# shenyunhang/APE

Hardware: NVIDIA H100
Metric: images_per_sec (higher is better)
Workload: dtype f16

## Files before the change

ape_b200/_lib.py:

```python
import ctypes
import os

import torch

_HERE = os.path.dirname(os.path.abspath(__file__))
LIB_PATH = os.path.join(_HERE, "libape_b200.so")

APE_DTYPE_F32, APE_DTYPE_F16, APE_DTYPE_BF16, APE_DTYPE_E4M3 = 0, 1, 2, 3
_DTYPE_CODE = {torch.float32: APE_DTYPE_F32, torch.float16: APE_DTYPE_F16, torch.bfloat16: APE_DTYPE_BF16,
               torch.float8_e4m3fn: APE_DTYPE_E4M3}

CONTAINER_ONLY = os.environ.get("APE_B200_CONTAINER_ONLY") == "1"


class _NotLoaded:
    def __getattr__(self, name):
        raise RuntimeError(f"libape_b200.so is not loaded (APE_B200_CONTAINER_ONLY=1): `{name}` is unavailable; "
                           "ape_b200 has no CPU / PyTorch fallback")


if CONTAINER_ONLY:
    lib = _NotLoaded()
elif not os.path.exists(LIB_PATH):
    raise ImportError(
        f"{LIB_PATH} not found: build it with `make` (or `python -c 'import __graft_entry__ as g; g.build()'`). "
        "ape_b200 has no CPU / PyTorch fallback."
    )
else:
    lib = ctypes.CDLL(LIB_PATH)

_vp, _i, _i64 = ctypes.c_void_p, ctypes.c_int, ctypes.c_int64


def _declare(lib):

    lib.ape_abi_version.restype = _i
    lib.ape_abi_version.argtypes = []
    lib.ape_last_error.restype = ctypes.c_char_p
    lib.ape_last_error.argtypes = []
    lib.ape_launch_count.restype = ctypes.c_uint64
    lib.ape_launch_count.argtypes = []
    lib.ape_msda_fwd.restype = _i
    lib.ape_msda_fwd.argtypes = [_vp] * 6 + [_i] * 8 + [_vp]
    lib.ape_msda_fwd_variant.restype = _i
    lib.ape_msda_fwd_variant.argtypes = [_vp] * 6 + [_i] * 9 + [_vp]
    lib.ape_msda_fused_fwd.restype = _i
    lib.ape_msda_fused_fwd.argtypes = [_vp, _vp, _vp, _vp, _i64, _vp, _i64, _vp, _i, _vp] + [_i] * 9 + [_vp]

    lib.ape_msda_bwd.restype = _i
    lib.ape_msda_bwd.argtypes = [_vp] * 9 + [_i] * 8 + [_vp]
    lib.ape_msda_pair_values.restype = _i
    lib.ape_msda_pair_values.argtypes = [_vp, _i64, _vp, _vp, _i, _i, _i, _i, _i, _vp]
    lib.ape_msda_pair_supported.restype = _i
    lib.ape_msda_pair_supported.argtypes = [_vp, _i, _i, _i, _i, _i]
    lib.ape_msda_pair_fused_fwd.restype = _i
    lib.ape_msda_pair_fused_fwd.argtypes = [_vp, _vp, _vp, _vp, _vp, _i64, _vp, _i64, _vp, _i, _vp] + [_i] * 12 + [_vp]
    lib.ape_gemm_tn.restype = _i
    lib.ape_gemm_tn.argtypes = [_vp, _i64, _vp, _i64, _vp, _i64, _vp, _vp, _i64] + [_i] * 7 + [_vp]

    lib.ape_gemm_tn_ex.restype = _i
    lib.ape_gemm_tn_ex.argtypes = [_vp, _i64, _vp, _i64, _vp, _i64, _vp, _vp, _i64] + [_i] * 8 + [_vp]
    lib.ape_gemm_tn_fused.restype = _i
    lib.ape_gemm_tn_fused.argtypes = [_vp, _i64, _vp, _i64, _vp, _i64, _vp, _vp, _i64] + [_i] * 8 + [_vp, _i, _vp, ctypes.c_float, ctypes.c_float, _vp, _i, _vp]
    lib.ape_gemm_tn_e4m3.restype = _i
    lib.ape_gemm_tn_e4m3.argtypes = [_vp, _i64, _vp, _i64, _vp, _vp, _vp, _i64, _vp, _i, _i, _i, _i, _i, _vp, _i, _vp]
    lib.ape_conv3x3_nhwc.restype = _i
    lib.ape_conv3x3_nhwc.argtypes = [_vp, _vp, _vp, _vp] + [_i] * 7 + [_vp]
    lib.ape_gemm_set_trace.restype = None
    lib.ape_gemm_set_trace.argtypes = [_vp]
    lib.ape_ffn_fused.restype = _i
    lib.ape_ffn_fused.argtypes = [_vp, _i64, _vp, _i64, _vp, _vp, _i64, _vp, _vp, _i64] + [_i] * 5 + [_vp]
    lib.ape_gemm_tn_rope.restype = _i
    lib.ape_gemm_tn_rope.argtypes = [_vp, _i64, _vp, _i64, _vp, _i64, _vp, _i, _i, _i, _i, _i, _vp, _vp, _vp, _i, _i, _i, _i, _vp]

    lib.ape_layernorm.restype = _i
    lib.ape_layernorm.argtypes = [_vp, _i64, _vp, _i64, _vp, _vp, _vp, _i, _i, ctypes.c_float, _i, _i, _vp]
    lib.ape_layernorm_e4m3.restype = _i
    lib.ape_layernorm_e4m3.argtypes = [_vp, _i64, _vp, _i64, _vp, _vp, _vp, _vp, _i, _i, ctypes.c_float, _i, _vp]
    lib.ape_layernorm_ex.restype = _i
    lib.ape_layernorm_ex.argtypes = [_vp, _i64, _vp, _i64, _vp, _vp, ctypes.c_float, _vp, _vp, ctypes.c_float, _vp, _i64, _i,
                                     _vp, _i64, _vp, _i64, _i, _i, _i, _i, _vp]
    lib.ape_groupnorm_workspace_bytes.restype = _i64
    lib.ape_groupnorm_workspace_bytes.argtypes = [_i, _i, _i]
    lib.ape_groupnorm_nhwc.restype = _i
    lib.ape_groupnorm_nhwc.argtypes = [_vp, _i64, _vp, _i64, _i64, _vp, _vp, _vp, _i, _i, _i, _i, ctypes.c_float, _i, _i, _vp]
    lib.ape_rope_qk.restype = _i
    lib.ape_rope_qk.argtypes = [_vp, _i64, _vp, _vp, _vp, _i, _i, _i, _i, _i, _vp]

    lib.ape_text_embed_packed.restype = _i
    lib.ape_text_embed_packed.argtypes = [_vp] * 5 + [_i] * 4 + [_vp]
    lib.ape_rows_gather.restype = _i
    lib.ape_rows_gather.argtypes = [_vp, _i64, _vp, _vp, _i64, _i, _i, _vp]

    lib.ape_attn_fwd.restype = _i
    lib.ape_attn_fwd.argtypes = [_vp, _i64, _vp, _i64, _i, _i, _i, _i, ctypes.c_float, _i, _vp]
    lib.ape_attn_fwd_ex.restype = _i
    lib.ape_attn_fwd_ex.argtypes = [_vp, _i64, _vp, _i64, _i, _i, _i, _i, _i, ctypes.c_float, _i, _vp, _i, _i, _i64, _vp]
    lib.ape_attn_fwd_mapped.restype = _i
    lib.ape_attn_fwd_mapped.argtypes = [_vp, _i64, _vp, _i64, _i, _i, _i, _i, _i, ctypes.c_float, _i, _vp, _i, _i, _i64, _vp, _vp]
    lib.ape_attn_fwd_seg.restype = _i
    lib.ape_attn_fwd_seg.argtypes = [_vp, _i64, _vp, _i64, _i, _i, _i, _i, _i, ctypes.c_float, _i, _vp, _i, _i, _i64, _vp, _vp]
    lib.ape_attn_variant.restype = _i
    lib.ape_attn_variant.argtypes = [_i]
    lib.ape_attn_cross_fwd.restype = _i
    lib.ape_attn_cross_fwd.argtypes = [_vp, _i64, _vp, _i64, _vp, _i64, _vp, _i64, _i, _i, _i, _i, _i, _i, ctypes.c_float, _i, _vp]
    lib.ape_vlf_pool_workspace_bytes.restype = _i64
    lib.ape_vlf_pool_workspace_bytes.argtypes = [_i, _i, _i, _i]
    lib.ape_vlf_pool.restype = _i
    lib.ape_vlf_pool.argtypes = [_vp, _vp, _vp, _vp, ctypes.POINTER(ctypes.c_void_p), ctypes.POINTER(_i)] + [_i] * 6 + [_vp]
    lib.ape_nms_workspace_bytes.restype = _i64
    lib.ape_nms_workspace_bytes.argtypes = [_i]
    lib.ape_nms_sorted.restype = _i
    lib.ape_nms_sorted.argtypes = [_vp, _i, ctypes.c_float, _vp, _vp, _vp, _vp]
    lib.ape_nms_sorted_dev.restype = _i
    lib.ape_nms_sorted_dev.argtypes = [_vp, _i, _vp, ctypes.c_float, _vp, _vp, _vp, _vp]
    lib.ape_nms_classwise_workspace_bytes.restype = _i64
    lib.ape_nms_classwise_workspace_bytes.argtypes = [_i]
    lib.ape_nms_classwise.restype = _i
    lib.ape_nms_classwise.argtypes = [_vp, _vp, _i64, _vp, _i, _i, ctypes.c_float, ctypes.c_float, _vp, _vp, _vp]
    lib.ape_ref_update.restype = _i
    lib.ape_ref_update.argtypes = [_vp, _vp, _vp, _vp, _vp, _i, _i, _i, ctypes.c_float, _vp]
    lib.ape_gemv_f32.restype = _i
    lib.ape_gemv_f32.argtypes = [_vp, _vp, _vp, _vp, _i, _i, _i, _vp]
    lib.ape_mask_crop_workspace_bytes.restype = _i64
    lib.ape_mask_crop_workspace_bytes.argtypes = [_i, _i, _i]
    lib.ape_mask_crop.restype = _i
    lib.ape_mask_crop.argtypes = [_vp] * 5 + [_i] * 7 + [_vp]
    lib.ape_mask_paste.restype = _i
    lib.ape_mask_paste.argtypes = [_vp, _vp, _vp, _i, _i, _i, _i, ctypes.c_float, _vp]
    lib.ape_mask_paste_rle.restype = _i
    lib.ape_mask_paste_rle.argtypes = [_vp, _vp, _i, _i, _i, _i, ctypes.c_float, _vp, _vp, _vp, _vp]
    lib.ape_rle_to_string.restype = _i
    lib.ape_rle_to_string.argtypes = [_vp, _i, _vp]
    lib.ape_resample_ksize.restype = _i
    lib.ape_resample_ksize.argtypes = [_i, _i]
    lib.ape_resample_coeffs_u8.restype = _i
    lib.ape_resample_coeffs_u8.argtypes = [_i, _i, _vp, _vp]
    lib.ape_resample_u8.restype = _i
    lib.ape_resample_u8.argtypes = [_vp, _i64, _vp, _vp, _i64, _i64, _vp, _vp, _i, _vp, _vp, _i] + [_i] * 6 + [_vp]
    lib.ape_semseg_resample.restype = _i
    lib.ape_semseg_resample.argtypes = [_vp, _vp, _vp, _i64] + [_i] * 13 + [_vp]
    lib.ape_semseg_keys_init.restype = _i
    lib.ape_semseg_keys_init.argtypes = [_vp, _i64, ctypes.c_float, _i, _vp]
    lib.ape_gemm_tn_argmax.restype = _i
    lib.ape_gemm_tn_argmax.argtypes = [_vp, _i64, _vp, _i64, _vp, _i, _i, _i, _i, _i, _vp]
    lib.ape_semseg_keys_decode.restype = _i
    lib.ape_semseg_keys_decode.argtypes = [_vp, _i64, _vp, _vp, _vp]
    lib.ape_panoptic_winners.restype = _i
    lib.ape_panoptic_winners.argtypes = [_vp] * 5 + [_i] * 9 + [ctypes.c_float, _i, _vp]



if not CONTAINER_ONLY:
    _declare(lib)

EXPORTS = (
    "ape_abi_version",
    "ape_last_error",
    "ape_launch_count",
    "ape_msda_fwd",
    "ape_msda_fwd_variant",
    "ape_msda_fused_fwd",
    "ape_msda_bwd",
    "ape_msda_pair_values",
    "ape_msda_pair_supported",
    "ape_msda_pair_fused_fwd",
    "ape_gemm_tn",
    "ape_gemm_tn_ex",
    "ape_gemm_tn_fused",
    "ape_gemm_tn_e4m3",
    "ape_conv3x3_nhwc",
    "ape_gemm_tn_rope",
    "ape_ffn_fused",
    "ape_gemm_set_trace",
    "ape_layernorm",
    "ape_layernorm_e4m3",
    "ape_layernorm_ex",
    "ape_rope_qk",
    "ape_text_embed_packed",
    "ape_rows_gather",
    "ape_attn_fwd",
    "ape_attn_fwd_ex",
    "ape_attn_fwd_mapped",
    "ape_attn_fwd_seg",
    "ape_attn_variant",
    "ape_attn_cross_fwd",
    "ape_groupnorm_workspace_bytes",
    "ape_groupnorm_nhwc",
    "ape_vlf_pool_workspace_bytes",
    "ape_vlf_pool",
    "ape_nms_workspace_bytes",
    "ape_nms_sorted",
    "ape_nms_sorted_dev",
    "ape_nms_classwise_workspace_bytes",
    "ape_nms_classwise",
    "ape_ref_update",
    "ape_gemv_f32",
    "ape_mask_crop_workspace_bytes",
    "ape_mask_crop",
    "ape_mask_paste",
    "ape_mask_paste_rle",
    "ape_rle_to_string",
    "ape_resample_ksize",
    "ape_resample_coeffs_u8",
    "ape_resample_u8",
    "ape_semseg_resample",
    "ape_semseg_keys_init",
    "ape_gemm_tn_argmax",
    "ape_semseg_keys_decode",
    "ape_panoptic_winners",
)


def dtype_code(dt: torch.dtype) -> int:
    try:
        return _DTYPE_CODE[dt]
    except KeyError:
        raise RuntimeError(f"ape_b200: unsupported dtype {dt} (float32 / float16 / bfloat16 / float8_e4m3fn only)") from None


def check(status: int, what: str) -> None:
    if status != 0:
        msg = lib.ape_last_error().decode("utf-8", "replace")
        raise RuntimeError(f"{what} failed (status {status}): {msg}")


def current_stream_ptr() -> int:
    return torch.cuda.current_stream().cuda_stream


def launch_count() -> int:
    return int(lib.ape_launch_count())
```

ape_b200/csrc/ffn_fused.cu:

```cuda
#include "attn.cuh"
#include "common.cuh"
#include "tc.cuh"

namespace ape {
namespace {

constexpr int E = 256, BM = 128, HC = 64;
constexpr int kThreads = 384;

struct alignas(1024) FfnSmem {
  uint8_t x[E / 64][BM * 128];
  uint8_t w1[2][E / 64][HC * 128];
  uint8_t w2[2][E * 128];
  uint64_t x_full, w1_full[2], w1_empty[2], w2_full[2], w2_empty[2];
};

struct FfnParams {
  const float *b1, *b2;
  const void *x;
  float *out;
  long long ldx, ldo;
  int M, F;
};

template <typename T, int CL>
__global__ void __launch_bounds__(kThreads, 1)
ffn_fused_kernel(const __grid_constant__ CUtensorMap map_x, const __grid_constant__ CUtensorMap map_w1,
                 const __grid_constant__ CUtensorMap map_w2, const FfnParams p) {
  extern __shared__ uint8_t smem_raw[];
  pdl_launch_dependents();
  FfnSmem &s = *reinterpret_cast<FfnSmem *>((reinterpret_cast<uintptr_t>(smem_raw) + 1023) & ~uintptr_t(1023));
  const int warp = threadIdx.x >> 5, lane = threadIdx.x & 31;
  const int rank = CL > 1 ? (int)tc::cluster_ctarank() : 0;
  const int row0 = blockIdx.x * BM;
  const int nch = p.F / HC;

  if (warp == 8 && lane == 0) {
    tc::prefetch_tensormap(&map_x);
    tc::prefetch_tensormap(&map_w1);
    tc::prefetch_tensormap(&map_w2);
    tc::mbar_init(&s.x_full, 1);
#pragma unroll
    for (int b = 0; b < 2; ++b) {
      tc::mbar_init(&s.w1_full[b], 1);
      tc::mbar_init(&s.w1_empty[b], 8 * CL);
      tc::mbar_init(&s.w2_full[b], 1);
      tc::mbar_init(&s.w2_empty[b], 8 * CL);
    }
    tc::fence_mbar_init();
  }
  __syncthreads();
  if (CL > 1) tc::cluster_sync_all();
  pdl_wait();

  if (warp >= 8) {
    tc::setmaxnreg_dec<40>();
    if (warp == 8 && lane == 0) {
      tc::mbar_expect_tx(&s.x_full, E * BM * 2);
#pragma unroll
      for (int c = 0; c < E / 64; ++c)
#pragma unroll
        for (int h = 0; h < 2; ++h) tc::tma_load_2d(s.x[c] + h * 64 * 128, &map_x, &s.x_full, c * 64, row0 + h * 64);
      for (int j = 0; j < nch; ++j) {
        const int b = j & 1, n = j >> 1;
        tc::mbar_wait(&s.w1_empty[b], (n & 1) ^ 1);
        tc::mbar_expect_tx(&s.w1_full[b], E * HC * 2);
        if (CL == 1) {
#pragma unroll
          for (int c = 0; c < E / 64; ++c) tc::tma_load_2d(s.w1[b][c], &map_w1, &s.w1_full[b], c * 64, j * HC);
        } else {
#pragma unroll
          for (int c = 2 * rank; c < 2 * rank + 2; ++c)
            tc::tma_load_2d_multicast(s.w1[b][c], &map_w1, &s.w1_full[b], c * 64, j * HC, (uint16_t)3);
        }
        tc::mbar_wait(&s.w2_empty[b], (n & 1) ^ 1);
        tc::mbar_expect_tx(&s.w2_full[b], E * HC * 2);
        if (CL == 1) {
#pragma unroll
          for (int q = 0; q < E / 64; ++q) tc::tma_load_2d(s.w2[b] + q * 64 * 128, &map_w2, &s.w2_full[b], j * HC, q * 64);
        } else {
#pragma unroll
          for (int q = 2 * rank; q < 2 * rank + 2; ++q)
            tc::tma_load_2d_multicast(s.w2[b] + q * 64 * 128, &map_w2, &s.w2_full[b], j * HC, q * 64, (uint16_t)3);
        }
      }
    }
    __syncwarp();
  } else {
    tc::setmaxnreg_inc<232>();
    const int g = warp >> 2, tq = lane & 3;
    auto release = [&](uint64_t *bar) {
      if (lane == 0) {
        tc::mbar_arrive(bar);
        if (CL > 1) tc::mbar_arrive_cluster(tc::mapa_u32(bar, (uint32_t)(rank ^ 1)));
      }
    };
    auto issue_s = [&](float *sc, int b) {
#pragma unroll
      for (int c = 0; c < E / 64; ++c) {
        const uint64_t dx = tc::make_smem_desc_sw128(tc::smem_u32(s.x[c] + g * 64 * 128));
        const uint64_t dw = tc::make_smem_desc_sw128(tc::smem_u32(s.w1[b][c]));
#pragma unroll
        for (int k = 0; k < 4; ++k) tc::Wgmma<64, T>::template ss<0>(sc, dx + 2 * k, dw + 2 * k, (c | k) != 0);
      }
    };
    float o[E / 2];
#pragma unroll
    for (int i = 0; i < E / 2; ++i) o[i] = 0.f;
    float sc[32];
    tc::mbar_wait(&s.x_full, 0);
    tc::mbar_wait(&s.w1_full[0], 0);
    tc::wgmma_fence();
    issue_s(sc, 0);
    tc::wgmma_commit();
    tc::wgmma_wait<0>();
    tc::fence_regs<32>(sc);
    release(&s.w1_empty[0]);

    for (int j = 0; j < nch; ++j) {
      const int b = j & 1, n = j >> 1;
      uint32_t pa[4][4];
#pragma unroll
      for (int jj = 0; jj < 8; ++jj) {
        float2 bb = make_float2(0.f, 0.f);
        if (p.b1 != nullptr) bb = __ldg(reinterpret_cast<const float2 *>(p.b1 + j * HC + 8 * jj + 2 * tq));
#pragma unroll
        for (int h = 0; h < 2; ++h) {
          float v0 = sc[4 * jj + 2 * h], v1 = sc[4 * jj + 2 * h + 1];
          if (p.b1 != nullptr) {
            v0 += bb.x;
            v1 += bb.y;
          }
          pa[jj >> 1][2 * (jj & 1) + h] = attn::pack2<T>(fmaxf(v0, 0.f), fmaxf(v1, 0.f));
        }
      }
      tc::mbar_wait(&s.w2_full[b], n & 1);
      tc::fence_regs<E / 2>(o);
      tc::wgmma_fence();
      const uint64_t dw2 = tc::make_smem_desc_sw128(tc::smem_u32(s.w2[b]));
#pragma unroll
      for (int kk = 0; kk < 4; ++kk) tc::Wgmma<256, T>::template rs<0>(o, pa[kk], dw2 + 2 * kk, (j | kk) != 0);
      tc::wgmma_commit();
      if (j + 1 < nch) {
        const int b1 = b ^ 1;
        tc::mbar_wait(&s.w1_full[b1], ((j + 1) >> 1) & 1);
        issue_s(sc, b1);
        tc::wgmma_commit();
        tc::wgmma_wait<1>();
        tc::fence_regs<E / 2>(o);
        release(&s.w2_empty[b]);
        tc::wgmma_wait<0>();
        tc::fence_regs<32>(sc);
        release(&s.w1_empty[b1]);
      } else {
        tc::wgmma_wait<0>();
        tc::fence_regs<E / 2>(o);
        release(&s.w2_empty[b]);
      }
    }

    const T *xg = reinterpret_cast<const T *>(p.x);
#pragma unroll
    for (int h = 0; h < 2; ++h) {
      const int m = row0 + g * 64 + (warp & 3) * 16 + (lane >> 2) + 8 * h;
      if (m < p.M) {
        const T *xr = xg + (size_t)m * p.ldx + 2 * tq;
        float *dst = p.out + (size_t)m * p.ldo + 2 * tq;
#pragma unroll
        for (int jj = 0; jj < E / 8; ++jj) {
          float v0 = o[4 * jj + 2 * h], v1 = o[4 * jj + 2 * h + 1];
          if (p.b2 != nullptr) {
            const float2 bb = __ldg(reinterpret_cast<const float2 *>(p.b2 + 8 * jj + 2 * tq));
            v0 += bb.x;
            v1 += bb.y;
          }
          const float2 r = Elem<T>::load2(xr + 8 * jj);
          v0 += r.x;
          v1 += r.y;
          *reinterpret_cast<float2 *>(dst + 8 * jj) = make_float2(v0, v1);
        }
      }
    }
  }
  __syncthreads();
  if (CL > 1) tc::cluster_sync_all();
}

template <typename T, int CL>
int launch(const CUtensorMap &mx, const CUtensorMap &m1, const CUtensorMap &m2, const FfnParams &p, cudaStream_t st) {
  const size_t smem = sizeof(FfnSmem) + 1024;
  auto k = ffn_fused_kernel<T, CL>;
  static bool set = false;
  if (!set) {
    cudaError_t e = cudaFuncSetAttribute(k, cudaFuncAttributeMaxDynamicSharedMemorySize, (int)smem);
    if (e != cudaSuccess) return fail((int)e, "ffn_fused: cudaFuncSetAttribute(smem=%zu): %s", smem, cudaGetErrorString(e));
    set = true;
  }
  const int tiles = (p.M + BM - 1) / BM;
  cudaLaunchConfig_t cfg{};
  cfg.gridDim = dim3((unsigned)((tiles + CL - 1) / CL * CL));
  cfg.blockDim = dim3(kThreads);
  cfg.dynamicSmemBytes = smem;
  cfg.stream = st;
  cudaLaunchAttribute attr[2];
  attr[0].id = cudaLaunchAttributeClusterDimension;
  attr[0].val.clusterDim.x = CL;
  attr[0].val.clusterDim.y = 1;
  attr[0].val.clusterDim.z = 1;
  attr[1].id = cudaLaunchAttributeProgrammaticStreamSerialization;
  attr[1].val.programmaticStreamSerializationAllowed = pdl_enabled() ? 1 : 0;
  cfg.attrs = attr;
  cfg.numAttrs = 2;
  cudaError_t e = cudaLaunchKernelEx(&cfg, k, mx, m1, m2, p);
  if (e != cudaSuccess) return fail((int)e, "ffn_fused_kernel launch: %s", cudaGetErrorString(e));
  return check_launch("ffn_fused_kernel");
}

}
}

using namespace ape;

extern "C" int ape_ffn_fused(const void *x, int64_t ldx, const void *w1, int64_t ldw1, const float *b1, const void *w2,
                             int64_t ldw2, const float *b2, float *out, int64_t ldo, int M, int E_, int F, int dtype,
                             int variant, void *stream) {
  if (dtype != APE_DTYPE_F16 && dtype != APE_DTYPE_BF16)
    return fail(APE_ERR_INVALID_ARG, "ffn_fused: operands must be fp16 or bf16 (got dtype %d)", dtype);
  if (E_ != E) return fail(APE_ERR_UNSUPPORTED, "ffn_fused: embedding width %d (only %d)", E_, E);
  if (F <= 0 || F % HC) return fail(APE_ERR_UNSUPPORTED, "ffn_fused: hidden width %d is not a positive multiple of %d", F, HC);
  if (M < 0) return fail(APE_ERR_INVALID_ARG, "ffn_fused: bad row count %d", M);
  if (variant < 0 || variant > 2) return fail(APE_ERR_INVALID_ARG, "ffn_fused: bad variant %d", variant);
  if (ldo == 0) ldo = E;
  if (M == 0) return APE_OK;
  if (!x || !w1 || !w2 || !out) return fail(APE_ERR_NULL_PTR, "ffn_fused: null pointer argument");
  if (((reinterpret_cast<uintptr_t>(x) | reinterpret_cast<uintptr_t>(w1) | reinterpret_cast<uintptr_t>(w2)) & 15) ||
      ldx % 8 || ldw1 % 8 || ldw2 % 8)
    return fail(APE_ERR_INVALID_ARG, "ffn_fused: x / w1 / w2 base and row pitch must be 16-byte aligned (TMA)");
  if (ldx < E || ldw1 < E || ldw2 < F || ldo < E) return fail(APE_ERR_INVALID_ARG, "ffn_fused: row pitch smaller than the row");
  if ((reinterpret_cast<uintptr_t>(out) & 7) || ldo % 2 ||
      ((reinterpret_cast<uintptr_t>(b1) | reinterpret_cast<uintptr_t>(b2)) & 7))
    return fail(APE_ERR_INVALID_ARG, "ffn_fused: out (and its row pitch) and b1 / b2 must allow 8-byte pairs");
  CUtensorMap mx, m1, m2;
  if (int rc = attn::make_map(&mx, x, dtype, M, E, ldx)) return rc;
  if (int rc = attn::make_map(&m1, w1, dtype, F, E, ldw1)) return rc;
  if (int rc = attn::make_map(&m2, w2, dtype, E, F, ldw2)) return rc;
  FfnParams p{b1, b2, x, out, ldx, ldo, M, F};
  const bool cluster = variant == 2;
  cudaStream_t st = reinterpret_cast<cudaStream_t>(stream);
  if (dtype == APE_DTYPE_BF16)
    return cluster ? launch<__nv_bfloat16, 2>(mx, m1, m2, p, st) : launch<__nv_bfloat16, 1>(mx, m1, m2, p, st);
  return cluster ? launch<__half, 2>(mx, m1, m2, p, st) : launch<__half, 1>(mx, m1, m2, p, st);
}
```

ape_b200/csrc/norm_rope.cu:

```cuda
#include <cuda_fp8.h>

#include "common.cuh"

namespace ape {
namespace {

template <typename T>
struct Vec8 {
  static constexpr int kBytes = 8 * sizeof(T);
};

template <typename T>
__device__ __forceinline__ void load8(const T *p, float *f) {
  if constexpr (sizeof(T) == 4) {
    const float4 a = *reinterpret_cast<const float4 *>(p), b = *reinterpret_cast<const float4 *>(p + 4);
    f[0] = a.x; f[1] = a.y; f[2] = a.z; f[3] = a.w; f[4] = b.x; f[5] = b.y; f[6] = b.z; f[7] = b.w;
  } else {
    const uint4 v = *reinterpret_cast<const uint4 *>(p);
    Elem<T>::unpack(v, f);
  }
}
template <typename T>
__device__ __forceinline__ void store8(T *p, const float *f) {
  if constexpr (sizeof(T) == 4) {
    *reinterpret_cast<float4 *>(p) = make_float4(f[0], f[1], f[2], f[3]);
    *reinterpret_cast<float4 *>(p + 4) = make_float4(f[4], f[5], f[6], f[7]);
  } else {
    *reinterpret_cast<uint4 *>(p) = Elem<T>::pack(f);
  }
}

__device__ __forceinline__ float warp_sum(float v) {
#pragma unroll
  for (int o = 16; o > 0; o >>= 1) v += __shfl_xor_sync(0xffffffffu, v, o);
  return v;
}

template <typename TI, typename TO, int MAXV>
__global__ void __launch_bounds__(256)
layernorm_kernel(const TI *__restrict__ x, long long ldx, TO *__restrict__ y, long long ldy,
                 const float *__restrict__ w, const float *__restrict__ b, const int *__restrict__ row_map,
                 int rows, int C, float eps) {
  pdl_prologue();
  const int warp = (blockIdx.x * blockDim.x + threadIdx.x) >> 5, lane = threadIdx.x & 31;
  if (warp >= rows) return;
  const TI *xr = x + (size_t)warp * ldx;
  const int nvec = (C + 7) >> 3;
  float v[MAXV][8];
  float sum = 0.f;
#pragma unroll
  for (int i = 0; i < MAXV; ++i) {
    const int j = lane + 32 * i;
    if (j < nvec) {
      load8<TI>(xr + 8 * j, v[i]);
#pragma unroll
      for (int k = 0; k < 8; ++k) {
        if (8 * j + k >= C) v[i][k] = 0.f;
        sum += v[i][k];
      }
    }
  }
  const float mean = warp_sum(sum) / (float)C;
  float sq = 0.f;
#pragma unroll
  for (int i = 0; i < MAXV; ++i) {
    const int j = lane + 32 * i;
    if (j < nvec) {
#pragma unroll
      for (int k = 0; k < 8; ++k) {
        const float d = (8 * j + k < C) ? v[i][k] - mean : 0.f;
        sq += d * d;
      }
    }
  }
  const float rstd = rsqrtf(warp_sum(sq) / (float)C + eps);
  const int orow = row_map ? row_map[warp] : warp;
  TO *yr = y + (size_t)orow * ldy;
#pragma unroll
  for (int i = 0; i < MAXV; ++i) {
    const int j = lane + 32 * i;
    if (j < nvec) {
      float o[8];
      if (8 * j + 8 <= C) {
        const float4 w0 = __ldg(reinterpret_cast<const float4 *>(w + 8 * j)), w1 = __ldg(reinterpret_cast<const float4 *>(w + 8 * j) + 1);
        const float4 b0 = __ldg(reinterpret_cast<const float4 *>(b + 8 * j)), b1 = __ldg(reinterpret_cast<const float4 *>(b + 8 * j) + 1);
        const float ww[8] = {w0.x, w0.y, w0.z, w0.w, w1.x, w1.y, w1.z, w1.w};
        const float bb[8] = {b0.x, b0.y, b0.z, b0.w, b1.x, b1.y, b1.z, b1.w};
#pragma unroll
        for (int k = 0; k < 8; ++k) o[k] = (v[i][k] - mean) * rstd * ww[k] + bb[k];
      } else {
#pragma unroll
        for (int k = 0; k < 8; ++k)
          o[k] = (8 * j + k < C) ? (v[i][k] - mean) * rstd * __ldg(w + 8 * j + k) + __ldg(b + 8 * j + k) : 0.f;
      }
      store8<TO>(yr + 8 * j, o);
    }
  }
}

template <typename TI, int MAXV>
__global__ void __launch_bounds__(256)
layernorm_e4m3_kernel(const TI *__restrict__ x, long long ldx, uint8_t *__restrict__ y, long long ldy, float *__restrict__ scale,
                      const float *__restrict__ w, const float *__restrict__ b, const int *__restrict__ row_map,
                      int rows, int C, float eps) {
  pdl_prologue();
  const int warp = (blockIdx.x * blockDim.x + threadIdx.x) >> 5, lane = threadIdx.x & 31;
  if (warp >= rows) return;
  const TI *xr = x + (size_t)warp * ldx;
  const int nvec = (C + 7) >> 3;
  float v[MAXV][8];
  float sum = 0.f;
#pragma unroll
  for (int i = 0; i < MAXV; ++i) {
    const int j = lane + 32 * i;
    if (j < nvec) {
      load8<TI>(xr + 8 * j, v[i]);
#pragma unroll
      for (int k = 0; k < 8; ++k) {
        if (8 * j + k >= C) v[i][k] = 0.f;
        sum += v[i][k];
      }
    }
  }
  const float mean = warp_sum(sum) / (float)C;
  float sq = 0.f;
#pragma unroll
  for (int i = 0; i < MAXV; ++i) {
    const int j = lane + 32 * i;
    if (j < nvec) {
#pragma unroll
      for (int k = 0; k < 8; ++k) {
        const float d = (8 * j + k < C) ? v[i][k] - mean : 0.f;
        sq += d * d;
      }
    }
  }
  const float rstd = rsqrtf(warp_sum(sq) / (float)C + eps);
  float amax = 0.f;
#pragma unroll
  for (int i = 0; i < MAXV; ++i) {
    const int j = lane + 32 * i;
    if (j < nvec) {
#pragma unroll
      for (int k = 0; k < 8; ++k) {
        v[i][k] = (8 * j + k < C) ? (v[i][k] - mean) * rstd * __ldg(w + 8 * j + k) + __ldg(b + 8 * j + k) : 0.f;
        amax = fmaxf(amax, fabsf(v[i][k]));
      }
    }
  }
#pragma unroll
  for (int o = 16; o > 0; o >>= 1) amax = fmaxf(amax, __shfl_xor_sync(0xffffffffu, amax, o));
  const float s = amax / 448.f;
  const int orow = row_map ? row_map[warp] : warp;
  uint8_t *yr = y + (size_t)orow * ldy;
#pragma unroll
  for (int i = 0; i < MAXV; ++i) {
    const int j = lane + 32 * i;
    if (j < nvec) {
      uint32_t q[2];
#pragma unroll
      for (int h = 0; h < 2; ++h) {
        float2 lo = make_float2(0.f, 0.f), hi = make_float2(0.f, 0.f);
        if (s > 0.f) {
          lo = make_float2(v[i][4 * h] / s, v[i][4 * h + 1] / s);
          hi = make_float2(v[i][4 * h + 2] / s, v[i][4 * h + 3] / s);
        }
        q[h] = (uint32_t)__nv_cvt_float2_to_fp8x2(lo, __NV_SATFINITE, __NV_E4M3) |
               ((uint32_t)__nv_cvt_float2_to_fp8x2(hi, __NV_SATFINITE, __NV_E4M3) << 16);
      }
      *reinterpret_cast<uint2 *>(yr + 8 * j) = make_uint2(q[0], q[1]);
    }
  }
  if (lane == 0) scale[orow] = s;
}

template <typename TI, typename TO, int MAXV, bool NORM = true>
__global__ void __launch_bounds__(256)
layernorm_ex_kernel(const TI *__restrict__ x, long long ldx, TO *__restrict__ y, long long ldy, const float *__restrict__ w,
                    const float *__restrict__ b, float eps, const float *__restrict__ w2, const float *__restrict__ b2,
                    float eps2, const float *__restrict__ col_add, long long col_add_stride, int rows_per_image,
                    const TO *__restrict__ row_add, long long ld_add, TO *__restrict__ y2, long long ldy2, int rows, int C) {
  pdl_prologue();
  const int warp = (blockIdx.x * blockDim.x + threadIdx.x) >> 5, lane = threadIdx.x & 31;
  if (warp >= rows) return;
  const TI *xr = x + (size_t)warp * ldx;
  const int nvec = C >> 3;
  float v[MAXV][8];
  float sum = 0.f;
#pragma unroll
  for (int i = 0; i < MAXV; ++i) {
    const int j = lane + 32 * i;
    if (j < nvec) {
      load8<TI>(xr + 8 * j, v[i]);
#pragma unroll
      for (int k = 0; k < 8; ++k) sum += v[i][k];
    }
  }
  if constexpr (NORM) {
  float mean = warp_sum(sum) / (float)C;
  float sq = 0.f;
#pragma unroll
  for (int i = 0; i < MAXV; ++i)
    if (lane + 32 * i < nvec) {
#pragma unroll
      for (int k = 0; k < 8; ++k) {
        const float d = v[i][k] - mean;
        sq += d * d;
      }
    }
  float rstd = rsqrtf(warp_sum(sq) / (float)C + eps);
  sum = 0.f;
#pragma unroll
  for (int i = 0; i < MAXV; ++i) {
    const int j = lane + 32 * i;
    if (j < nvec) {
      float ww[8], bb[8];
      load8<float>(w + 8 * j, ww);
      load8<float>(b + 8 * j, bb);
#pragma unroll
      for (int k = 0; k < 8; ++k) {
        v[i][k] = (v[i][k] - mean) * rstd * ww[k] + bb[k];
        sum += v[i][k];
      }
    }
  }
  if (w2) {
    mean = warp_sum(sum) / (float)C;
    sq = 0.f;
#pragma unroll
    for (int i = 0; i < MAXV; ++i)
      if (lane + 32 * i < nvec) {
#pragma unroll
        for (int k = 0; k < 8; ++k) {
          const float d = v[i][k] - mean;
          sq += d * d;
        }
      }
    rstd = rsqrtf(warp_sum(sq) / (float)C + eps2);
#pragma unroll
    for (int i = 0; i < MAXV; ++i) {
      const int j = lane + 32 * i;
      if (j < nvec) {
        float ww[8], bb[8];
        load8<float>(w2 + 8 * j, ww);
        load8<float>(b2 + 8 * j, bb);
#pragma unroll
        for (int k = 0; k < 8; ++k) v[i][k] = (v[i][k] - mean) * rstd * ww[k] + bb[k];
      }
    }
  }
  }
  const float *ca = col_add ? col_add + (size_t)(warp / rows_per_image) * col_add_stride : nullptr;
#pragma unroll
  for (int i = 0; i < MAXV; ++i) {
    const int j = lane + 32 * i;
    if (j < nvec) {
      if (ca) {
        float cc[8];
        load8<float>(ca + 8 * j, cc);
#pragma unroll
        for (int k = 0; k < 8; ++k) v[i][k] += cc[k];
      }
      if (NORM || y) store8<TO>(y + (size_t)warp * ldy + 8 * j, v[i]);
      if (y2) {
        float a[8], o[8];
        load8<TO>(row_add + (size_t)warp * ld_add + 8 * j, a);
        float r[8];
        if constexpr (sizeof(TO) == 4) {
#pragma unroll
          for (int k = 0; k < 8; ++k) r[k] = v[i][k];
        } else {
          Elem<TO>::unpack(Elem<TO>::pack(v[i]), r);
        }
#pragma unroll
        for (int k = 0; k < 8; ++k) o[k] = r[k] + a[k];
        store8<TO>(y2 + (size_t)warp * ldy2 + 8 * j, o);
      }
    }
  }
}

__device__ __forceinline__ float block_sum_256(float v, float *s_part) {
  v = warp_sum(v);
  const int warp = threadIdx.x >> 5, lane = threadIdx.x & 31;
  __syncthreads();
  if (lane == 0) s_part[warp] = v;
  __syncthreads();
  float t = 0.f;
#pragma unroll
  for (int i = 0; i < 8; ++i) t += s_part[i];
  return t;
}

template <typename TI, typename TO>
__global__ void __launch_bounds__(256)
layernorm_wide_kernel(const TI *__restrict__ x, long long ldx, TO *__restrict__ y, long long ldy,
                      const float *__restrict__ w, const float *__restrict__ b, const int *__restrict__ row_map,
                      int rows, int C, float eps) {
  pdl_prologue();
  __shared__ float s_part[8];
  const int row = blockIdx.x;
  const bool wb_aligned = ((reinterpret_cast<uintptr_t>(w) | reinterpret_cast<uintptr_t>(b)) & 15) == 0;
  const TI *xr = x + (size_t)row * ldx;
  const int nvec = (C + 7) >> 3;
  float v[2][8];
  float sum = 0.f;
#pragma unroll
  for (int i = 0; i < 2; ++i) {
    const int j = threadIdx.x + 256 * i;
    if (j < nvec) {
      load8<TI>(xr + 8 * j, v[i]);
#pragma unroll
      for (int k = 0; k < 8; ++k) {
        if (8 * j + k >= C) v[i][k] = 0.f;
        sum += v[i][k];
      }
    }
  }
  const float mean = block_sum_256(sum, s_part) / (float)C;
  float sq = 0.f;
#pragma unroll
  for (int i = 0; i < 2; ++i) {
    const int j = threadIdx.x + 256 * i;
    if (j < nvec) {
#pragma unroll
      for (int k = 0; k < 8; ++k) {
        const float d = (8 * j + k < C) ? v[i][k] - mean : 0.f;
        sq += d * d;
      }
    }
  }
  const float rstd = rsqrtf(block_sum_256(sq, s_part) / (float)C + eps);
  TO *yr = y + (size_t)(row_map ? row_map[row] : row) * ldy;
#pragma unroll
  for (int i = 0; i < 2; ++i) {
    const int j = threadIdx.x + 256 * i;
    if (j < nvec) {
      float o[8];
      if (8 * j + 8 <= C && wb_aligned) {
        float ww[8], bb[8];
        load8<float>(w + 8 * j, ww);
        load8<float>(b + 8 * j, bb);
#pragma unroll
        for (int k = 0; k < 8; ++k) o[k] = (v[i][k] - mean) * rstd * ww[k] + bb[k];
      } else {
#pragma unroll
        for (int k = 0; k < 8; ++k)
          o[k] = (8 * j + k < C) ? (v[i][k] - mean) * rstd * __ldg(w + 8 * j + k) + __ldg(b + 8 * j + k) : 0.f;
      }
      store8<TO>(yr + 8 * j, o);
    }
  }
}

template <typename T>
__global__ void __launch_bounds__(256)
rope_qk_kernel(T *__restrict__ qkv, long long ld, const float *__restrict__ cosr, const float *__restrict__ sinr,
               const int *__restrict__ pos_map, int M, int C, int hd, int npos) {
  pdl_prologue();
  const long long idx = (long long)blockIdx.x * blockDim.x + threadIdx.x;
  const int vec_per_row = 2 * C / 8;
  if (idx >= (long long)M * vec_per_row) return;
  const int m = (int)(idx / vec_per_row), j = (int)(idx % vec_per_row);
  const int col = j * 8;
  const int d = col % hd;
  const int pos = pos_map ? pos_map[m] : m % npos;
  T *p = qkv + (size_t)m * ld + col;
  float t[8], o[8];
  load8<T>(p, t);
  const float *c = cosr + (size_t)pos * hd + d, *s = sinr + (size_t)pos * hd + d;
#pragma unroll
  for (int i = 0; i < 8; i += 2) {
    o[i] = t[i] * c[i] - t[i + 1] * s[i];
    o[i + 1] = t[i + 1] * c[i + 1] + t[i] * s[i + 1];
  }
  store8<T>(p, o);
}

template <typename TI, typename TO>
int launch_ln(const void *x, long long ldx, void *y, long long ldy, const float *w, const float *b, const int *row_map,
              int rows, int C, float eps, cudaStream_t st) {
  const int blocks = (rows + 7) / 8;
  const bool aligned = (reinterpret_cast<uintptr_t>(w) & 15) == 0 && (reinterpret_cast<uintptr_t>(b) & 15) == 0;
  if (C <= 256 && aligned)
    APE_LAUNCH((layernorm_kernel<TI, TO, 1>), blocks, 256, 0, st, (const TI *)x, ldx, (TO *)y, ldy, w, b, row_map, rows, C, eps);
  else if (C <= 1024 && aligned)
    APE_LAUNCH((layernorm_kernel<TI, TO, 4>), blocks, 256, 0, st, (const TI *)x, ldx, (TO *)y, ldy, w, b, row_map, rows, C, eps);
  else
    APE_LAUNCH((layernorm_wide_kernel<TI, TO>), rows, 256, 0, st, (const TI *)x, ldx, (TO *)y, ldy, w, b, row_map, rows, C, eps);
  return check_launch("layernorm_kernel");
}

}
}

using namespace ape;

extern "C" int ape_layernorm(const void *x, int64_t ldx, void *y, int64_t ldy, const float *weight, const float *bias,
                             const int *row_map, int rows, int C, float eps, int in_dtype, int out_dtype, void *stream) {
  if (rows < 0 || C <= 0 || C > 4096) return fail(APE_ERR_INVALID_ARG, "layernorm: rows=%d C=%d (C <= 4096)", rows, C);
  if (ldx < ((C + 7) & ~7) || ldy < ((C + 7) & ~7))
    return fail(APE_ERR_INVALID_ARG, "layernorm: row pitch must cover C rounded up to 8 elements");
  if (rows == 0) return APE_OK;
  if (!x || !y || !weight || !bias) return fail(APE_ERR_NULL_PTR, "layernorm: null pointer argument");
  const int ie = dtype_size(in_dtype), oe = dtype_size(out_dtype);
  if ((ldx * ie) % 16 || (ldy * oe) % 16 || (reinterpret_cast<uintptr_t>(x) & 15) || (reinterpret_cast<uintptr_t>(y) & 15))
    return fail(APE_ERR_INVALID_ARG, "layernorm: rows must be 16-byte aligned");
  cudaStream_t st = reinterpret_cast<cudaStream_t>(stream);
#define APE_LN(TI, TO) return launch_ln<TI, TO>(x, ldx, y, ldy, weight, bias, row_map, rows, C, eps, st)
  if (in_dtype == APE_DTYPE_F32) {
    if (out_dtype == APE_DTYPE_F32) APE_LN(float, float);
    if (out_dtype == APE_DTYPE_F16) APE_LN(float, __half);
    if (out_dtype == APE_DTYPE_BF16) APE_LN(float, __nv_bfloat16);
  } else if (in_dtype == APE_DTYPE_F16) {
    if (out_dtype == APE_DTYPE_F32) APE_LN(__half, float);
    if (out_dtype == APE_DTYPE_F16) APE_LN(__half, __half);
  } else if (in_dtype == APE_DTYPE_BF16) {
    if (out_dtype == APE_DTYPE_F32) APE_LN(__nv_bfloat16, float);
    if (out_dtype == APE_DTYPE_BF16) APE_LN(__nv_bfloat16, __nv_bfloat16);
  }
#undef APE_LN
  return fail(APE_ERR_UNSUPPORTED, "layernorm: dtype pair (%d -> %d) not supported", in_dtype, out_dtype);
}

extern "C" int ape_layernorm_e4m3(const void *x, int64_t ldx, void *y, int64_t ldy, float *scale, const float *weight,
                                  const float *bias, const int *row_map, int rows, int C, float eps, int in_dtype, void *stream) {
  if (rows < 0 || C <= 0 || C > 1024) return fail(APE_ERR_INVALID_ARG, "layernorm_e4m3: rows=%d C=%d (C <= 1024)", rows, C);
  if (ldx < ((C + 7) & ~7) || ldy < ((C + 7) & ~7))
    return fail(APE_ERR_INVALID_ARG, "layernorm_e4m3: row pitch must cover C rounded up to 8 elements");
  if (in_dtype != APE_DTYPE_F32 && in_dtype != APE_DTYPE_F16 && in_dtype != APE_DTYPE_BF16)
    return fail(APE_ERR_UNSUPPORTED, "layernorm_e4m3: input dtype %d not supported", in_dtype);
  if (rows == 0) return APE_OK;
  if (!x || !y || !scale || !weight || !bias) return fail(APE_ERR_NULL_PTR, "layernorm_e4m3: null pointer argument");
  if ((ldx * dtype_size(in_dtype)) % 16 || ldy % 16 || (reinterpret_cast<uintptr_t>(x) & 15) || (reinterpret_cast<uintptr_t>(y) & 15))
    return fail(APE_ERR_INVALID_ARG, "layernorm_e4m3: rows must be 16-byte aligned");
  cudaStream_t st = reinterpret_cast<cudaStream_t>(stream);
  const int blocks = (rows + 7) / 8;
#define APE_LN8(TI)                                                                                                        \
  do {                                                                                                                     \
    if (C <= 256)                                                                                                          \
      APE_LAUNCH((layernorm_e4m3_kernel<TI, 1>), blocks, 256, 0, st, (const TI *)x, ldx, (uint8_t *)y, ldy, scale, weight, bias, \
                 row_map, rows, C, eps);                                                                                   \
    else                                                                                                                   \
      APE_LAUNCH((layernorm_e4m3_kernel<TI, 4>), blocks, 256, 0, st, (const TI *)x, ldx, (uint8_t *)y, ldy, scale, weight, bias, \
                 row_map, rows, C, eps);                                                                                   \
  } while (0)
  if (in_dtype == APE_DTYPE_F32) APE_LN8(float);
  else if (in_dtype == APE_DTYPE_F16) APE_LN8(__half);
  else APE_LN8(__nv_bfloat16);
#undef APE_LN8
  return check_launch("layernorm_e4m3_kernel");
}

extern "C" int ape_layernorm_ex(const void *x, int64_t ldx, void *y, int64_t ldy, const float *weight, const float *bias,
                                float eps, const float *weight2, const float *bias2, float eps2, const float *col_add,
                                int64_t col_add_stride, int rows_per_image, const void *row_add, int64_t ld_add, void *y2,
                                int64_t ldy2, int rows, int C, int in_dtype, int out_dtype, void *stream) {
  if (rows < 0 || C <= 0 || C > 1024 || C % 8 != 0) return fail(APE_ERR_INVALID_ARG, "layernorm_ex: rows=%d C=%d (C %% 8 == 0, C <= 1024)", rows, C);
  if (ldx < C || ldy < C || (y2 && (ldy2 < C || ld_add < C)))
    return fail(APE_ERR_INVALID_ARG, "layernorm_ex: row pitch smaller than C");
  if (rows == 0) return APE_OK;
  const bool norm = weight != nullptr;
  if (!norm && (bias || weight2 || !(y || y2)))
    return fail(APE_ERR_INVALID_ARG, "layernorm_ex: without weight, bias and weight2 must be null and y or y2 given");
  if (!x || (norm && (!y || !bias)) || (weight2 && !bias2) || (y2 && !row_add) || (col_add && rows_per_image <= 0))
    return fail(APE_ERR_NULL_PTR, "layernorm_ex: null pointer argument");
  const int ie = dtype_size(in_dtype), oe = dtype_size(out_dtype);
  const uintptr_t al = reinterpret_cast<uintptr_t>(x) | reinterpret_cast<uintptr_t>(y) | reinterpret_cast<uintptr_t>(y2) |
                       reinterpret_cast<uintptr_t>(row_add) | reinterpret_cast<uintptr_t>(weight) | reinterpret_cast<uintptr_t>(bias) |
                       reinterpret_cast<uintptr_t>(weight2) | reinterpret_cast<uintptr_t>(bias2) | reinterpret_cast<uintptr_t>(col_add);
  if ((ldx * ie) % 16 || (ldy * oe) % 16 || (ldy2 * oe) % 16 || (ld_add * oe) % 16 || (col_add_stride * 4) % 16 || (al & 15))
    return fail(APE_ERR_INVALID_ARG, "layernorm_ex: rows / vectors must be 16-byte aligned");
  cudaStream_t st = reinterpret_cast<cudaStream_t>(stream);
  const int blocks = (rows + 7) / 8;
#define APE_LNX(TI, TO)                                                                                                   \
  do {                                                                                                                    \
    if (!norm && C <= 256)                                                                                                \
      APE_LAUNCH((ape::layernorm_ex_kernel<TI, TO, 1, false>), blocks, 256, 0, st, (const TI *)x, ldx, (TO *)y, ldy, weight, bias, eps, \
          weight2, bias2, eps2, col_add, col_add_stride, rows_per_image > 0 ? rows_per_image : 1, (const TO *)row_add, ld_add, (TO *)y2, \
          ldy2, rows, C);                                                                                                 \
    else if (!norm)                                                                                                       \
      APE_LAUNCH((ape::layernorm_ex_kernel<TI, TO, 4, false>), blocks, 256, 0, st, (const TI *)x, ldx, (TO *)y, ldy, weight, bias, eps, \
          weight2, bias2, eps2, col_add, col_add_stride, rows_per_image > 0 ? rows_per_image : 1, (const TO *)row_add, ld_add, (TO *)y2, \
          ldy2, rows, C);                                                                                                 \
    else if (C <= 256)                                                                                                    \
      APE_LAUNCH((ape::layernorm_ex_kernel<TI, TO, 1>), blocks, 256, 0, st, (const TI *)x, ldx, (TO *)y, ldy, weight, bias, eps, weight2, bias2, eps2, \
          col_add, col_add_stride, rows_per_image > 0 ? rows_per_image : 1, (const TO *)row_add, ld_add, (TO *)y2, ldy2, rows, C);  \
    else                                                                                                                  \
      APE_LAUNCH((ape::layernorm_ex_kernel<TI, TO, 4>), blocks, 256, 0, st, (const TI *)x, ldx, (TO *)y, ldy, weight, bias, eps, weight2, bias2, eps2, \
          col_add, col_add_stride, rows_per_image > 0 ? rows_per_image : 1, (const TO *)row_add, ld_add, (TO *)y2, ldy2, rows, C);  \
    return check_launch("layernorm_ex_kernel");                                                                          \
  } while (0)
  if (in_dtype == APE_DTYPE_F16 && out_dtype == APE_DTYPE_F16) APE_LNX(__half, __half);
  if (in_dtype == APE_DTYPE_BF16 && out_dtype == APE_DTYPE_BF16) APE_LNX(__nv_bfloat16, __nv_bfloat16);
  if (in_dtype == APE_DTYPE_F32 && out_dtype == APE_DTYPE_F32) APE_LNX(float, float);
  if (in_dtype == APE_DTYPE_F32 && out_dtype == APE_DTYPE_F16) APE_LNX(float, __half);
  if (in_dtype == APE_DTYPE_F32 && out_dtype == APE_DTYPE_BF16) APE_LNX(float, __nv_bfloat16);
#undef APE_LNX
  return fail(APE_ERR_UNSUPPORTED, "layernorm_ex: dtype pair (%d -> %d) not supported", in_dtype, out_dtype);
}

extern "C" int ape_rope_qk(void *qkv, int64_t ld, const float *cos_table, const float *sin_table, const int *pos_map,
                           int M, int C, int head_dim, int npos, int dtype, void *stream) {
  if (M < 0 || C <= 0 || head_dim <= 0 || head_dim % 8 != 0 || C % head_dim != 0 || npos <= 0)
    return fail(APE_ERR_INVALID_ARG, "rope: M=%d C=%d head_dim=%d npos=%d", M, C, head_dim, npos);
  if (M == 0) return APE_OK;
  if (!qkv || !cos_table || !sin_table) return fail(APE_ERR_NULL_PTR, "rope: null pointer argument");
  if ((ld * dtype_size(dtype)) % 16 || (reinterpret_cast<uintptr_t>(qkv) & 15))
    return fail(APE_ERR_INVALID_ARG, "rope: rows must be 16-byte aligned");
  cudaStream_t st = reinterpret_cast<cudaStream_t>(stream);
  const long long n = (long long)M * (2 * C / 8);
  const unsigned blocks = (unsigned)((n + 255) / 256);
  if (dtype == APE_DTYPE_F32)
    APE_LAUNCH((rope_qk_kernel<float>), blocks, 256, 0, st, (float *)qkv, ld, cos_table, sin_table, pos_map, M, C, head_dim, npos);
  else if (dtype == APE_DTYPE_F16)
    APE_LAUNCH((rope_qk_kernel<__half>), blocks, 256, 0, st, (__half *)qkv, ld, cos_table, sin_table, pos_map, M, C, head_dim, npos);
  else if (dtype == APE_DTYPE_BF16)
    APE_LAUNCH((rope_qk_kernel<__nv_bfloat16>), blocks, 256, 0, st, (__nv_bfloat16 *)qkv, ld, cos_table, sin_table, pos_map, M, C, head_dim, npos);
  else
    return fail(APE_ERR_INVALID_ARG, "rope: unknown dtype %d", dtype);
  return check_launch("rope_qk_kernel");
}

namespace ape {
namespace {

constexpr int kGnRowsPerCta = 64;

template <typename T>
__global__ void __launch_bounds__(256)
gn_partial_kernel(const T *__restrict__ x, long long ldx, int rows_per_image, int C, int cpg,
                  float *__restrict__ partial ) {
  pdl_prologue();
  const int vec_per_row = C / 8;
  const int b = blockIdx.y, strip = blockIdx.x;
  const int r0 = strip * kGnRowsPerCta, r1 = min(rows_per_image, r0 + kGnRowsPerCta);
  const int v = threadIdx.x % vec_per_row, ro = threadIdx.x / vec_per_row, rstep = 256 / vec_per_row;
  float s = 0.f, ss = 0.f;
  for (int r = r0 + ro; r < r1; r += rstep) {
    float f[8];
    load8<T>(x + ((size_t)b * rows_per_image + r) * ldx + 8 * v, f);
#pragma unroll
    for (int k = 0; k < 8; ++k) { s += f[k]; ss += f[k] * f[k]; }
  }
  __shared__ float sh[256][2];
  sh[threadIdx.x][0] = s;
  sh[threadIdx.x][1] = ss;
  __syncthreads();
  if (threadIdx.x < vec_per_row) {
    float a = 0.f, c = 0.f;
    for (int j = threadIdx.x; j < 256; j += vec_per_row) { a += sh[j][0]; c += sh[j][1]; }
    float *dst = partial + (((size_t)b * gridDim.x + strip) * vec_per_row + threadIdx.x) * 2;
    dst[0] = a;
    dst[1] = c;
  }
}

__global__ void gn_finalize_kernel(const float *__restrict__ partial, int B, int strips, int vec_per_row, int vec_per_group,
                                   float count, float eps, float *__restrict__ stats ) {
  pdl_prologue();
  const int idx = (blockIdx.x * blockDim.x + threadIdx.x) >> 5, lane = threadIdx.x & 31;
  const int G = vec_per_row / vec_per_group;
  if (idx >= B * G) return;
  const int b = idx / G, g = idx % G;
  double s = 0.0, ss = 0.0;
  for (int st = lane; st < strips; st += 32)
    for (int v = 0; v < vec_per_group; ++v) {
      const float2 p = *reinterpret_cast<const float2 *>(partial + (((size_t)b * strips + st) * vec_per_row + g * vec_per_group + v) * 2);
      s += p.x;
      ss += p.y;
    }
#pragma unroll
  for (int o = 16; o > 0; o >>= 1) {
    s += __shfl_xor_sync(0xffffffffu, s, o);
    ss += __shfl_xor_sync(0xffffffffu, ss, o);
  }
  if (lane == 0) {
    const double mean = s / count;
    const double var = fmax(ss / count - mean * mean, 0.0);
    stats[idx * 2] = (float)mean;
    stats[idx * 2 + 1] = (float)(1.0 / sqrt(var + (double)eps));
  }
}

template <typename TI, typename TO>
__global__ void __launch_bounds__(256)
gn_apply_kernel(const TI *__restrict__ x, long long ldx, TO *__restrict__ y, long long ldy, long long y_batch_stride,
                const float *__restrict__ w, const float *__restrict__ bias, const float *__restrict__ stats, int rows_per_image,
                long long total_rows, int C, int vec_per_group) {
  pdl_prologue();
  const int vec_per_row = C / 8;
  const long long idx = (long long)blockIdx.x * blockDim.x + threadIdx.x;
  if (idx >= total_rows * vec_per_row) return;
  const long long row = idx / vec_per_row;
  const int v = (int)(idx % vec_per_row);
  const int b = (int)(row / rows_per_image);
  const int G = vec_per_row / vec_per_group;
  const float mean = stats[(b * G + v / vec_per_group) * 2], rstd = stats[(b * G + v / vec_per_group) * 2 + 1];
  float f[8], o[8];
  load8<TI>(x + (size_t)row * ldx + 8 * v, f);
#pragma unroll
  for (int k = 0; k < 8; ++k) o[k] = (f[k] - mean) * rstd * __ldg(w + 8 * v + k) + __ldg(bias + 8 * v + k);
  store8<TO>(y + (size_t)b * y_batch_stride + (size_t)(row - (long long)b * rows_per_image) * ldy + 8 * v, o);
}

}
}

extern "C" int64_t ape_groupnorm_workspace_bytes(int B, int rows_per_image, int C) {
  const int64_t strips = (rows_per_image + ape::kGnRowsPerCta - 1) / ape::kGnRowsPerCta;
  return ((int64_t)B * strips * (C / 8) * 2 + (int64_t)B * C) * 4;
}

extern "C" int ape_groupnorm_nhwc(const void *x, int64_t ldx, void *y, int64_t ldy, int64_t y_batch_stride,
                                  const float *weight, const float *bias, void *workspace, int B, int rows_per_image, int C, int groups, float eps, int in_dtype,
                                  int out_dtype, void *stream) {
  using namespace ape;
  if (B < 0 || rows_per_image <= 0 || C <= 0 || groups <= 0 || C % groups != 0 || (C / groups) % 8 != 0 || 256 % (C / 8) != 0)
    return fail(APE_ERR_UNSUPPORTED, "groupnorm: C=%d groups=%d (channels per group must be a multiple of 8, C/8 must divide 256)", C, groups);
  if (B == 0) return APE_OK;
  if (!x || !y || !weight || !bias || !workspace) return fail(APE_ERR_NULL_PTR, "groupnorm: null pointer argument");
  if (y_batch_stride == 0) y_batch_stride = (int64_t)rows_per_image * ldy;
  if ((ldx * dtype_size(in_dtype)) % 16 || (ldy * dtype_size(out_dtype)) % 16 || (y_batch_stride * dtype_size(out_dtype)) % 16 ||
      (reinterpret_cast<uintptr_t>(x) & 15) || (reinterpret_cast<uintptr_t>(y) & 15))
    return fail(APE_ERR_INVALID_ARG, "groupnorm: rows must be 16-byte aligned");
  cudaStream_t st = reinterpret_cast<cudaStream_t>(stream);
  const int strips = (rows_per_image + kGnRowsPerCta - 1) / kGnRowsPerCta;
  const int vpr = C / 8, vpg = C / groups / 8;
  float *partial = reinterpret_cast<float *>(workspace);
  float *stats = partial + (size_t)B * strips * vpr * 2;
  if (in_dtype == APE_DTYPE_F32) APE_LAUNCH((gn_partial_kernel<float>), dim3(strips, B), 256, 0, st, (const float *)x, ldx, rows_per_image, C, C / groups, partial);
  else if (in_dtype == APE_DTYPE_F16) APE_LAUNCH((gn_partial_kernel<__half>), dim3(strips, B), 256, 0, st, (const __half *)x, ldx, rows_per_image, C, C / groups, partial);
  else APE_LAUNCH((gn_partial_kernel<__nv_bfloat16>), dim3(strips, B), 256, 0, st, (const __nv_bfloat16 *)x, ldx, rows_per_image, C, C / groups, partial);
  if (int rc = check_launch("gn_partial_kernel")) return rc;
  APE_LAUNCH((gn_finalize_kernel), (B * groups + 3) / 4, 128, 0, st, partial, B, strips, vpr, vpg, (float)rows_per_image * (C / groups), eps, stats);
  if (int rc = check_launch("gn_finalize_kernel")) return rc;
  const long long total_rows = (long long)B * rows_per_image;
  const unsigned blocks = (unsigned)((total_rows * vpr + 255) / 256);
#define APE_GN(TI, TO) APE_LAUNCH((gn_apply_kernel<TI, TO>), blocks, 256, 0, st, (const TI *)x, ldx, (TO *)y, ldy, y_batch_stride, weight, bias, stats, rows_per_image, total_rows, C, vpg)
  if (in_dtype == APE_DTYPE_F32 && out_dtype == APE_DTYPE_F32) APE_GN(float, float);
  else if (in_dtype == APE_DTYPE_F16 && out_dtype == APE_DTYPE_F16) APE_GN(__half, __half);
  else if (in_dtype == APE_DTYPE_BF16 && out_dtype == APE_DTYPE_BF16) APE_GN(__nv_bfloat16, __nv_bfloat16);
  else if (in_dtype == APE_DTYPE_F16 && out_dtype == APE_DTYPE_F32) APE_GN(__half, float);
  else if (in_dtype == APE_DTYPE_BF16 && out_dtype == APE_DTYPE_F32) APE_GN(__nv_bfloat16, float);
  else return fail(APE_ERR_UNSUPPORTED, "groupnorm: dtype pair (%d -> %d) not supported", in_dtype, out_dtype);
#undef APE_GN
  return check_launch("gn_apply_kernel");
}


namespace ape {
namespace {
__global__ void __launch_bounds__(256) gemv_f32_kernel(const float *__restrict__ W, const float *__restrict__ x,
                                                       const float *__restrict__ bias, float *__restrict__ y, int B, int N, int K) {
  pdl_prologue();
  const int warp = (blockIdx.x * blockDim.x + threadIdx.x) >> 5, lane = threadIdx.x & 31;
  if (warp >= N) return;
  const float4 *w4 = reinterpret_cast<const float4 *>(W + (size_t)warp * K);
  float acc[4] = {0.f, 0.f, 0.f, 0.f};
#pragma unroll 4
  for (int k = lane; k < K / 4; k += 32) {
    const float4 w = __ldg(w4 + k);
#pragma unroll
    for (int b = 0; b < 4; ++b) {
      if (b < B) {
        const float4 xv = __ldg(reinterpret_cast<const float4 *>(x + (size_t)b * K) + k);
        acc[b] = fmaf(w.x, xv.x, fmaf(w.y, xv.y, fmaf(w.z, xv.z, fmaf(w.w, xv.w, acc[b]))));
      }
    }
  }
#pragma unroll
  for (int b = 0; b < 4; ++b) {
#pragma unroll
    for (int o = 16; o > 0; o >>= 1) acc[b] += __shfl_xor_sync(0xffffffffu, acc[b], o);
  }
  if (lane == 0) {
    const float bb = bias != nullptr ? __ldg(bias + warp) : 0.f;
    for (int b = 0; b < B && b < 4; ++b) y[(size_t)b * N + warp] = acc[b] + bb;
  }
}
}
}

extern "C" int ape_gemv_f32(const float *W, const float *x, const float *bias, float *y, int B, int N, int K, void *stream) {
  using namespace ape;
  if (!W || !x || !y) return fail(APE_ERR_NULL_PTR, "gemv: null pointer");
  if (B <= 0 || B > 4 || N <= 0 || K <= 0 || K % 4) return fail(APE_ERR_UNSUPPORTED, "gemv: B=%d (1..4) N=%d K=%d (multiple of 4)", B, N, K);
  if ((reinterpret_cast<uintptr_t>(W) | reinterpret_cast<uintptr_t>(x)) & 15) return fail(APE_ERR_INVALID_ARG, "gemv: W / x must be 16-byte aligned");
  APE_LAUNCH(gemv_f32_kernel, (N + 7) / 8, 256, 0, (cudaStream_t)stream, W, x, bias, y, B, N, K);
  return check_launch("gemv_f32_kernel");
}


namespace ape {
namespace {
__global__ void __launch_bounds__(256) ref_update_kernel(const float *__restrict__ delta, const float *__restrict__ ref,
                                                         const float *__restrict__ valid_ratios, float *__restrict__ new_ref,
                                                         float *__restrict__ ref_in, int rows, int Q, int L, float eps) {
  pdl_prologue();
  const int i = blockIdx.x * blockDim.x + threadIdx.x;
  if (i >= rows * 4) return;
  const int row = i >> 2, c = i & 3, b = row / Q;
  float x = fminf(fmaxf(__ldg(ref + i), 0.f), 1.f);
  const float x1 = fmaxf(x, eps), x2 = fmaxf(1.f - x, eps);
  const float y = __ldg(delta + i) + logf(x1 / x2);
  const float r = 1.f / (1.f + expf(-y));
  new_ref[i] = r;
  for (int l = 0; l < L; ++l) ref_in[((size_t)row * L + l) * 4 + c] = r * __ldg(valid_ratios + ((size_t)b * L + l) * 2 + (c & 1));
}
}
}

extern "C" int ape_ref_update(const float *delta, const float *ref, const float *valid_ratios, float *new_ref, float *ref_in, int B,
                              int Q, int L, float eps, void *stream) {
  using namespace ape;
  if (!delta || !ref || !valid_ratios || !new_ref || !ref_in) return fail(APE_ERR_NULL_PTR, "ref_update: null pointer");
  if (B <= 0 || Q <= 0 || L <= 0) return fail(APE_ERR_INVALID_ARG, "ref_update: B=%d Q=%d L=%d", B, Q, L);
  const int n = B * Q * 4;
  APE_LAUNCH(ref_update_kernel, (n + 255) / 256, 256, 0, (cudaStream_t)stream, delta, ref, valid_ratios, new_ref, ref_in, B * Q, Q, L, eps);
  return check_launch("ref_update_kernel");
}


namespace ape {
namespace {
__global__ void __launch_bounds__(256) text_embed_packed_kernel(const float *__restrict__ tok_emb, const float *__restrict__ pos_emb,
                                                                const int *__restrict__ tok, const int *__restrict__ pos,
                                                                float *__restrict__ x, int rows, int D, int vocab, int ctx) {
  pdl_prologue();
  const long long idx = (long long)blockIdx.x * blockDim.x + threadIdx.x;
  const int vec_per_row = D / 4;
  if (idx >= (long long)rows * vec_per_row) return;
  const int r = (int)(idx / vec_per_row), j = (int)(idx % vec_per_row);
  const int t = tok[r], q = pos[r];
  float4 o = make_float4(0.f, 0.f, 0.f, 0.f);
  if (q >= 0 && q < ctx && t >= 0 && t < vocab) {
    const float4 a = __ldg(reinterpret_cast<const float4 *>(tok_emb + (size_t)t * D) + j);
    const float4 b = __ldg(reinterpret_cast<const float4 *>(pos_emb + (size_t)q * D) + j);
    o = make_float4(a.x + b.x, a.y + b.y, a.z + b.z, a.w + b.w);
  }
  reinterpret_cast<float4 *>(x + (size_t)r * D)[j] = o;
}

__global__ void __launch_bounds__(256) rows_gather_kernel(const float *__restrict__ x, long long ldx, const long long *__restrict__ rows,
                                                          float *__restrict__ out, long long ldo, int n, int D) {
  pdl_prologue();
  const long long idx = (long long)blockIdx.x * blockDim.x + threadIdx.x;
  const int vec_per_row = D / 4;
  if (idx >= (long long)n * vec_per_row) return;
  const int i = (int)(idx / vec_per_row), j = (int)(idx % vec_per_row);
  reinterpret_cast<float4 *>(out + (size_t)i * ldo)[j] = reinterpret_cast<const float4 *>(x + (size_t)rows[i] * ldx)[j];
}
}
}

extern "C" int ape_text_embed_packed(const float *token_embedding, const float *positional_embedding, const int *tok, const int *pos,
                                     float *x, int rows, int D, int vocab, int ctx, void *stream) {
  using namespace ape;
  if (rows < 0 || D <= 0 || D % 4 || vocab <= 0 || ctx <= 0)
    return fail(APE_ERR_INVALID_ARG, "text_embed_packed: rows=%d D=%d (multiple of 4) vocab=%d ctx=%d", rows, D, vocab, ctx);
  if (rows == 0) return APE_OK;
  if (!token_embedding || !positional_embedding || !tok || !pos || !x) return fail(APE_ERR_NULL_PTR, "text_embed_packed: null pointer argument");
  if ((reinterpret_cast<uintptr_t>(token_embedding) | reinterpret_cast<uintptr_t>(positional_embedding) | reinterpret_cast<uintptr_t>(x)) & 15)
    return fail(APE_ERR_INVALID_ARG, "text_embed_packed: tables and x must be 16-byte aligned");
  const long long n = (long long)rows * (D / 4);
  APE_LAUNCH(text_embed_packed_kernel, (unsigned)((n + 255) / 256), 256, 0, (cudaStream_t)stream, token_embedding, positional_embedding,
             tok, pos, x, rows, D, vocab, ctx);
  return check_launch("text_embed_packed_kernel");
}

extern "C" int ape_rows_gather(const float *x, int64_t ldx, const int64_t *rows, float *out, int64_t ldo, int n, int D, void *stream) {
  using namespace ape;
  if (n < 0 || D <= 0 || D % 4 || ldx < D || ldo < D) return fail(APE_ERR_INVALID_ARG, "rows_gather: n=%d D=%d (multiple of 4, pitches >= D)", n, D);
  if (n == 0) return APE_OK;
  if (!x || !rows || !out) return fail(APE_ERR_NULL_PTR, "rows_gather: null pointer argument");
  if (ldx % 4 || ldo % 4 || ((reinterpret_cast<uintptr_t>(x) | reinterpret_cast<uintptr_t>(out)) & 15))
    return fail(APE_ERR_INVALID_ARG, "rows_gather: rows must be 16-byte aligned");
  const long long nv = (long long)n * (D / 4);
  APE_LAUNCH(rows_gather_kernel, (unsigned)((nv + 255) / 256), 256, 0, (cudaStream_t)stream, x, (long long)ldx,
             reinterpret_cast<const long long *>(rows), out, (long long)ldo, n, D);
  return check_launch("rows_gather_kernel");
}
```

ape_b200/layers/common.py:

```python
import torch
import torch.nn as nn
import torch.nn.functional as F


class LayerNorm2d(nn.Module):

    def __init__(self, channels, eps=1e-6):
        super().__init__()
        self.weight = nn.Parameter(torch.ones(channels))
        self.bias = nn.Parameter(torch.zeros(channels))
        self.eps = eps

    def forward(self, x):
        return F.layer_norm(x.permute(0, 2, 3, 1), (x.shape[1],), self.weight, self.bias, self.eps).permute(0, 3, 1, 2)


class ConvNorm(nn.Conv2d):

    def __init__(self, cin, cout, kernel_size, padding=0, bias=True, norm=None, activation=None):
        super().__init__(cin, cout, kernel_size, padding=padding, bias=bias)
        self.norm = norm
        self.activation = activation

    def forward(self, x):
        x = F.conv2d(x, self.weight, self.bias, self.stride, self.padding)
        if self.norm is not None:
            x = self.norm(x)
        if self.activation is not None:
            x = self.activation(x)
        return x


class MLP(nn.Module):

    def __init__(self, input_dim, hidden_dim, output_dim, num_layers):
        super().__init__()
        self.num_layers = num_layers
        h = [hidden_dim] * (num_layers - 1)
        self.layers = nn.ModuleList(nn.Linear(n, k) for n, k in zip([input_dim] + h, h + [output_dim]))

    def forward(self, x, out_dtype=None):
        if x.is_cuda and x.dtype in (torch.float16, torch.bfloat16):
            from .. import ops

            for i, layer in enumerate(self.layers):
                last = i == self.num_layers - 1
                x = ops.linear_module_tc(layer, x, act=None if last else "relu", out_dtype=out_dtype if last else None)
            return x
        for i, layer in enumerate(self.layers):
            x = F.relu(layer(x)) if i < self.num_layers - 1 else layer(x)
        return x


class FFN(nn.Module):

    def __init__(self, embed_dim, feedforward_dim):
        super().__init__()
        self.layers = nn.Sequential(
            nn.Sequential(nn.Linear(embed_dim, feedforward_dim), nn.ReLU(inplace=True), nn.Dropout(0.0)),
            nn.Linear(feedforward_dim, embed_dim),
            nn.Dropout(0.0),
        )

    def forward(self, x, out_dtype=None):
        if x.is_cuda and x.dtype in (torch.float16, torch.bfloat16):
            from .. import ops

            fc1, fc2 = self.layers[0][0], self.layers[1]
            if out_dtype == torch.float32 and x.shape[-1] == 256 and fc1.out_features % 64 == 0:
                w1, b1 = ops.packed(fc1, x.dtype)
                w2, b2 = ops.packed(fc2, x.dtype)
                return ops.ffn_fused(x, w1, b1, w2, b2)
            h = ops.linear_module_tc(fc1, x, act="relu")
            return ops.linear_module_tc(fc2, h, residual=x.contiguous(), out_dtype=out_dtype)
        return x + self.layers[1](F.relu(self.layers[0][0](x)))


def inverse_sigmoid(x, eps=1e-3):
    x = x.clamp(min=0, max=1)
    return torch.log(x.clamp(min=eps) / (1 - x).clamp(min=eps))


def box_cxcywh_to_xyxy(b):
    cx, cy, w, h = b.unbind(-1)
    return torch.stack([cx - 0.5 * w, cy - 0.5 * h, cx + 0.5 * w, cy + 0.5 * h], dim=-1)
```

ape_b200/modeling/transformer.py:

```python
import copy
import math

import torch
import torch.nn as nn
import torch.nn.functional as F
import torchvision

from .. import ops
from ..layers import MultiScaleDeformableAttention
from ..layers.common import FFN, box_cxcywh_to_xyxy, inverse_sigmoid


class _SelfAttention(nn.Module):

    def __init__(self, embed_dim, num_heads):
        super().__init__()
        self.embed_dim, self.num_heads = embed_dim, num_heads
        self.attn = nn.MultiheadAttention(embed_dim, num_heads, dropout=0.0, batch_first=True)

    def _packed(self, dtype):
        w, b = self.attn.in_proj_weight, self.attn.in_proj_bias
        wo, bo = self.attn.out_proj.weight, self.attn.out_proj.bias
        E, nh = self.embed_dim, self.num_heads
        hd = E // nh

        def build():
            def pad_rows(wpart, bpart):
                wp = wpart.new_zeros(nh, 64, E)
                wp[:, :hd] = wpart.view(nh, hd, E)
                bp = bpart.new_zeros(nh, 64)
                bp[:, :hd] = bpart.view(nh, hd)
                return wp.view(nh * 64, E), bp.view(nh * 64)
            wq, bq = pad_rows(w[:E], b[:E])
            wk, bk = pad_rows(w[E:2 * E], b[E:2 * E])
            wv, bv = pad_rows(w[2 * E:], b[2 * E:])
            wop = wo.new_zeros(E, nh, 64)
            wop[:, :, :hd] = wo.view(E, nh, hd)
            return (torch.cat([wq, wk], 0).detach().to(dtype).contiguous(), torch.cat([bq, bk]).detach().float().contiguous(),
                    wv.detach().to(dtype).contiguous(), bv.detach().float().contiguous(),
                    wop.view(E, nh * 64).detach().to(dtype).contiguous(), bo.detach().float().contiguous())

        return ops.cached(self, "_pk", dtype, (w._version, b._version, wo._version, bo._version, w.data_ptr()), build)

    def forward(self, x, pos):
        E, nh = self.embed_dim, self.num_heads
        if x.is_cuda and x.dtype in (torch.float16, torch.bfloat16) and E // nh <= 64:
            wqk, bqk, wv, bv, wo, bo = self._packed(x.dtype)
            B, N, _ = x.shape
            NP = (N + 127) // 128 * 128
            C = nh * 64
            bk = (B, NP, C, x.dtype, str(x.device))
            bufs = self.__dict__.setdefault("_qkv_bufs", {})
            if bk not in bufs:
                bufs[bk] = torch.zeros((B, NP, 3 * C), dtype=x.dtype, device=x.device)
            buf = bufs[bk]
            xp = x + pos.to(x.dtype)
            for b in range(B):
                ops.linear_tc(xp[b], wqk, bqk, out=buf[b, :N, : 2 * C])
                ops.linear_tc(x[b], wv, bv, out=buf[b, :N, 2 * C:])
            o = ops.attention_qkv(buf.view(B * NP, 3 * C), B, NP, nh, 64, (E // nh) ** -0.5, n_valid=N).view(B, NP, C)
            outs = [ops.linear_tc(o[b, :N], wo, bo, residual=x[b].contiguous(), out_dtype=torch.float32) for b in range(B)]
            return outs[0].unsqueeze(0) if B == 1 else torch.stack(outs)
        w, b = self.attn.in_proj_weight, self.attn.in_proj_bias
        qk = F.linear(x + pos, w[: 2 * E], b[: 2 * E])
        v = F.linear(x, w[2 * E:], b[2 * E:])
        B, N, _ = x.shape
        q, k = qk[..., :E], qk[..., E:]
        q, k, v = (t.reshape(B, N, nh, E // nh).transpose(1, 2) for t in (q, k, v))
        o = F.scaled_dot_product_attention(q, k, v).transpose(1, 2).reshape(B, N, E)
        return x + self.attn.out_proj(o)


class _EncoderLayer(nn.Module):

    def __init__(self, embed_dim, num_heads, ffn_dim, num_levels):
        super().__init__()
        self.embed_dim = embed_dim
        self.pre_norm = False
        self.attentions = nn.ModuleList([MultiScaleDeformableAttention(
            embed_dim=embed_dim, num_heads=num_heads, dropout=0.0, batch_first=True, num_levels=num_levels)])
        self.ffns = nn.ModuleList([FFN(embed_dim, ffn_dim)])
        self.norms = nn.ModuleList([nn.LayerNorm(embed_dim), nn.LayerNorm(embed_dim)])

    def forward(self, query, query_pos, key_padding_mask, reference_points, spatial_shapes, level_start_index,
                host_shapes=None, query_with_pos=None, defer_last_norm=False):
        x = self.attentions[0](query, None, query, None, query_pos=query_pos, key_padding_mask=key_padding_mask,
                               reference_points=reference_points, spatial_shapes=spatial_shapes,
                               level_start_index=level_start_index, host_shapes=host_shapes,
                               query_with_pos=query_with_pos,
                               sum_dtype=torch.float32 if query.dtype != torch.float32 else None)
        if query.dtype in (torch.float16, torch.bfloat16):
            x = ops.layernorm_module(self.norms[0], x, out_dtype=query.dtype)
            x = self.ffns[0](x, out_dtype=torch.float32)
            if defer_last_norm:
                return x
            return ops.layernorm_module(self.norms[1], x, out_dtype=query.dtype)
        x = self.norms[0](x)
        x = self.ffns[0](x)
        return self.norms[1](x)


class _DecoderLayer(nn.Module):

    def __init__(self, embed_dim, num_heads, ffn_dim, num_levels):
        super().__init__()
        self.embed_dim = embed_dim
        self.pre_norm = False
        self.attentions = nn.ModuleList([
            _SelfAttention(embed_dim, num_heads),
            MultiScaleDeformableAttention(embed_dim=embed_dim, num_heads=num_heads, dropout=0.0, batch_first=True,
                                          num_levels=num_levels)])
        self.ffns = nn.ModuleList([FFN(embed_dim, ffn_dim)])
        self.norms = nn.ModuleList([nn.LayerNorm(embed_dim) for _ in range(3)])

    def forward(self, query, value, query_pos, key_padding_mask, reference_points, spatial_shapes, level_start_index):
        if query.is_cuda and query.dtype in (torch.float16, torch.bfloat16) and value.dtype == query.dtype:
            dt = query.dtype
            x = self.attentions[0](query, query_pos)
            x = ops.layernorm_module(self.norms[0], x, out_dtype=dt)
            x = self.attentions[1](x, None, value, None, query_pos=query_pos.to(dt), key_padding_mask=key_padding_mask,
                                   reference_points=reference_points, spatial_shapes=spatial_shapes,
                                   level_start_index=level_start_index, sum_dtype=torch.float32)
            x = ops.layernorm_module(self.norms[1], x, out_dtype=dt)
            x = self.ffns[0](x, out_dtype=torch.float32)
            return ops.layernorm_module(self.norms[2], x, out_dtype=dt)
        x = self.attentions[0](query, query_pos)
        x = self.norms[0](x)
        x = self.attentions[1](x, None, value, None, query_pos=query_pos, key_padding_mask=key_padding_mask,
                               reference_points=reference_points, spatial_shapes=spatial_shapes,
                               level_start_index=level_start_index)
        x = self.norms[1](x)
        x = self.ffns[0](x)
        return self.norms[2](x)


class DeformableDetrTransformerEncoderVL(nn.Module):
    def __init__(self, embed_dim=256, num_heads=8, feedforward_dim=1024, attn_dropout=0.1, ffn_dropout=0.1,
                 num_layers=6, post_norm=False, num_feature_levels=4, vl_layer=None, use_act_checkpoint=False,
                 pytorch_attn=False):
        super().__init__()
        self.num_layers = num_layers
        self.layers = nn.ModuleList([_EncoderLayer(embed_dim, num_heads, feedforward_dim, num_feature_levels)
                                     for _ in range(num_layers)])
        self.embed_dim = embed_dim
        self.pre_norm = False
        self.post_norm_layer = nn.LayerNorm(embed_dim) if post_norm else None
        self.vl_layers = nn.ModuleList([copy.deepcopy(vl_layer) for _ in range(num_layers)])
        self.record_taps = False

    def forward(self, query, key, value, query_l, attention_mask_l, query_pos=None, key_pos=None, attn_masks=None,
                query_key_padding_mask=None, key_padding_mask=None, **kwargs):
        engine_dtype = torch.get_autocast_dtype("cuda") if torch.is_autocast_enabled("cuda") else None
        if engine_dtype is not None:
            query, query_pos = query.to(engine_dtype), query_pos.to(engine_dtype)
            if query_l is not None and query_l.shape[1] == 1 and attention_mask_l is None and query.shape[-1] % 8 == 0 \
                    and all(v is not None and not v.b_attn.attn.use_attention_mask_v for v in self.vl_layers):
                return self._engine_single_token(query.contiguous(), query_pos.contiguous(), query_l,
                                                 query_key_padding_mask, kwargs)
        if self.record_taps:
            self.taps = {}
        for i, (vl_layer, layer) in enumerate(zip(self.vl_layers, self.layers)):
            if vl_layer is not None and query_l is not None:
                query, query_l = vl_layer(query, query_l, attention_mask_v=query_key_padding_mask,
                                          attention_mask_l=attention_mask_l)
                if engine_dtype is not None:
                    query = query.to(engine_dtype)
                if self.record_taps:
                    self.taps[f"vlf{i}.v"] = query
            query = layer(query, query_pos, query_key_padding_mask, kwargs["reference_points"],
                          kwargs["spatial_shapes"], kwargs["level_start_index"], kwargs.get("host_shapes"))
            if self.record_taps:
                self.taps[f"enc{i}"] = query
        if self.post_norm_layer is not None:
            query = self.post_norm_layer(query)
        return query, query_l

    def _engine_single_token(self, x, query_pos, query_l, key_padding_mask, kwargs):
        pending = None
        dt = x.dtype
        if self.record_taps:
            self.taps = {}
        for i, (vl_layer, layer) in enumerate(zip(self.vl_layers, self.layers)):
            b = vl_layer.b_attn
            with torch.autocast("cuda", enabled=False):
                ln_l = ops.layernorm(query_l.float().contiguous(), b.layer_norm_l.weight.float(), b.layer_norm_l.bias.float(),
                                     eps=b.layer_norm_l.eps, out_dtype=torch.float32)
                dv, qa, qc = b.single_token_language_side(ln_l)
                shift = (b.gamma_v.float() * dv.float()).reshape(x.shape[0], -1).contiguous()
            vw, vb = ops.packed(b.layer_norm_v, dt)
            if pending is None:
                query, qpos = ops.layernorm_ex(x, vw, vb, b.layer_norm_v.eps, col_add=shift, row_add=query_pos, out_dtype=dt)
            else:
                query, qpos = ops.layernorm_ex(x, pending[0], pending[1], pending[2], weight2=vw, bias2=vb,
                                               eps2=b.layer_norm_v.eps, col_add=shift, row_add=query_pos, out_dtype=dt)
            if self.record_taps:
                self.taps[f"vlf{i}.v"] = query
            with torch.autocast("cuda", enabled=False):
                dl = b.single_token_pool(query, qa, qc, shift=shift)
                query_l = ln_l + b.gamma_l.float() * dl
            x = layer(query, query_pos, key_padding_mask, kwargs["reference_points"], kwargs["spatial_shapes"],
                      kwargs["level_start_index"], kwargs.get("host_shapes"), query_with_pos=qpos, defer_last_norm=True)
            nw, nb = ops.packed(layer.norms[1], dt)
            pending = (nw, nb, layer.norms[1].eps)
        x = ops.layernorm(x, pending[0], pending[1], eps=pending[2], out_dtype=dt)
        if self.post_norm_layer is not None:
            x = self.post_norm_layer(x)
        return x, query_l


class DeformableDetrTransformerDecoderVL(nn.Module):
    def __init__(self, embed_dim=256, num_heads=8, feedforward_dim=1024, attn_dropout=0.1, ffn_dropout=0.1,
                 num_layers=6, return_intermediate=True, num_feature_levels=4, use_act_checkpoint=False,
                 look_forward_twice=False, pytorch_attn=False):
        super().__init__()
        self.num_layers = num_layers
        self.layers = nn.ModuleList([_DecoderLayer(embed_dim, num_heads, feedforward_dim, num_feature_levels)
                                     for _ in range(num_layers)])
        self.return_intermediate = return_intermediate
        self.bbox_embed = None
        self.class_embed = None
        self.look_forward_twice = look_forward_twice

    def forward(self, query, key, value, query_pos=None, key_pos=None, attn_masks=None, query_key_padding_mask=None,
                key_padding_mask=None, reference_points=None, valid_ratios=None, **kwargs):
        output = query
        engine_dtype = torch.get_autocast_dtype("cuda") if torch.is_autocast_enabled("cuda") else None
        if engine_dtype is not None and value.dtype == engine_dtype:
            output, query_pos = output.to(engine_dtype), query_pos.to(engine_dtype)
        intermediate, intermediate_ref = [], []
        fused_ref = engine_dtype is not None and self.bbox_embed is not None and reference_points.is_cuda and \
            reference_points.shape[-1] == 4 and reference_points.dtype == torch.float32
        next_ref_in = None
        for i, layer in enumerate(self.layers):
            if next_ref_in is not None:
                ref_in = next_ref_in
            elif reference_points.shape[-1] == 4:
                ref_in = reference_points[:, :, None] * torch.cat([valid_ratios, valid_ratios], -1)[:, None]
            else:
                ref_in = reference_points[:, :, None] * valid_ratios[:, None]
            output = layer(output, value, query_pos, key_padding_mask, ref_in, kwargs["spatial_shapes"],
                           kwargs["level_start_index"])
            if self.bbox_embed is not None:
                tmp = self.bbox_embed[i](output, out_dtype=torch.float32).float()
                if fused_ref:
                    new_ref, next_ref_in = ops.ref_update(tmp, reference_points, valid_ratios)
                elif reference_points.shape[-1] == 4:
                    new_ref = (tmp + inverse_sigmoid(reference_points)).sigmoid()
                else:
                    new_ref = tmp
                    new_ref[..., :2] = tmp[..., :2] + inverse_sigmoid(reference_points)
                    new_ref = new_ref.sigmoid()
                reference_points = new_ref.detach()
            if self.return_intermediate:
                intermediate.append(output)
                intermediate_ref.append(new_ref if self.look_forward_twice else reference_points)
        if self.return_intermediate:
            return torch.stack(intermediate), torch.stack(intermediate_ref)
        return output, reference_points


class DeformableDetrTransformerVL(nn.Module):
    def __init__(self, encoder=None, decoder=None, num_feature_levels=4, as_two_stage=False,
                 two_stage_num_proposals=300, assign_first_stage=False, pre_nms_topk=1000, nms_thresh_enc=0.9,
                 proposal_ambiguous=0):
        super().__init__()
        if not (as_two_stage and assign_first_stage):
            raise NotImplementedError("ape_b200: only the two-stage / assign_first_stage configuration APE uses")
        self.encoder, self.decoder = encoder, decoder
        self.num_feature_levels = num_feature_levels
        self.as_two_stage = as_two_stage
        self.two_stage_num_proposals = two_stage_num_proposals
        self.assign_first_stage = assign_first_stage
        self.pre_nms_topk = pre_nms_topk
        self.nms_thresh_enc = nms_thresh_enc
        self.proposal_ambiguous = proposal_ambiguous
        self.embed_dim = encoder.embed_dim
        E = self.embed_dim
        self.level_embeds = nn.Parameter(torch.Tensor(num_feature_levels, E))
        self.enc_output = nn.Linear(E, E)
        self.enc_output_norm = nn.LayerNorm(E)
        self.pos_trans = nn.Linear(E * 2, E * 2)
        self.pos_trans_norm = nn.LayerNorm(E * 2)
        self.pix_trans = nn.Linear(E, E)
        self.pix_trans_norm = nn.LayerNorm(E)
        self.init_weights()

    def init_weights(self):
        for p in self.parameters():
            if p.dim() > 1:
                nn.init.xavier_uniform_(p)
        for m in self.modules():
            if isinstance(m, MultiScaleDeformableAttention):
                m.init_weights()
        nn.init.normal_(self.level_embeds)

    def gen_encoder_output_proposals(self, memory, memory_padding_mask, spatial_shapes, mask_prompt_flatten=None):
        N, S, C = memory.shape
        dev = memory.device
        proposals, level_ids = [], []
        cur = 0
        for lvl, (H, W) in enumerate(spatial_shapes):
            m = memory_padding_mask[:, cur:cur + H * W].view(N, H, W, 1)
            valid_H = torch.sum(~m[:, :, 0, 0], 1)
            valid_W = torch.sum(~m[:, 0, :, 0], 1)
            gy, gx = torch.meshgrid(torch.linspace(0, H - 1, H, dtype=torch.float32, device=dev),
                                    torch.linspace(0, W - 1, W, dtype=torch.float32, device=dev), indexing="ij")
            grid = torch.cat([gx.unsqueeze(-1), gy.unsqueeze(-1)], -1)
            scale = torch.cat([valid_W.unsqueeze(-1), valid_H.unsqueeze(-1)], 1).view(N, 1, 1, 2)
            grid = (grid.unsqueeze(0).expand(N, -1, -1, -1) + 0.5) / scale
            wh = torch.ones_like(grid) * 0.05 * (2.0 ** lvl)
            proposals.append(torch.cat((grid, wh), -1).view(N, -1, 4))
            cur += H * W
            level_ids.append(grid.new_ones(H * W, dtype=torch.long) * lvl)
        out = torch.cat(proposals, 1)
        valid = ((out > 0.01) & (out < 0.99)).all(-1, keepdim=True)
        out = torch.log(out / (1 - out))
        out = out.masked_fill(memory_padding_mask.unsqueeze(-1), float("inf"))
        out = out.masked_fill(~valid, float("inf"))
        mem = memory.masked_fill(memory_padding_mask.unsqueeze(-1), float(0)).masked_fill(~valid, float(0))
        if mask_prompt_flatten is not None:
            out = out.masked_fill(~mask_prompt_flatten.unsqueeze(-1), float("inf"))
            mem = mem.masked_fill(~mask_prompt_flatten.unsqueeze(-1), float(0))
        mem = self.enc_output_norm(self.enc_output(mem))
        return mem, out.to(mem.dtype), torch.cat(level_ids)

    @staticmethod
    def get_reference_points(spatial_shapes, valid_ratios, device):
        pts = []
        for lvl, (H, W) in enumerate(spatial_shapes):
            ry, rx = torch.meshgrid(torch.linspace(0.5, H - 0.5, H, dtype=torch.float32, device=device),
                                    torch.linspace(0.5, W - 0.5, W, dtype=torch.float32, device=device), indexing="ij")
            ry = ry.reshape(-1)[None] / (valid_ratios[:, None, lvl, 1] * H)
            rx = rx.reshape(-1)[None] / (valid_ratios[:, None, lvl, 0] * W)
            pts.append(torch.stack((rx, ry), -1))
        ref = torch.cat(pts, 1)
        return ref[:, :, None] * valid_ratios[:, None]

    @staticmethod
    def get_valid_ratio(mask):
        _, H, W = mask.shape
        vh = torch.sum(~mask[:, :, 0], 1).float() / H
        vw = torch.sum(~mask[:, 0, :], 1).float() / W
        return torch.stack([vw, vh], -1)

    @staticmethod
    def get_proposal_pos_embed(proposals, num_pos_feats=128, temperature=10000):
        dim_t = torch.arange(num_pos_feats, dtype=torch.float32, device=proposals.device)
        dim_t = temperature ** (2 * torch.div(dim_t, 2, rounding_mode="floor") / num_pos_feats)
        proposals = proposals.sigmoid() * (2 * math.pi)
        pos = proposals[:, :, :, None] / dim_t
        return torch.stack((pos[:, :, :, 0::2].sin(), pos[:, :, :, 1::2].cos()), dim=4).flatten(2)

    def select_proposals(self, logit, coord_unact, level_ids, n_levels):
        topk = self.two_stage_num_proposals
        S = logit.size(0)
        fallback = torch.sort(logit, descending=True, stable=True)[1][: min(topk, S)]
        if S < topk:
            return fallback
        dev = logit.device
        boxes = box_cxcywh_to_xyxy(coord_unact.sigmoid()).clamp(0, 1)
        lvls = torch.arange(n_levels, device=dev)
        lvl_mask = level_ids[None] == lvls[:, None]
        k = min(self.pre_nms_topk, S)
        pre = torch.sort(logit.sigmoid()[None] * lvl_mask, dim=1, descending=True, stable=True)[1][:, :k].reshape(-1)
        b = boxes[pre].float()
        sc = logit[pre].float()
        ids = level_ids[pre]
        b = b + (ids.to(b) * (b.max() + 1))[:, None]
        order = sc.sort(0, descending=True)[1]
        keep_mask, count = ops.nms_sorted_mask(b.index_select(0, order).contiguous(), self.nms_thresh_enc)
        cand = pre[order]
        kept = keep_mask.bool()
        q_per_l = topk // n_levels
        per_lvl = (level_ids[cand][None] == lvls[:, None]) & kept[None]
        km = (per_lvl & (per_lvl.cumsum(1) <= q_per_l)).any(0)
        num_to_add = topk - km.sum()
        extra = kept & ~km
        km = km | (extra & (extra.cumsum(0) <= num_to_add))
        sel = torch.nonzero_static(km, size=topk, fill_value=0)[:, 0]
        picked = cand[sel]
        return torch.where(count.to(torch.int64) < topk, fallback, picked)

    def geometry(self, shapes, multi_level_masks, multi_level_pos_embeds):
        dev = multi_level_masks[0].device
        mask_flatten = torch.cat([m.flatten(1) for m in multi_level_masks], 1)
        pos_flatten = torch.cat([p.flatten(2).transpose(1, 2) for p in multi_level_pos_embeds], 1)
        spatial_shapes = torch.as_tensor(shapes, dtype=torch.long, device=dev)
        level_start_index = torch.cat((spatial_shapes.new_zeros((1,)), spatial_shapes.prod(1).cumsum(0)[:-1]))
        valid_ratios = torch.stack([self.get_valid_ratio(m) for m in multi_level_masks], 1).to(torch.float32)
        reference_points = self.get_reference_points(shapes, valid_ratios, dev).to(torch.float32)
        N = mask_flatten.shape[0]
        proposals, level_ids = [], []
        cur = 0
        for lvl, (H, W) in enumerate(shapes):
            m = mask_flatten[:, cur:cur + H * W].view(N, H, W, 1)
            valid_H = torch.sum(~m[:, :, 0, 0], 1)
            valid_W = torch.sum(~m[:, 0, :, 0], 1)
            gy, gx = torch.meshgrid(torch.linspace(0, H - 1, H, dtype=torch.float32, device=dev),
                                    torch.linspace(0, W - 1, W, dtype=torch.float32, device=dev), indexing="ij")
            grid = torch.cat([gx.unsqueeze(-1), gy.unsqueeze(-1)], -1)
            scale = torch.cat([valid_W.unsqueeze(-1), valid_H.unsqueeze(-1)], 1).view(N, 1, 1, 2)
            grid = (grid.unsqueeze(0).expand(N, -1, -1, -1) + 0.5) / scale
            wh = torch.ones_like(grid) * 0.05 * (2.0 ** lvl)
            proposals.append(torch.cat((grid, wh), -1).view(N, -1, 4))
            cur += H * W
            level_ids.append(grid.new_ones(H * W, dtype=torch.long) * lvl)
        out = torch.cat(proposals, 1)
        valid = ((out > 0.01) & (out < 0.99)).all(-1, keepdim=True)
        out = torch.log(out / (1 - out))
        out = out.masked_fill(mask_flatten.unsqueeze(-1), float("inf")).masked_fill(~valid, float("inf"))
        return dict(shapes=list(shapes), mask_flatten=mask_flatten, pos_flatten=pos_flatten, spatial_shapes=spatial_shapes,
                    level_start_index=level_start_index, valid_ratios=valid_ratios, reference_points=reference_points,
                    output_proposals=out, proposal_invalid=mask_flatten.unsqueeze(-1) | ~valid,
                    level_ids=torch.cat(level_ids), has_padding=bool(mask_flatten.any()))

    def _encode(self, feat_flatten, pos_flatten, geo, query_l, attention_mask_l):
        return self.encoder(
            query=feat_flatten, key=None, value=None, query_l=query_l, attention_mask_l=attention_mask_l,
            query_pos=pos_flatten, query_key_padding_mask=geo["mask_flatten"] if geo["has_padding"] else None,
            spatial_shapes=geo["spatial_shapes"], reference_points=geo["reference_points"],
            level_start_index=geo["level_start_index"], valid_ratios=geo["valid_ratios"],
            host_shapes=geo["shapes"])

    def stage_encode(self, multi_level_feats, geo, query_l, attention_mask_l=None, mask_prompt_flatten=None,
                     feat_flatten=None):
        if feat_flatten is None:
            feat_flatten = torch.cat([f.flatten(2).transpose(1, 2) for f in multi_level_feats], 1)
        engine_dtype = torch.get_autocast_dtype("cuda") if torch.is_autocast_enabled("cuda") else torch.float32
        ck = (self.level_embeds._version, self.level_embeds.data_ptr())
        cache = geo.setdefault("_pos_lvl", {})
        if engine_dtype not in cache or cache[engine_dtype][0] != ck:
            with torch.no_grad():
                lvl_embed = torch.cat([self.level_embeds[i].view(1, 1, -1).expand(1, h * w, -1)
                                       for i, (h, w) in enumerate(geo["shapes"])], 1)
                cache[engine_dtype] = (ck, (geo["pos_flatten"] + lvl_embed.float()).to(engine_dtype).contiguous())
        pos_flatten = cache[engine_dtype][1]
        memory, query_l = self._encode(feat_flatten, pos_flatten, geo, query_l, attention_mask_l)
        output_proposals = geo["output_proposals"]
        invalid = geo["proposal_invalid"]
        if mask_prompt_flatten is not None:
            output_proposals = output_proposals.masked_fill(~mask_prompt_flatten.unsqueeze(-1), float("inf"))
            invalid = invalid | ~mask_prompt_flatten.unsqueeze(-1)
        nd = self.decoder.num_layers
        if memory.is_cuda and memory.dtype in (torch.float16, torch.bfloat16):
            output_memory, enc_cls, enc_coord = self._engine_proposal_heads(memory, invalid, output_proposals, nd)
            return memory, query_l, output_memory, enc_cls, enc_coord
        output_memory = self.enc_output_norm(self.enc_output(memory.masked_fill(invalid, float(0))))
        output_proposals = output_proposals.to(output_memory.dtype)
        enc_cls = self.decoder.class_embed[nd](output_memory)
        enc_coord = self.decoder.bbox_embed[nd](output_memory) + output_proposals
        if self.proposal_ambiguous:
            cls_all = torch.stack([enc_cls] + [m(output_memory) for m in self.decoder.class_embed_ambiguous], dim=1)
            coord_all = torch.stack([enc_coord] + [m(output_memory) + output_proposals
                                                   for m in self.decoder.bbox_embed_ambiguous], dim=1)
            idx = torch.argmax(cls_all, dim=1, keepdim=True)
            enc_cls = torch.gather(cls_all, 1, idx).squeeze(1)
            enc_coord = torch.gather(coord_all, 1, idx.repeat(1, 1, 1, 4)).squeeze(1)
        return memory, query_l, output_memory, enc_cls, enc_coord

    def _engine_proposal_heads(self, memory, invalid, output_proposals, nd):
        dt = memory.dtype
        cls_mods = [self.decoder.class_embed[nd]] + (list(self.decoder.class_embed_ambiguous) if self.proposal_ambiguous else [])
        box_mods = [self.decoder.bbox_embed[nd]] + (list(self.decoder.bbox_embed_ambiguous) if self.proposal_ambiguous else [])
        params = [p for m in cls_mods + box_mods for p in m.parameters()]
        def build():
            E = self.embed_dim
            wc = torch.zeros(8, E, device=memory.device, dtype=dt)
            bc = torch.zeros(8, device=memory.device, dtype=torch.float32)
            for j, m in enumerate(cls_mods):
                wc[j] = m.weight[0].to(dt)
                bc[j] = m.bias[0].float()
            w0 = torch.cat([m.layers[0].weight for m in box_mods], 0).to(dt).contiguous()
            b0 = torch.cat([m.layers[0].bias for m in box_mods], 0).float().contiguous()
            rest = []
            for m in box_mods:
                mids = [(l.weight.detach().to(dt).contiguous(), l.bias.detach().float().contiguous()) for l in m.layers[1:-1]]
                wl = torch.zeros(8, m.layers[-1].weight.shape[1], device=memory.device, dtype=dt)
                bl = torch.zeros(8, device=memory.device, dtype=torch.float32)
                wl[:4] = m.layers[-1].weight.to(dt)
                bl[:4] = m.layers[-1].bias.float()
                rest.append((mids, wl, bl))
            return wc, bc, w0, b0, rest, len(cls_mods)

        wc, bc, w0, b0, rest, n = ops.cached(self, "_heads_pk", dt, (tuple(p._version for p in params), params[0].data_ptr()), build)
        om = ops.linear_module_tc(self.enc_output, memory.masked_fill(invalid, float(0)))
        output_memory = ops.layernorm_module(self.enc_output_norm, om)
        B, S, E = output_memory.shape
        cls_all = ops.linear_tc(output_memory, wc, bc, out_dtype=torch.float32)[..., :n]
        h0 = ops.linear_tc(output_memory, w0, b0, act="relu")
        props = output_proposals.float()
        coords = []
        for j, (mids, wl, bl) in enumerate(rest):
            h = h0[..., j * E:(j + 1) * E]
            for (w, b) in mids:
                h = ops.linear_tc(h, w, b, act="relu")
            coords.append(ops.linear_tc(h, wl, bl, out_dtype=torch.float32)[..., :4] + props)
        if n == 1:
            return output_memory, cls_all, coords[0]
        idx = torch.argmax(cls_all, dim=-1, keepdim=True)
        enc_cls = torch.gather(cls_all, 2, idx)
        coord_all = torch.stack(coords, dim=2)
        enc_coord = torch.gather(coord_all, 2, idx.unsqueeze(-1).expand(-1, -1, 1, 4)).squeeze(2)
        return output_memory, enc_cls, enc_coord

    def stage_select(self, enc_cls, enc_coord, geo):
        logit = enc_cls[..., 0].float()
        coord = enc_coord.float()
        return torch.stack([self.select_proposals(logit[b], coord[b], geo["level_ids"], len(geo["shapes"]))
                            for b in range(logit.shape[0])])

    def stage_decode(self, memory, output_memory, enc_coord, topk_proposals, geo):
        c = memory.shape[-1]
        topk_unact = torch.gather(enc_coord.float(), 1, topk_proposals.unsqueeze(-1).repeat(1, 1, 4)).detach()
        reference = topk_unact.sigmoid()
        topk_feats = torch.gather(output_memory, 1, topk_proposals.unsqueeze(-1).expand(-1, -1, c)).detach()
        if memory.is_cuda and memory.dtype in (torch.float16, torch.bfloat16):
            emb = self.get_proposal_pos_embed(topk_unact).to(memory.dtype)
            pos_trans_out = ops.layernorm_module(self.pos_trans_norm, ops.linear_module_tc(self.pos_trans, emb))
            query_pos, query = torch.split(pos_trans_out, c, dim=2)
            query = query + ops.layernorm_module(self.pix_trans_norm, ops.linear_module_tc(self.pix_trans, topk_feats.to(memory.dtype)))
        else:
            pos_trans_out = self.pos_trans_norm(self.pos_trans(self.get_proposal_pos_embed(topk_unact).to(topk_unact.dtype)))
            query_pos, query = torch.split(pos_trans_out, c, dim=2)
            query = query + self.pix_trans_norm(self.pix_trans(topk_feats))
        inter_states, inter_references = self.decoder(
            query=query, key=None, value=memory, query_pos=query_pos,
            key_padding_mask=geo["mask_flatten"] if geo["has_padding"] else None,
            reference_points=reference, spatial_shapes=geo["spatial_shapes"],
            level_start_index=geo["level_start_index"], valid_ratios=geo["valid_ratios"])
        return inter_states, reference, inter_references

    def forward(self, multi_level_feats, multi_level_masks, multi_level_pos_embeds, query_embed, query_l,
                attention_mask_l, multi_level_masks_prompt, **kwargs):
        shapes = [(int(f.shape[2]), int(f.shape[3])) for f in multi_level_feats]
        geo = kwargs.get("geometry") or self.geometry(shapes, multi_level_masks, multi_level_pos_embeds)
        mask_prompt_flatten = None
        if multi_level_masks_prompt is not None:
            mask_prompt_flatten = torch.cat([m.flatten(1) for m in multi_level_masks_prompt], 1)
        memory, query_l, output_memory, enc_cls, enc_coord = self.stage_encode(
            multi_level_feats, geo, query_l, attention_mask_l, mask_prompt_flatten)
        topk_proposals = self.stage_select(enc_cls, enc_coord, geo)
        inter_states, init_reference_out, inter_references = self.stage_decode(
            memory, output_memory, enc_coord, topk_proposals, geo)
        self.last_topk_proposals = topk_proposals
        return (inter_states, init_reference_out, inter_references, enc_cls, enc_coord,
                geo["output_proposals"].sigmoid(), memory, query_l)


class DeformableDetrTransformerEncoder(DeformableDetrTransformerEncoderVL):

    def __init__(self, embed_dim=256, num_heads=8, feedforward_dim=1024, attn_dropout=0.1, ffn_dropout=0.1, num_layers=6,
                 post_norm=False, num_feature_levels=4, use_act_checkpoint=False, pytorch_attn=False):
        super().__init__(embed_dim=embed_dim, num_heads=num_heads, feedforward_dim=feedforward_dim, attn_dropout=attn_dropout,
                         ffn_dropout=ffn_dropout, num_layers=num_layers, post_norm=post_norm,
                         num_feature_levels=num_feature_levels, vl_layer=None, use_act_checkpoint=use_act_checkpoint,
                         pytorch_attn=pytorch_attn)
        del self.vl_layers

    def forward(self, query, key, value, query_pos=None, key_pos=None, attn_masks=None, query_key_padding_mask=None,
                key_padding_mask=None, **kwargs):
        engine_dtype = torch.get_autocast_dtype("cuda") if torch.is_autocast_enabled("cuda") else None
        if engine_dtype is not None:
            query, query_pos = query.to(engine_dtype), query_pos.to(engine_dtype)
            if query.is_cuda and query.shape[-1] % 8 == 0:
                return self._engine_schedule(query.contiguous(), query_pos.contiguous(), query_key_padding_mask, kwargs)
        if self.record_taps:
            self.taps = {}
        for i, layer in enumerate(self.layers):
            query = layer(query, query_pos, query_key_padding_mask, kwargs["reference_points"], kwargs["spatial_shapes"],
                          kwargs["level_start_index"], kwargs.get("host_shapes"))
            if self.record_taps:
                self.taps[f"enc{i}"] = query
        if self.post_norm_layer is not None:
            query = self.post_norm_layer(query)
        return query

    def _engine_schedule(self, x, query_pos, key_padding_mask, kwargs):
        dt = x.dtype
        if self.record_taps:
            self.taps = {}
        _, qpos = ops.layernorm_ex(x, None, None, 0.0, row_add=query_pos)
        last = len(self.layers) - 1
        for i, layer in enumerate(self.layers):
            s = layer(x, query_pos, key_padding_mask, kwargs["reference_points"], kwargs["spatial_shapes"],
                      kwargs["level_start_index"], kwargs.get("host_shapes"), query_with_pos=qpos, defer_last_norm=True)
            nw, nb = ops.packed(layer.norms[1], dt)
            if i < last:
                x, qpos = ops.layernorm_ex(s, nw, nb, layer.norms[1].eps, row_add=query_pos, out_dtype=dt)
            else:
                x = ops.layernorm(s, nw, nb, eps=layer.norms[1].eps, out_dtype=dt)
            if self.record_taps:
                self.taps[f"enc{i}"] = x
        if self.post_norm_layer is not None:
            x = self.post_norm_layer(x)
        return x


class DeformableDetrTransformerDecoder(DeformableDetrTransformerDecoderVL):

    def __init__(self, embed_dim=256, num_heads=8, feedforward_dim=1024, attn_dropout=0.1, ffn_dropout=0.1, num_layers=6,
                 return_intermediate=True, num_feature_levels=4, use_act_checkpoint=False, pytorch_attn=False):
        super().__init__(embed_dim=embed_dim, num_heads=num_heads, feedforward_dim=feedforward_dim, attn_dropout=attn_dropout,
                         ffn_dropout=ffn_dropout, num_layers=num_layers, return_intermediate=return_intermediate,
                         num_feature_levels=num_feature_levels, use_act_checkpoint=use_act_checkpoint,
                         look_forward_twice=False, pytorch_attn=pytorch_attn)


class DeformableDetrTransformer(DeformableDetrTransformerVL):

    def gen_encoder_output_proposals(self, memory, memory_padding_mask, spatial_shapes):
        return super().gen_encoder_output_proposals(memory, memory_padding_mask, spatial_shapes)

    def _encode(self, feat_flatten, pos_flatten, geo, query_l, attention_mask_l):
        if query_l is not None or attention_mask_l is not None:
            raise ValueError("ape_b200.DeformableDetrTransformer has no fusion layers: language features go to the classifier")
        memory = self.encoder(
            query=feat_flatten, key=None, value=None, query_pos=pos_flatten,
            query_key_padding_mask=geo["mask_flatten"] if geo["has_padding"] else None,
            spatial_shapes=geo["spatial_shapes"], reference_points=geo["reference_points"],
            level_start_index=geo["level_start_index"], valid_ratios=geo["valid_ratios"], host_shapes=geo["shapes"])
        return memory, None

    def forward(self, multi_level_feats, multi_level_masks, multi_level_pos_embeds, query_embed, **kwargs):
        return super().forward(multi_level_feats, multi_level_masks, multi_level_pos_embeds, query_embed, None, None, None,
                               **kwargs)[:7]
```

ape_b200/ops.py:

```python
import ctypes

import torch

from . import _lib

_NS = "ape"

PROFILE_EVENTS = None


class _timed:
    def __init__(self, tag):
        self.tag = tag

    def __enter__(self):
        if PROFILE_EVENTS is not None:
            self.a = torch.cuda.Event(enable_timing=True)
            self.b = torch.cuda.Event(enable_timing=True)
            self.a.record()
        return self

    def __exit__(self, *exc):
        if PROFILE_EVENTS is not None:
            self.b.record()
            PROFILE_EVENTS.append((self.tag, self.a, self.b))
        return False
_FWD_SCHEMA = (
    "ms_deform_attn_forward(Tensor value, Tensor spatial_shapes, Tensor level_start_index, "
    "Tensor sampling_loc, Tensor attn_weight, int im2col_step) -> Tensor"
)
_BWD_SCHEMA = (
    "ms_deform_attn_backward(Tensor value, Tensor spatial_shapes, Tensor level_start_index, "
    "Tensor sampling_loc, Tensor attn_weight, Tensor grad_output, int im2col_step) -> Tensor[]"
)


def _require(cond: bool, msg: str) -> None:
    if not cond:
        raise RuntimeError(msg)


def _check_inputs(value, spatial_shapes, level_start_index, sampling_loc, attn_weight):
    for name, t in (
        ("value", value),
        ("spatial_shapes", spatial_shapes),
        ("level_start_index", level_start_index),
        ("sampling_loc", sampling_loc),
        ("attn_weight", attn_weight),
    ):
        _require(t.is_contiguous(), f"{name} tensor has to be contiguous")
        _require(t.is_cuda, f"{name} must be a CUDA tensor")
    _require(value.dim() == 4, "value must be [B,S,H,D]")
    _require(sampling_loc.dim() == 6 and sampling_loc.size(-1) == 2, "sampling_loc must be [B,Q,H,L,P,2]")
    _require(spatial_shapes.dtype == torch.int64 and level_start_index.dtype == torch.int64,
             "spatial_shapes / level_start_index must be int64")
    _require(sampling_loc.dtype == value.dtype and attn_weight.dtype == value.dtype,
             "sampling_loc / attn_weight must have value's dtype")
    B, S, H, D = value.shape
    _, Q, H2, L, P, _ = sampling_loc.shape
    _require(H2 == H and sampling_loc.size(0) == B, "sampling_loc shape does not match value")
    _require(tuple(attn_weight.shape) == (B, Q, H, L, P), "attn_weight must be [B,Q,H,L,P]")
    _require(spatial_shapes.shape == (L, 2) and level_start_index.shape == (L,), "bad level tensors")
    return B, S, H, D, L, Q, P


def ms_deform_attn_forward(value, spatial_shapes, level_start_index, sampling_loc, attn_weight,
                           im2col_step=64, variant=-1):
    if not value.is_cuda:
        raise RuntimeError("Not implemented on the CPU")
    B, S, H, D, L, Q, P = _check_inputs(value, spatial_shapes, level_start_index, sampling_loc, attn_weight)
    out = torch.empty((B, Q, H * D), dtype=value.dtype, device=value.device)
    with torch.cuda.device(value.device):
        rc = _lib.lib.ape_msda_fwd_variant(
            value.data_ptr(), spatial_shapes.data_ptr(), level_start_index.data_ptr(),
            sampling_loc.data_ptr(), attn_weight.data_ptr(), out.data_ptr(),
            B, S, H, D, L, Q, P, _lib.dtype_code(value.dtype), int(variant), _lib.current_stream_ptr())
    _lib.check(rc, "ape_msda_fwd")
    return out


def ms_deform_attn_fused_forward(value, spatial_shapes, level_start_index, sampling_offsets,
                                 attention_logits, reference_points, num_points):
    B, S, H, D = value.shape
    L = spatial_shapes.shape[0]
    Q = sampling_offsets.shape[1]
    P = int(num_points)
    _require(value.is_cuda and value.is_contiguous(), "value must be a contiguous CUDA tensor")
    ref = _check_fused(sampling_offsets, attention_logits, reference_points, B, Q, L)
    out = torch.empty((B, Q, H * D), dtype=value.dtype, device=value.device)
    with torch.cuda.device(value.device), _timed(("msda_fused", B, S, Q, L, P, value.element_size(),
                                                  sampling_offsets.element_size())):
        rc = _lib.lib.ape_msda_fused_fwd(
            value.data_ptr(), spatial_shapes.data_ptr(), level_start_index.data_ptr(),
            sampling_offsets.data_ptr(), sampling_offsets.stride(1),
            attention_logits.data_ptr(), attention_logits.stride(1),
            ref.data_ptr(), ref.shape[-1], out.data_ptr(),
            B, S, H, D, L, Q, P, _lib.dtype_code(value.dtype), _lib.dtype_code(sampling_offsets.dtype),
            _lib.current_stream_ptr())
    _lib.check(rc, "ape_msda_fused_fwd")
    return out


def _check_fused(sampling_offsets, attention_logits, reference_points, B, Q, L):
    _require(sampling_offsets.dtype == attention_logits.dtype, "offsets/logits dtype mismatch")
    _require(sampling_offsets.stride(-1) == 1 and attention_logits.stride(-1) == 1, "unit inner stride required")
    _require(sampling_offsets.stride(0) == Q * sampling_offsets.stride(1), "offsets batch stride")
    _require(attention_logits.stride(0) == Q * attention_logits.stride(1), "logits batch stride")
    ref = reference_points
    _require(ref.dtype == torch.float32 and ref.is_contiguous(), "reference_points must be contiguous fp32")
    _require(ref.shape[:3] == (B, Q, L), "reference_points must be [B,Q,L,2|4]")
    return ref


def msda_pair_supported(host_shapes, H, D, P, dtype):
    if dtype not in (torch.float16, torch.bfloat16):
        return False
    L = len(host_shapes)
    hs = (ctypes.c_int * (2 * L))(*[int(v) for hw in host_shapes for v in hw])
    return bool(_lib.lib.ape_msda_pair_supported(hs, L, int(H), int(D), int(P), _lib.dtype_code(dtype)))


def msda_pair_values(value, num_heads, token_mask=None):
    _require(value.is_cuda and value.dim() == 3 and value.stride(2) == 1 and value.stride(0) == value.shape[1] * value.stride(1),
             "msda_pair_values: CUDA [B,S,C] with uniform row pitch")
    B, S, C = value.shape
    H = int(num_heads)
    out = torch.empty((B, S, H, 2, C // H), dtype=value.dtype, device=value.device)
    mptr = None
    if token_mask is not None:
        token_mask = token_mask.to(torch.uint8).contiguous()
        _require(token_mask.numel() == B * S, "msda_pair_values: token_mask must be [B,S]")
        mptr = token_mask.data_ptr()
    with torch.cuda.device(value.device), _timed(("msda_pair_values", B, S, C)):
        rc = _lib.lib.ape_msda_pair_values(value.data_ptr(), value.stride(1), out.data_ptr(), mptr, B, S, H, C // H,
                                           _lib.dtype_code(value.dtype), _lib.current_stream_ptr())
    _lib.check(rc, "ape_msda_pair_values")
    return out


PAIR_TILE_W, PAIR_HEAD_MAJOR = -1, 0


def ms_deform_attn_pair_fused_forward(value2, spatial_shapes, level_start_index, host_shapes, sampling_offsets,
                                      attention_logits, reference_points, num_points, heads_per_cta=0, tile_w=None,
                                      head_major=None):
    B, S, H, two, D = value2.shape
    L = spatial_shapes.shape[0]
    Q = sampling_offsets.shape[1]
    _require(value2.is_cuda and value2.is_contiguous() and two == 2, "value2 must be a contiguous CUDA [B,S,H,2,D] tensor")
    ref = _check_fused(sampling_offsets, attention_logits, reference_points, B, Q, L)
    hs = (ctypes.c_int * (2 * L))(*[int(v) for hw in host_shapes for v in hw])
    out = torch.empty((B, Q, H * D), dtype=value2.dtype, device=value2.device)
    with torch.cuda.device(value2.device), _timed(("msda_fused", B, S, Q, L, int(num_points), value2.element_size(),
                                                   sampling_offsets.element_size())):
        rc = _lib.lib.ape_msda_pair_fused_fwd(
            value2.data_ptr(), spatial_shapes.data_ptr(), level_start_index.data_ptr(), hs,
            sampling_offsets.data_ptr(), sampling_offsets.stride(1), attention_logits.data_ptr(),
            attention_logits.stride(1), ref.data_ptr(), ref.shape[-1], out.data_ptr(), B, S, H, D, L, Q, int(num_points),
            _lib.dtype_code(value2.dtype), _lib.dtype_code(sampling_offsets.dtype), int(heads_per_cta),
            int(PAIR_TILE_W if tile_w is None else tile_w) if Q == S else 0,
            int(PAIR_HEAD_MAJOR if head_major is None else head_major), _lib.current_stream_ptr())
    _lib.check(rc, "ape_msda_pair_fused_fwd")
    return out


ACT = {None: 0, "none": 0, "relu": 1, "gelu": 2, "swiglu": 3, "clamp": 4}


def linear_tc(x, weight, bias=None, act=None, out_dtype=None, residual=None, tile_n=0, out=None, ln_fold=None, stats_out=False):
    _require(x.is_cuda and weight.is_cuda, "linear_tc: CUDA tensors only")
    _require(x.dtype == weight.dtype and x.dtype in (torch.float16, torch.bfloat16), "linear_tc: fp16/bf16 operands")
    K = x.shape[-1]
    N = weight.shape[0]
    _require(weight.shape[1] == K and x.stride(-1) == 1 and weight.stride(-1) == 1, "linear_tc: bad operand layout")
    x2 = x.reshape(-1, K)
    if x2.stride(0) % 8 or x2.data_ptr() % 16:
        x2 = x2.contiguous()
    _require(weight.stride(0) % 8 == 0 and weight.data_ptr() % 16 == 0, "linear_tc: weight rows must be 16-byte aligned")
    M = x2.shape[0]
    n_out = N // 2 if act == "swiglu" else N
    if out is None:
        out_dtype = out_dtype or x.dtype
        out = torch.empty((M, n_out), dtype=out_dtype, device=x.device)
        ret_view = True
    else:
        _require(out.dim() == 2 and out.shape == (M, n_out) and out.stride(1) == 1 and out.is_cuda, "linear_tc: bad `out`")
        out_dtype = out.dtype
        ret_view = False
    res_ptr, ldr, res_dt = None, 0, 0
    if residual is not None:
        r2 = residual.reshape(-1, n_out)
        _require(r2.stride(1) == 1 and r2.is_cuda, "linear_tc: residual needs unit inner stride")
        res_ptr, ldr, res_dt = r2.data_ptr(), r2.stride(0), _lib.dtype_code(r2.dtype)
    if bias is not None:
        _require(bias.dtype == torch.float32 and bias.is_contiguous() and bias.numel() == N, "linear_tc: bias must be fp32 [N]")
    stats = None
    if ln_fold is not None or stats_out:
        part, colsum, nparts, inv_c, eps = None, None, 0, 0.0, 0.0
        if ln_fold is not None:
            part, colsum, C, eps = ln_fold
            _require(part.dtype == torch.float32 and part.is_contiguous() and part.dim() == 3 and part.shape[0] == M and
                     part.shape[2] == 2, "linear_tc: ln_fold partials must be fp32 [M, nparts, 2]")
            _require(colsum.dtype == torch.float32 and colsum.is_contiguous() and colsum.numel() == N, "linear_tc: colsum fp32 [N]")
            nparts, inv_c = part.shape[1], 1.0 / float(C)
        nslab = 0
        if stats_out:
            nslab = (n_out + 63) // 64
            stats = torch.empty((M, nslab, 2), dtype=torch.float32, device=x.device)
        with torch.cuda.device(x.device), _timed(("gemm_tn", M, N, K)):
            rc = _lib.lib.ape_gemm_tn_fused(
                x2.data_ptr(), x2.stride(0), weight.data_ptr(), weight.stride(0), out.data_ptr(), out.stride(0),
                bias.data_ptr() if bias is not None else None, res_ptr, ldr, res_dt, M, N, K, _lib.dtype_code(x.dtype),
                _lib.dtype_code(out_dtype), ACT[act], int(tile_n), part.data_ptr() if part is not None else None, int(nparts),
                colsum.data_ptr() if colsum is not None else None, float(inv_c), float(eps),
                stats.data_ptr() if stats is not None else None, int(nslab), _lib.current_stream_ptr())
        _lib.check(rc, "ape_gemm_tn_fused")
    else:
        with torch.cuda.device(x.device), _timed(("gemm_tn", M, N, K)):
            rc = _lib.lib.ape_gemm_tn_ex(x2.data_ptr(), x2.stride(0), weight.data_ptr(), weight.stride(0), out.data_ptr(),
                                         out.stride(0), bias.data_ptr() if bias is not None else None, res_ptr, ldr, res_dt,
                                         M, N, K, _lib.dtype_code(x.dtype), _lib.dtype_code(out_dtype), ACT[act], int(tile_n),
                                         _lib.current_stream_ptr())
        _lib.check(rc, "ape_gemm_tn")
    res = out.view(*x.shape[:-1], n_out) if ret_view else out
    return (res, stats) if stats_out else res


def quantize_rows_e4m3(w):
    w = w.detach().float()
    s = w.abs().amax(1) / 448.0
    s = torch.where(s > 0, s, torch.ones_like(s))
    return (w / s[:, None]).clamp(-448.0, 448.0).to(torch.float8_e4m3fn).contiguous(), s.contiguous()


def linear_fp8(xq, x_scale, wq, w_scale, bias=None, act=None, stats_out=False, out=None, out_dtype=torch.float16):
    _require(xq.is_cuda and wq.is_cuda, "linear_fp8: CUDA tensors only")
    _require(xq.dtype == torch.float8_e4m3fn and wq.dtype == torch.float8_e4m3fn, "linear_fp8: e4m3 operands")
    _require(xq.dim() == 2 and wq.dim() == 2 and xq.shape[1] == wq.shape[1] and xq.stride(1) == 1 and wq.stride(1) == 1,
             "linear_fp8: xq [M, K] and wq [N, K] with unit inner stride")
    M, K = xq.shape
    N = wq.shape[0]
    for s, n, name in ((x_scale, M, "x_scale"), (w_scale, N, "w_scale")):
        _require(s.dtype == torch.float32 and s.is_contiguous() and s.numel() == n and s.is_cuda, f"linear_fp8: {name} fp32 [{n}]")
    if bias is not None:
        _require(bias.dtype == torch.float32 and bias.is_contiguous() and bias.numel() == N, "linear_fp8: bias must be fp32 [N]")
    _require(act in (None, "swiglu"), "linear_fp8: act None or 'swiglu'")
    n_out = N // 2 if act == "swiglu" else N
    if out is None:
        out = torch.empty((M, n_out), dtype=out_dtype, device=xq.device)
    _require(out.dim() == 2 and out.shape == (M, n_out) and out.stride(1) == 1 and out.is_cuda, "linear_fp8: bad `out`")
    stats, nslab = None, 0
    if stats_out:
        nslab = (n_out + 63) // 64
        stats = torch.empty((M, nslab, 2), dtype=torch.float32, device=xq.device)
    with torch.cuda.device(xq.device), _timed(("gemm_tn_e4m3", M, N, K)):
        rc = _lib.lib.ape_gemm_tn_e4m3(xq.data_ptr(), xq.stride(0), wq.data_ptr(), wq.stride(0), x_scale.data_ptr(),
                                       w_scale.data_ptr(), out.data_ptr(), out.stride(0),
                                       bias.data_ptr() if bias is not None else None, M, N, K, _lib.dtype_code(out.dtype),
                                       ACT[act], stats.data_ptr() if stats is not None else None, int(nslab),
                                       _lib.current_stream_ptr())
    _lib.check(rc, "ape_gemm_tn_e4m3")
    return (out, stats) if stats_out else out


def ffn_fused(x, w1, b1, w2, b2, out=None, variant=0):
    _require(x.is_cuda and w1.is_cuda and w2.is_cuda, "ffn_fused: CUDA tensors only")
    _require(x.dtype in (torch.float16, torch.bfloat16) and w1.dtype == x.dtype and w2.dtype == x.dtype,
             "ffn_fused: fp16/bf16 operands of one dtype")
    E = x.shape[-1]
    F = w1.shape[0]
    _require(w1.dim() == 2 and w2.dim() == 2 and tuple(w1.shape) == (F, E) and tuple(w2.shape) == (E, F) and
             w1.stride(1) == 1 and w2.stride(1) == 1, "ffn_fused: w1 must be [F, E] and w2 [E, F] with unit inner stride")
    for b, n in ((b1, F), (b2, E)):
        _require(b is None or (b.dtype == torch.float32 and b.is_contiguous() and b.numel() == n), "ffn_fused: biases fp32 [F] / [E]")
    x2 = x.reshape(-1, E)
    if x2.stride(1) != 1 or x2.stride(0) % 8 or x2.data_ptr() % 16:
        x2 = x2.contiguous()
    M = x2.shape[0]
    if out is None:
        out = torch.empty((M, E), dtype=torch.float32, device=x.device)
        res = out.view(*x.shape[:-1], E)
    else:
        _require(out.dtype == torch.float32 and out.dim() == 2 and tuple(out.shape) == (M, E) and out.stride(1) == 1 and out.is_cuda,
                 "ffn_fused: out must be fp32 [M, E] with unit inner stride")
        res = out
    with torch.cuda.device(x.device), _timed(("ffn_fused", M, E, F)):
        rc = _lib.lib.ape_ffn_fused(x2.data_ptr(), x2.stride(0), w1.data_ptr(), w1.stride(0),
                                    b1.data_ptr() if b1 is not None else None, w2.data_ptr(), w2.stride(0),
                                    b2.data_ptr() if b2 is not None else None, out.data_ptr(), out.stride(0), M, E, F,
                                    _lib.dtype_code(x.dtype), int(variant), _lib.current_stream_ptr())
    _lib.check(rc, "ape_ffn_fused")
    return res


def conv3x3_supported(H, W, Cin, Cout, dtype):
    if dtype not in (torch.float16, torch.bfloat16) or Cin % 64 or Cout % 8:
        return False
    tw = 128
    while tw > 8 and W % tw:
        tw >>= 1
    return W % tw == 0 and H % (128 // tw) == 0


def conv3x3_nhwc(x, weight_ohwi, bias=None, act=None):
    _require(x.is_cuda and x.dim() == 4 and x.is_contiguous() and weight_ohwi.is_contiguous() and x.dtype == weight_ohwi.dtype,
             "conv3x3: contiguous CUDA NHWC input and OHWI weight of one dtype")
    B, H, W, Cin = x.shape
    Cout = weight_ohwi.shape[0]
    _require(tuple(weight_ohwi.shape) == (Cout, 3, 3, Cin), "conv3x3: weight must be [Cout,3,3,Cin]")
    y = torch.empty((B, H, W, Cout), dtype=x.dtype, device=x.device)
    with torch.cuda.device(x.device), _timed(("conv3x3", B * H * W, Cout, 9 * Cin)):
        rc = _lib.lib.ape_conv3x3_nhwc(x.data_ptr(), weight_ohwi.data_ptr(), y.data_ptr(),
                                       bias.data_ptr() if bias is not None else None, B, H, W, Cin, Cout,
                                       _lib.dtype_code(x.dtype), ACT[act], _lib.current_stream_ptr())
    _lib.check(rc, "ape_conv3x3_nhwc")
    return y


def linear_rope_tc(x, weight, bias, cos, sin, num_channels, head_dim, pos_map=None):
    _require(x.is_cuda and x.dim() == 2 and x.dtype == weight.dtype and x.dtype in (torch.float16, torch.bfloat16),
             "linear_rope_tc: 2-D fp16/bf16 CUDA operands")
    M, K = x.shape
    N = weight.shape[0]
    _require(weight.shape[1] == K and x.stride(1) == 1 and weight.stride(1) == 1 and x.stride(0) % 8 == 0 and
             weight.stride(0) % 8 == 0, "linear_rope_tc: bad operand layout")
    _require(cos.dtype == torch.float32 and cos.is_contiguous() and sin.is_contiguous() and cos.shape[1] == head_dim,
             "linear_rope_tc: cos/sin must be contiguous fp32 [npos, head_dim]")
    out = torch.empty((M, N), dtype=x.dtype, device=x.device)
    with torch.cuda.device(x.device), _timed(("gemm_tn", M, N, K)):
        rc = _lib.lib.ape_gemm_tn_rope(x.data_ptr(), x.stride(0), weight.data_ptr(), weight.stride(0), out.data_ptr(), N,
                                       bias.data_ptr() if bias is not None else None, M, N, K, _lib.dtype_code(x.dtype),
                                       _lib.dtype_code(x.dtype), cos.data_ptr(), sin.data_ptr(),
                                       pos_map.data_ptr() if pos_map is not None else None, cos.shape[0], int(head_dim),
                                       2 * int(num_channels), 0, _lib.current_stream_ptr())
    _lib.check(rc, "ape_gemm_tn_rope")
    return out


def cached(obj, slot, dtype, key, build):
    d = obj.__dict__.setdefault(slot, {})
    e = d.get(dtype)
    if e is None or e[0] != key:
        with torch.no_grad():
            e = (key, build())
        d[dtype] = e
    return e[1]


def packed(module, dtype, extra=None):
    w, b = module.weight, getattr(module, "bias", None)
    key = (w._version, w.data_ptr(), None if b is None else (b._version, b.data_ptr()))
    return cached(module, "_ape_packed", dtype, key, lambda: (
        w.detach().to(dtype if w.dim() >= 2 else torch.float32).contiguous(),
        None if b is None else b.detach().to(torch.float32).contiguous()))


def linear_module_tc(module, x, act=None, residual=None, out_dtype=None, out=None):
    w, b = packed(module, x.dtype)
    return linear_tc(x, w, b, act=act, residual=residual, out_dtype=out_dtype, out=out)


def layernorm_module(module, x, out_dtype=None):
    w, b = packed(module, torch.float32)
    return layernorm(x, w, b, eps=module.eps, out_dtype=out_dtype)


def layernorm(x, weight, bias, eps=1e-5, out_dtype=None, row_map=None, out=None, scale_out=None):
    C = x.shape[-1]
    x2 = x.reshape(-1, C) if x.dim() != 2 else x
    _require(x2.is_cuda and x2.stride(1) == 1, "layernorm: CUDA tensor with unit inner stride")
    _require(weight.dtype == torch.float32 and bias.dtype == torch.float32, "layernorm: fp32 weight / bias")
    rows = x2.shape[0]
    out_dtype = out.dtype if out is not None else (out_dtype or x.dtype)
    if out_dtype == torch.float8_e4m3fn:
        if out is None:
            out = torch.empty((rows, (C + 15) // 16 * 16), dtype=out_dtype, device=x.device)[:, :C]
        _require(out.dim() == 2 and out.stride(1) == 1 and out.is_cuda, "layernorm: bad e4m3 `out`")
        if scale_out is None:
            scale_out = torch.empty((out.shape[0],), dtype=torch.float32, device=x.device)
        _require(scale_out.dtype == torch.float32 and scale_out.is_contiguous() and scale_out.numel() == out.shape[0],
                 "layernorm: scale_out must be fp32 [output rows]")
        with torch.cuda.device(x.device), _timed(("layernorm_e4m3", rows, C)):
            rc = _lib.lib.ape_layernorm_e4m3(x2.data_ptr(), x2.stride(0), out.data_ptr(), out.stride(0), scale_out.data_ptr(),
                                             weight.data_ptr(), bias.data_ptr(),
                                             row_map.data_ptr() if row_map is not None else None, rows, C, float(eps),
                                             _lib.dtype_code(x2.dtype), _lib.current_stream_ptr())
        _lib.check(rc, "ape_layernorm_e4m3")
        return out, scale_out
    if out is None:
        out = torch.empty((rows, C), dtype=out_dtype, device=x.device)
    with torch.cuda.device(x.device), _timed(("layernorm", rows, C)):
        rc = _lib.lib.ape_layernorm(x2.data_ptr(), x2.stride(0), out.data_ptr(), out.stride(0), weight.data_ptr(),
                                    bias.data_ptr(), row_map.data_ptr() if row_map is not None else None, rows, C,
                                    float(eps), _lib.dtype_code(x2.dtype), _lib.dtype_code(out.dtype),
                                    _lib.current_stream_ptr())
    _lib.check(rc, "ape_layernorm")
    return out if x.dim() == 2 or out.shape[1] != C else out.view(*x.shape[:-1], C)


def layernorm_ex(x, weight, bias, eps, weight2=None, bias2=None, eps2=0.0, col_add=None, row_add=None, out_dtype=None):
    C = x.shape[-1]
    _require(x.is_cuda and x.is_contiguous(), "layernorm_ex: contiguous CUDA tensor")
    x2 = x.view(-1, C)
    rows = x2.shape[0]
    rpi = x.shape[-2] if x.dim() == 3 else rows
    out_dtype = out_dtype or x.dtype
    if weight is None:
        _require(bias is None and weight2 is None, "layernorm_ex: bias / weight2 without weight")
    add_only = weight is None and col_add is None and out_dtype == x.dtype
    _require(not add_only or row_add is not None, "layernorm_ex: nothing to compute")
    y = x if add_only else torch.empty(x.shape, dtype=out_dtype, device=x.device)
    y2 = None
    if row_add is not None:
        _require(row_add.dtype == out_dtype and row_add.is_contiguous() and row_add.numel() == x.numel(),
                 "layernorm_ex: row_add must match x in the output dtype")
        y2 = torch.empty(x.shape, dtype=out_dtype, device=x.device)
    if col_add is not None:
        col_add = col_add.reshape(-1, C)
        _require(col_add.dtype == torch.float32 and col_add.is_contiguous() and col_add.shape[0] * rpi == rows,
                 "layernorm_ex: col_add must be fp32 [images, C]")
    for t in (weight, bias, weight2, bias2):
        _require(t is None or (t.dtype == torch.float32 and t.is_contiguous()), "layernorm_ex: fp32 weights")
    with torch.cuda.device(x.device), _timed(("layernorm_ex", rows, C, weight2 is not None, row_add is not None)):
        rc = _lib.lib.ape_layernorm_ex(
            x2.data_ptr(), C, None if add_only else y.data_ptr(), C, weight.data_ptr() if weight is not None else None,
            bias.data_ptr() if bias is not None else None, float(eps),
            weight2.data_ptr() if weight2 is not None else None, bias2.data_ptr() if bias2 is not None else None, float(eps2),
            col_add.data_ptr() if col_add is not None else None, C, int(rpi),
            row_add.data_ptr() if row_add is not None else None, C, y2.data_ptr() if y2 is not None else None, C,
            rows, C, _lib.dtype_code(x.dtype), _lib.dtype_code(out_dtype), _lib.current_stream_ptr())
    _lib.check(rc, "ape_layernorm_ex")
    return y, y2


def groupnorm_nhwc(x, weight, bias, groups, eps=1e-5, out_dtype=None, out=None):
    _require(x.is_cuda and x.dim() == 3 and x.is_contiguous(), "groupnorm_nhwc: contiguous CUDA [B, rows, C]")
    B, rows, C = x.shape
    if out is None:
        out = torch.empty((B, rows, C), dtype=out_dtype or x.dtype, device=x.device)
    _require(out.shape == x.shape and out.stride(2) == 1 and out.stride(1) == C, "groupnorm_nhwc: bad `out` view")
    ws = torch.empty((int(_lib.lib.ape_groupnorm_workspace_bytes(B, rows, C)),), dtype=torch.uint8, device=x.device)
    with torch.cuda.device(x.device), _timed(("groupnorm", B, rows, C)):
        rc = _lib.lib.ape_groupnorm_nhwc(x.data_ptr(), C, out.data_ptr(), C, out.stride(0) if B > 1 else 0, weight.data_ptr(),
                                         bias.data_ptr(), ws.data_ptr(), B, rows, C, int(groups), float(eps),
                                         _lib.dtype_code(x.dtype), _lib.dtype_code(out.dtype), _lib.current_stream_ptr())
    _lib.check(rc, "ape_groupnorm_nhwc")
    return out


def rope_qk_(qkv, cos, sin, num_channels, head_dim, pos_map=None):
    _require(qkv.is_cuda and qkv.dim() == 2 and qkv.stride(1) == 1, "rope: qkv must be a 2-D CUDA tensor")
    _require(cos.dtype == torch.float32 and cos.is_contiguous() and sin.is_contiguous() and cos.shape[1] == head_dim,
             "rope: cos/sin must be contiguous fp32 [npos, head_dim]")
    with torch.cuda.device(qkv.device), _timed(("rope_qk", qkv.shape[0], num_channels)):
        rc = _lib.lib.ape_rope_qk(qkv.data_ptr(), qkv.stride(0), cos.data_ptr(), sin.data_ptr(),
                                  pos_map.data_ptr() if pos_map is not None else None, qkv.shape[0], num_channels,
                                  head_dim, cos.shape[0], _lib.dtype_code(qkv.dtype), _lib.current_stream_ptr())
    _lib.check(rc, "ape_rope_qk")
    return qkv


def attention_supported(n, head_dim, dtype):
    return head_dim == 64 and n % 128 == 0 and dtype in (torch.float16, torch.bfloat16)


def attention_qkv(qkv, num_seq, n, heads, head_dim, scale, n_valid=None, stats_out=False, seq_stride=None, causal=False,
                  out_row_map=None, out=None, seg_start=None):
    _require(qkv.is_cuda and qkv.dim() == 2 and qkv.stride(1) == 1, "attention: qkv must be a 2-D CUDA tensor")
    stride = n if seq_stride is None else int(seq_stride)
    _require(qkv.shape[0] >= (num_seq - 1) * stride + (n_valid or n) and qkv.shape[1] == 3 * heads * head_dim, "attention: qkv shape")
    C = heads * head_dim
    if seg_start is not None:
        _require(seg_start.is_cuda and seg_start.dtype == torch.int32 and seg_start.dim() == 1 and seg_start.is_contiguous() and
                 seg_start.numel() == num_seq * n, "attention: seg_start must be a contiguous int32 CUDA vector with one entry per query row")
        _require(out_row_map is None and not stats_out, "attention: seg_start goes with neither out_row_map nor stats_out")
    if out_row_map is not None:
        _require(out_row_map.is_cuda and out_row_map.dtype == torch.int32 and out_row_map.dim() == 1 and
                 out_row_map.is_contiguous() and out_row_map.numel() >= (num_seq - 1) * stride + min(stride, n),
                 "attention: out_row_map must be a contiguous int32 CUDA vector with one entry per query row")
        _require(out is not None and out.is_cuda and out.dim() == 2 and out.dtype == qkv.dtype and out.shape[1] == C and
                 out.stride(1) == 1, "attention: out_row_map needs `out` [rows, heads*head_dim] in qkv's dtype")
    else:
        _require(out is None, "attention: `out` is only taken with out_row_map")
        alloc = torch.zeros if (stride < n or (n_valid is not None and n_valid < n)) else torch.empty
        out = alloc((qkv.shape[0], C), dtype=qkv.dtype, device=qkv.device)
    stats = torch.empty((out.shape[0], heads, 2), dtype=torch.float32, device=qkv.device) if stats_out else None
    args = (qkv.data_ptr(), qkv.stride(0), out.data_ptr(), out.stride(0), int(num_seq), int(n), int(n if n_valid is None else n_valid),
            int(heads), int(head_dim), float(scale), _lib.dtype_code(qkv.dtype), stats.data_ptr() if stats is not None else None,
            stride, 1 if causal else 0, int(qkv.shape[0]))
    with torch.cuda.device(qkv.device), _timed(("attention", num_seq, n, heads)):
        if seg_start is not None:
            rc = _lib.lib.ape_attn_fwd_seg(*args, seg_start.data_ptr(), _lib.current_stream_ptr())
        elif out_row_map is None:
            rc = _lib.lib.ape_attn_fwd_ex(*args, _lib.current_stream_ptr())
        else:
            rc = _lib.lib.ape_attn_fwd_mapped(*args, out_row_map.data_ptr(), _lib.current_stream_ptr())
    _lib.check(rc, "ape_attn_fwd")
    return (out, stats) if stats_out else out


def text_embed_packed(token_embedding, positional_embedding, tok, pos):
    for t in (token_embedding, positional_embedding):
        _require(t.is_cuda and t.dtype == torch.float32 and t.dim() == 2 and t.is_contiguous(), "text_embed_packed: contiguous fp32 CUDA tables")
    D = token_embedding.shape[1]
    _require(positional_embedding.shape[1] == D, "text_embed_packed: tables of one width")
    for t in (tok, pos):
        _require(t.is_cuda and t.dtype == torch.int32 and t.dim() == 1 and t.is_contiguous() and t.numel() == tok.numel(),
                 "text_embed_packed: tok / pos must be contiguous int32 CUDA vectors of one length")
    x = torch.empty((tok.numel(), D), dtype=torch.float32, device=tok.device)
    with torch.cuda.device(tok.device), _timed(("text_embed_packed", tok.numel(), D)):
        rc = _lib.lib.ape_text_embed_packed(token_embedding.data_ptr(), positional_embedding.data_ptr(), tok.data_ptr(), pos.data_ptr(),
                                            x.data_ptr(), tok.numel(), D, token_embedding.shape[0], positional_embedding.shape[0],
                                            _lib.current_stream_ptr())
    _lib.check(rc, "ape_text_embed_packed")
    return x


def rows_gather(x, rows):
    _require(x.is_cuda and x.dtype == torch.float32 and x.dim() == 2 and x.stride(1) == 1, "rows_gather: fp32 2-D CUDA tensor")
    _require(rows.is_cuda and rows.dtype == torch.int64 and rows.dim() == 1 and rows.is_contiguous(), "rows_gather: contiguous int64 CUDA rows")
    out = torch.empty((rows.numel(), x.shape[1]), dtype=torch.float32, device=x.device)
    with torch.cuda.device(x.device), _timed(("rows_gather", rows.numel(), x.shape[1])):
        rc = _lib.lib.ape_rows_gather(x.data_ptr(), x.stride(0), rows.data_ptr(), out.data_ptr(), out.stride(0), rows.numel(),
                                      x.shape[1], _lib.current_stream_ptr())
    _lib.check(rc, "ape_rows_gather")
    return out


def attention_cross(q, k, v, num_seq, nq, nkv, n_valid, heads, head_dim, scale):
    for t in (q, k, v):
        _require(t.is_cuda and t.dim() == 2 and t.stride(1) == 1 and t.dtype == q.dtype, "attention_cross: 2-D CUDA tensors of one dtype")
    C = heads * head_dim
    _require(q.shape == (num_seq * nq, C) and k.shape == (num_seq * nkv, C) and v.shape == (num_seq * nkv, C), "attention_cross: shapes")
    out = torch.empty((num_seq * nq, C), dtype=q.dtype, device=q.device)
    with torch.cuda.device(q.device), _timed(("attention_cross", num_seq, nq, n_valid, heads, head_dim)):
        rc = _lib.lib.ape_attn_cross_fwd(q.data_ptr(), q.stride(0), k.data_ptr(), k.stride(0), v.data_ptr(), v.stride(0),
                                         out.data_ptr(), out.stride(0), int(num_seq), int(nq), int(nkv), int(n_valid), int(heads),
                                         int(head_dim), float(scale), _lib.dtype_code(q.dtype), _lib.current_stream_ptr())
    _lib.check(rc, "ape_attn_cross_fwd")
    return out


def vlf_pool(v, qa, qc, stable_softmax_2d=True):
    _require(v.is_cuda and v.dim() == 3 and v.is_contiguous(), "vlf_pool: contiguous CUDA [B,S,C]")
    B, S, C = v.shape
    NH = qa.shape[1]
    qa = qa.float().contiguous()
    qc = qc.float().contiguous()
    nbytes = int(_lib.lib.ape_vlf_pool_workspace_bytes(B, S, C, NH))
    ws = torch.empty((nbytes // 4,), dtype=torch.float32, device=v.device)
    ptr, strips = ctypes.c_void_p(), ctypes.c_int()
    with torch.cuda.device(v.device), _timed(("vlf_pool", B, S, C, NH)):
        rc = _lib.lib.ape_vlf_pool(v.data_ptr(), qa.data_ptr(), qc.data_ptr(), ws.data_ptr(), ctypes.byref(ptr),
                                   ctypes.byref(strips), B, S, C, NH, 1 if stable_softmax_2d else 0,
                                   _lib.dtype_code(v.dtype), _lib.current_stream_ptr())
    _lib.check(rc, "ape_vlf_pool")
    off = (ptr.value - ws.data_ptr()) // 4
    part = ws[off: off + B * strips.value * NH * (C + 1)].view(B, strips.value, NH, C + 1).sum(1)
    return part[..., :C] / part[..., C:]


def nms_sorted_mask(sorted_boxes, iou_threshold, n_valid=None):
    _require(sorted_boxes.is_cuda and sorted_boxes.dim() == 2 and sorted_boxes.shape[1] == 4 and
             sorted_boxes.dtype == torch.float32 and sorted_boxes.is_contiguous(), "nms: boxes must be contiguous CUDA fp32 [n,4]")
    n = sorted_boxes.shape[0]
    keep = torch.empty((n,), dtype=torch.uint8, device=sorted_boxes.device)
    count = torch.zeros((1,), dtype=torch.int32, device=sorted_boxes.device)
    if n == 0:
        return keep, count
    ws = torch.empty((int(_lib.lib.ape_nms_workspace_bytes(n)),), dtype=torch.uint8, device=sorted_boxes.device)
    with torch.cuda.device(sorted_boxes.device), _timed(("nms", n)):
        if n_valid is None:
            rc = _lib.lib.ape_nms_sorted(sorted_boxes.data_ptr(), n, float(iou_threshold), ws.data_ptr(), keep.data_ptr(),
                                         count.data_ptr(), _lib.current_stream_ptr())
        else:
            _require(n_valid.is_cuda and n_valid.dtype == torch.int32 and n_valid.numel() == 1, "nms: n_valid must be int32 [1]")
            rc = _lib.lib.ape_nms_sorted_dev(sorted_boxes.data_ptr(), n, n_valid.data_ptr(), float(iou_threshold), ws.data_ptr(),
                                             keep.data_ptr(), count.data_ptr(), _lib.current_stream_ptr())
    _lib.check(rc, "ape_nms_sorted")
    return keep, count


def nms_classwise(boxes, scores, score_thresh, iou_threshold, row_valid=None):
    _require(boxes.is_cuda and boxes.dtype == torch.float32 and boxes.is_contiguous() and boxes.dim() == 2 and boxes.shape[1] == 4,
             "nms_classwise: boxes must be contiguous CUDA fp32 [Q,4]")
    _require(scores.is_cuda and scores.dtype == torch.float32 and scores.dim() == 2 and scores.stride(1) == 1 and
             scores.shape[0] == boxes.shape[0], "nms_classwise: scores must be CUDA fp32 [Q,N]")
    Q, N = scores.shape
    _require(Q <= 1024, f"nms_classwise: at most 1024 queries (got {Q})")
    out = torch.empty((N, Q), dtype=torch.float32, device=scores.device)
    ws = torch.empty((max(1, int(_lib.lib.ape_nms_classwise_workspace_bytes(Q))),), dtype=torch.uint8, device=scores.device)
    if row_valid is not None:
        _require(row_valid.dtype == torch.uint8 and row_valid.is_contiguous() and row_valid.numel() == Q, "nms_classwise: row_valid uint8 [Q]")
    with torch.cuda.device(scores.device), _timed(("nms_classwise", Q, N)):
        rc = _lib.lib.ape_nms_classwise(boxes.data_ptr(), scores.data_ptr(), scores.stride(0),
                                        row_valid.data_ptr() if row_valid is not None else None, Q, N, float(score_thresh),
                                        float(iou_threshold), ws.data_ptr(), out.data_ptr(), _lib.current_stream_ptr())
    _lib.check(rc, "ape_nms_classwise")
    return out


def nms(boxes, scores, iou_threshold):
    _require(boxes.is_cuda and boxes.dim() == 2 and boxes.shape[1] == 4, "nms: boxes must be CUDA [n,4]")
    n = boxes.shape[0]
    if n == 0:
        return torch.empty((0,), dtype=torch.int64, device=boxes.device)
    order = scores.sort(0, descending=True)[1]
    keep, _ = nms_sorted_mask(boxes.float().index_select(0, order).contiguous(), iou_threshold)
    return order[keep.bool()]


def batched_nms(boxes, scores, idxs, iou_threshold):
    if boxes.numel() == 0:
        return torch.empty((0,), dtype=torch.int64, device=boxes.device)
    if boxes.shape[0] > 32768:
        raise RuntimeError(f"ape_b200.ops.batched_nms: {boxes.shape[0]} candidates need a dense IoU bit matrix of "
                           f"{boxes.shape[0] ** 2 // 8 / 2 ** 30:.1f} GiB; use ops.nms_classwise (per-class NMS over shared boxes)")
    boxes = boxes.float()
    max_coordinate = boxes.max()
    offsets = idxs.to(boxes) * (max_coordinate + torch.tensor(1).to(boxes))
    return nms(boxes + offsets[:, None], scores, iou_threshold)


def ref_update(delta, ref, valid_ratios, eps=1e-3):
    _require(delta.is_cuda and delta.dtype == torch.float32 and ref.dtype == torch.float32 and delta.shape == ref.shape and
             delta.shape[-1] == 4 and delta.dim() == 3, "ref_update: CUDA fp32 [B,Q,4] tensors")
    B, Q, _ = delta.shape
    L = valid_ratios.shape[1]
    delta, ref = delta.contiguous(), ref.contiguous()
    vr = valid_ratios.float().contiguous()
    new_ref = torch.empty_like(delta)
    ref_in = torch.empty((B, Q, L, 4), dtype=torch.float32, device=delta.device)
    with torch.cuda.device(delta.device), _timed(("ref_update", B, Q, L)):
        rc = _lib.lib.ape_ref_update(delta.data_ptr(), ref.data_ptr(), vr.data_ptr(), new_ref.data_ptr(), ref_in.data_ptr(), B, Q, L,
                                     float(eps), _lib.current_stream_ptr())
    _lib.check(rc, "ape_ref_update")
    return new_ref, ref_in


def gemv_f32(x, weight, bias=None):
    _require(x.is_cuda and weight.is_cuda and x.dtype == torch.float32 and weight.dtype == torch.float32, "gemv_f32: CUDA fp32 tensors")
    K = x.shape[-1]
    N = weight.shape[0]
    x2 = x.reshape(-1, K).contiguous()
    weight = weight.contiguous()
    _require(weight.shape[1] == K and K % 4 == 0, "gemv_f32: weight [N,K], K a multiple of 4")
    y = torch.empty((x2.shape[0], N), dtype=torch.float32, device=x.device)
    bptr = None
    if bias is not None:
        bias = bias.float().contiguous()
        bptr = bias.data_ptr()
    with torch.cuda.device(x.device), _timed(("gemv", x2.shape[0], N, K)):
        for b0 in range(0, x2.shape[0], 4):
            nb = min(4, x2.shape[0] - b0)
            rc = _lib.lib.ape_gemv_f32(weight.data_ptr(), x2[b0:].data_ptr(), bptr, y[b0:].data_ptr(), nb, N, K, _lib.current_stream_ptr())
            _lib.check(rc, "ape_gemv_f32")
    return y.view(*x.shape[:-1], N)


def mask_crop_and_resize(mask_logits, index, boxes, padded_hw, mask_size=128):
    _require(mask_logits.is_cuda and mask_logits.dim() == 3 and mask_logits.is_contiguous(), "mask_crop: contiguous CUDA logits [Q,h,w]")
    K = int(index.numel())
    out = torch.empty((K, mask_size, mask_size), dtype=torch.uint8, device=mask_logits.device)
    if K == 0:
        return out.bool()
    index = index.to(device=mask_logits.device, dtype=torch.int64).contiguous()
    boxes = boxes.to(device=mask_logits.device, dtype=torch.float32).contiguous()
    _require(tuple(boxes.shape) == (K, 4), "mask_crop: boxes must be [K,4]")
    Hp, Wp = int(padded_hw[0]), int(padded_hw[1])
    ws = torch.empty((int(_lib.lib.ape_mask_crop_workspace_bytes(K, Hp, Wp)),), dtype=torch.uint8, device=mask_logits.device)
    with torch.cuda.device(mask_logits.device), _timed(("mask_crop", K, Hp, Wp)):
        rc = _lib.lib.ape_mask_crop(mask_logits.data_ptr(), index.data_ptr(), boxes.data_ptr(), ws.data_ptr(), out.data_ptr(), K,
                                    mask_logits.shape[1], mask_logits.shape[2], Hp, Wp, int(mask_size),
                                    _lib.dtype_code(mask_logits.dtype), _lib.current_stream_ptr())
    _lib.check(rc, "ape_mask_crop")
    return out.view(torch.bool)


def paste_masks_in_image(masks, boxes, image_shape, threshold=0.5):
    N, S = masks.shape[0], masks.shape[-1]
    img_h, img_w = int(image_shape[0]), int(image_shape[1])
    out = torch.empty((N, img_h, img_w), dtype=torch.uint8, device=masks.device)
    if N == 0:
        return out.view(torch.bool)
    _require(masks.is_cuda and masks.dim() == 3 and masks.shape[1] == S, "mask_paste: CUDA masks [N,S,S]")
    m8 = masks.view(torch.uint8) if masks.dtype == torch.bool else (masks >= 0.5).to(torch.uint8)
    m8 = m8.contiguous()
    boxes = boxes.to(device=masks.device, dtype=torch.float32).contiguous()
    with torch.cuda.device(masks.device), _timed(("mask_paste", N, img_h, img_w)):
        rc = _lib.lib.ape_mask_paste(m8.data_ptr(), boxes.data_ptr(), out.data_ptr(), N, S, img_h, img_w, float(threshold),
                                     _lib.current_stream_ptr())
    _lib.check(rc, "ape_mask_paste")
    return out.view(torch.bool)


def rle_counts_to_string(counts):
    import numpy as np

    c = np.ascontiguousarray(counts, dtype=np.uint32)
    out = np.empty((7 * max(len(c), 1),), dtype=np.uint8)
    n = int(_lib.lib.ape_rle_to_string(c.ctypes.data, len(c), out.ctypes.data))
    _lib.check(0 if n >= 0 else n, "ape_rle_to_string")
    return out[:n].tobytes()


def paste_masks_rle(masks, boxes, image_shape, threshold=0.5):
    import numpy as np

    N, S = masks.shape[0], masks.shape[-1]
    H, W = int(image_shape[0]), int(image_shape[1])
    if N == 0:
        return []
    _require(masks.is_cuda and masks.dim() == 3 and masks.shape[1] == S, "paste_masks_rle: CUDA masks [N,S,S]")
    m8 = (masks.view(torch.uint8) if masks.dtype == torch.bool else (masks >= 0.5).to(torch.uint8)).contiguous()
    boxes = boxes.to(device=masks.device, dtype=torch.float32).contiguous()
    stream = _lib.current_stream_ptr()
    col_count = torch.empty((N, W), dtype=torch.int32, device=masks.device)
    with torch.cuda.device(masks.device), _timed(("mask_rle", N, H, W)):
        rc = _lib.lib.ape_mask_paste_rle(m8.data_ptr(), boxes.data_ptr(), N, S, H, W, float(threshold), col_count.data_ptr(), None,
                                         None, stream)
        _lib.check(rc, "ape_mask_paste_rle")
        csum = col_count.view(-1).to(torch.int64).cumsum(0)
        col_offset = (csum - col_count.view(-1)).contiguous()
        per_mask = csum.view(N, W)[:, -1].cpu()
        total = int(per_mask[-1])
        positions = torch.empty((max(total, 1),), dtype=torch.int32, device=masks.device)
        rc = _lib.lib.ape_mask_paste_rle(m8.data_ptr(), boxes.data_ptr(), N, S, H, W, float(threshold), None, col_offset.data_ptr(),
                                         positions.data_ptr(), stream)
        _lib.check(rc, "ape_mask_paste_rle")
    pos = positions[:total].cpu().numpy().astype(np.int64)
    ends = per_mask.numpy()
    out, lo = [], 0
    for n in range(N):
        p = pos[lo:int(ends[n])]
        lo = int(ends[n])
        counts = np.diff(np.concatenate(([0], p, [H * W])))
        out.append({"size": [H, W], "counts": rle_counts_to_string(counts)})
    return out


SEMSEG_BAND_BYTES = 256 << 20


def semseg_label(mask_logits, query_index, cls, padded_hw, img_hw, out_hw, class0_const=None, band_bytes=None):
    _require(mask_logits.is_cuda and mask_logits.dim() == 3 and mask_logits.is_contiguous(), "semseg_label: contiguous CUDA logits [Q,h,w]")
    _require(cls.dim() == 2 and cls.dtype in (torch.float16, torch.bfloat16), "semseg_label: cls must be fp16 / bf16 [K, N]")
    dev = mask_logits.device
    K, N = int(cls.shape[0]), int(cls.shape[1])
    _require(int(query_index.numel()) == K and N >= 1, "semseg_label: query_index [K] and cls [K, N >= 1] disagree")
    Hp, Wp = int(padded_hw[0]), int(padded_hw[1])
    ih, iw = int(img_hw[0]), int(img_hw[1])
    oh, ow = int(out_hw[0]), int(out_hw[1])
    _require(0 < ih <= Hp and 0 < iw <= Wp and oh > 0 and ow > 0, "semseg_label: bad image / output size")
    P = oh * ow
    keys = torch.empty((P,), dtype=torch.int64, device=dev)
    label = torch.empty((oh, ow), dtype=torch.int64, device=dev)
    score = torch.empty((oh, ow), dtype=torch.float32, device=dev)
    col_base = 0 if class0_const is None else 1
    init = (float("-inf"), 0) if class0_const is None else (float(class0_const), 0)
    if K == 0 and N > col_base and (class0_const is None or float(class0_const) < 0.0):
        init = (0.0, col_base)
    stream = _lib.current_stream_ptr()
    with torch.cuda.device(dev), _timed(("semseg_label", K, N, P)):
        _lib.check(_lib.lib.ape_semseg_keys_init(keys.data_ptr(), P, init[0], init[1], stream), "ape_semseg_keys_init")
        if K > 0:
            Kp = (K + 7) // 8 * 8
            dt = cls.dtype
            w = torch.zeros((N - col_base, Kp), dtype=dt, device=dev)
            w[:, :K] = cls[:, col_base:].t()
            index = query_index.to(device=dev, dtype=torch.int64).contiguous()
            budget = SEMSEG_BAND_BYTES if band_bytes is None else int(band_bytes)
            rows = max(1, min(oh, budget // (ow * Kp * 2)))
            ws = torch.empty((rows * ow, Kp), dtype=dt, device=dev)
            for r0 in range(0, oh, rows):
                nr = min(rows, oh - r0)
                rc = _lib.lib.ape_semseg_resample(mask_logits.data_ptr(), index.data_ptr(), ws.data_ptr(), Kp, K,
                                                  mask_logits.shape[1], mask_logits.shape[2], Hp, Wp, ih, iw, oh, ow, r0, nr,
                                                  _lib.dtype_code(mask_logits.dtype), _lib.dtype_code(dt), stream)
                _lib.check(rc, "ape_semseg_resample")
                if N > col_base:
                    rc = _lib.lib.ape_gemm_tn_argmax(ws.data_ptr(), Kp, w.data_ptr(), Kp, keys[r0 * ow:].data_ptr(), nr * ow,
                                                     N - col_base, Kp, col_base, _lib.dtype_code(dt), stream)
                    _lib.check(rc, "ape_gemm_tn_argmax")
        _lib.check(_lib.lib.ape_semseg_keys_decode(keys.data_ptr(), P, label.data_ptr(), score.data_ptr(), stream),
                   "ape_semseg_keys_decode")
    return label, score


def panoptic_winners(mask_logits, query_index, scores, padded_hw, img_hw, out_hw, prob):
    _require(mask_logits.is_cuda and mask_logits.dim() == 3 and mask_logits.is_contiguous(),
             "panoptic_winners: contiguous CUDA logits [Q,h,w]")
    dev = mask_logits.device
    K = int(query_index.numel())
    _require(query_index.dim() == 1 and scores.dim() == 1 and int(scores.numel()) == K,
             "panoptic_winners: query_index [K] and scores [K] disagree")
    Hp, Wp = int(padded_hw[0]), int(padded_hw[1])
    ih, iw = int(img_hw[0]), int(img_hw[1])
    oh, ow = int(out_hw[0]), int(out_hw[1])
    _require(0 < ih <= Hp and 0 < iw <= Wp and oh > 0 and ow > 0, "panoptic_winners: bad image / output size")
    index = query_index.to(device=dev, dtype=torch.int64).contiguous()
    sc = scores.to(device=dev, dtype=torch.float32).contiguous()
    ids = torch.empty((oh, ow), dtype=torch.int32, device=dev)
    counts = torch.empty((3, K), dtype=torch.int32, device=dev)
    with torch.cuda.device(dev), _timed(("panoptic_winners", K, oh * ow)):
        rc = _lib.lib.ape_panoptic_winners(mask_logits.data_ptr(), index.data_ptr(), sc.data_ptr(), ids.data_ptr(), counts.data_ptr(),
                                           K, mask_logits.shape[1], mask_logits.shape[2], Hp, Wp, ih, iw, oh, ow, float(prob),
                                           _lib.dtype_code(mask_logits.dtype), _lib.current_stream_ptr())
        _lib.check(rc, "ape_panoptic_winners")
    return ids, counts


_RESAMPLE_TABLES = {}


def resample_tables(in_size, out_size, device):
    key = (int(in_size), int(out_size), str(device))
    hit = _RESAMPLE_TABLES.get(key)
    if hit is None:
        ksize = int(_lib.lib.ape_resample_ksize(int(in_size), int(out_size)))
        _lib.check(0 if ksize > 0 else ksize, "ape_resample_ksize")
        bounds = torch.empty((out_size, 2), dtype=torch.int32)
        kk = torch.empty((out_size, ksize), dtype=torch.int32)
        _lib.check(_lib.lib.ape_resample_coeffs_u8(int(in_size), int(out_size), bounds.data_ptr(), kk.data_ptr()), "ape_resample_coeffs_u8")
        if len(_RESAMPLE_TABLES) > 64:
            _RESAMPLE_TABLES.clear()
        hit = _RESAMPLE_TABLES[key] = (bounds.to(device), kk.to(device), ksize)
    return hit


def resize_u8_bilinear(img, new_h, new_w, flip_channels=False, out=None):
    _require(img.is_cuda and img.dtype == torch.uint8 and img.dim() in (2, 3), "resize_u8_bilinear: CUDA uint8 [H,W,C] or [H,W] image")
    if img.dim() == 2:
        img = img.unsqueeze(-1)
    H, W, C = img.shape
    _require(1 <= C <= 4 and img.stride(2) == 1 and img.stride(1) == C, "resize_u8_bilinear: pixels must be contiguous (1-4 channels)")
    new_h, new_w = int(new_h), int(new_w)
    if out is None:
        out = torch.empty((C, new_h, new_w), dtype=torch.float32, device=img.device)
    _require(out.is_cuda and out.dtype == torch.float32 and out.dim() == 3 and out.shape[0] == C and out.shape[1] >= new_h and
             out.shape[2] >= new_w and out.stride(2) == 1, "resize_u8_bilinear: out must be float32 [C,>=new_h,>=new_w] with unit column stride")
    bh, kh, ksh = resample_tables(W, new_w, img.device)
    bv, kv, ksv = resample_tables(H, new_h, img.device)
    tmp = torch.empty((H, new_w, C), dtype=torch.uint8, device=img.device)
    with torch.cuda.device(img.device), _timed(("resample", H, W, new_h, new_w)):
        rc = _lib.lib.ape_resample_u8(img.data_ptr(), img.stride(0), tmp.data_ptr(), out.data_ptr(), out.stride(0), out.stride(1),
                                      bh.data_ptr(), kh.data_ptr(), ksh, bv.data_ptr(), kv.data_ptr(), ksv, H, W, C, new_h, new_w,
                                      1 if flip_channels else 0, _lib.current_stream_ptr())
    _lib.check(rc, "ape_resample_u8")
    return out[:, :new_h, :new_w]


def ms_deform_attn_backward(value, spatial_shapes, level_start_index, sampling_loc, attn_weight, grad_output, im2col_step=64):
    if not value.is_cuda:
        raise RuntimeError("Not implemented on the CPU")
    B, S, H, D, L, Q, P = _check_inputs(value, spatial_shapes, level_start_index, sampling_loc, attn_weight)
    _require(grad_output.is_cuda and grad_output.is_contiguous(), "grad_output tensor has to be contiguous")
    _require(grad_output.dtype == value.dtype and grad_output.numel() == B * Q * H * D, "grad_output must be [B,Q,H*D] of value's dtype")
    gv = torch.zeros((B, S, H, D), dtype=torch.float32, device=value.device)
    gl = torch.empty_like(sampling_loc)
    ga = torch.empty_like(attn_weight)
    with torch.cuda.device(value.device), _timed(("msda_bwd", B, S, Q, L, P, value.element_size())):
        rc = _lib.lib.ape_msda_bwd(value.data_ptr(), spatial_shapes.data_ptr(), level_start_index.data_ptr(), sampling_loc.data_ptr(),
                                   attn_weight.data_ptr(), grad_output.data_ptr(), gv.data_ptr(), gl.data_ptr(), ga.data_ptr(),
                                   B, S, H, D, L, Q, P, _lib.dtype_code(value.dtype), _lib.current_stream_ptr())
    _lib.check(rc, "ape_msda_bwd")
    return [gv if value.dtype == torch.float32 else gv.to(value.dtype), gl, ga]


def _ms_deform_attn_backward(value, spatial_shapes, level_start_index, sampling_loc, attn_weight,
                             grad_output, im2col_step):
    return ms_deform_attn_backward(value, spatial_shapes, level_start_index, sampling_loc, attn_weight, grad_output, im2col_step)


def _register():
    try:
        lib = torch.library.Library(_NS, "DEF")
    except Exception:
        lib = torch.library.Library(_NS, "FRAGMENT")
    defined = []
    for schema in (_FWD_SCHEMA, _BWD_SCHEMA):
        try:
            lib.define(schema)
            defined.append(schema.split("(")[0])
        except RuntimeError:
            pass

    def _fwd(value, spatial_shapes, level_start_index, sampling_loc, attn_weight, im2col_step):
        return ms_deform_attn_forward(value, spatial_shapes, level_start_index, sampling_loc, attn_weight, im2col_step)

    def _fwd_cpu(value, spatial_shapes, level_start_index, sampling_loc, attn_weight, im2col_step):
        raise RuntimeError("Not implemented on the CPU")

    if "ms_deform_attn_forward" in defined:
        lib.impl("ms_deform_attn_forward", _fwd, "CUDA")
        lib.impl("ms_deform_attn_forward", _fwd_cpu, "CPU")
    if "ms_deform_attn_backward" in defined:
        lib.impl("ms_deform_attn_backward", _ms_deform_attn_backward, "CUDA")
        lib.impl("ms_deform_attn_backward", lambda *a: _fwd_cpu(*a[:6]), "CPU")
    return lib


_LIBRARY = _register()
```

include/ape_b200.h:

```cpp
#ifndef APE_B200_H_
#define APE_B200_H_

#include <stdint.h>

#ifdef __cplusplus
extern "C" {
#endif

#define APE_ABI_VERSION 3

#define APE_DTYPE_F32 0
#define APE_DTYPE_F16 1
#define APE_DTYPE_BF16 2
#define APE_DTYPE_E4M3 3

#define APE_OK 0
#define APE_ERR_INVALID_ARG (-1)
#define APE_ERR_UNSUPPORTED (-2)
#define APE_ERR_NULL_PTR (-3)

int ape_abi_version(void);

const char *ape_last_error(void);

uint64_t ape_launch_count(void);

int ape_msda_fwd(const void *value, const int64_t *spatial_shapes, const int64_t *level_start,
                 const void *loc, const void *attn, void *out, int B, int S, int H, int D, int L,
                 int Q, int P, int dtype, void *stream);

int ape_msda_fwd_variant(const void *value, const int64_t *spatial_shapes, const int64_t *level_start,
                         const void *loc, const void *attn, void *out, int B, int S, int H, int D,
                         int L, int Q, int P, int dtype, int variant, void *stream);

int ape_msda_fused_fwd(const void *value, const int64_t *spatial_shapes, const int64_t *level_start,
                       const void *offsets, int64_t offs_row_stride, const void *logits,
                       int64_t logit_row_stride, const float *ref, int ref_dim, void *out, int B,
                       int S, int H, int D, int L, int Q, int P, int dtype, int offs_dtype,
                       void *stream);

int ape_msda_pair_values(const void *value, int64_t ld, void *value2, const uint8_t *token_mask, int B, int S, int H, int D,
                         int dtype, void *stream);
int ape_msda_pair_supported(const int *host_shapes, int L, int H, int D, int P, int dtype);
int ape_msda_pair_fused_fwd(const void *value2, const int64_t *spatial_shapes, const int64_t *level_start,
                            const int *host_shapes, const void *offsets, int64_t offs_row_stride, const void *logits,
                            int64_t logit_row_stride, const float *ref, int ref_dim, void *out, int B, int S, int H, int D,
                            int L, int Q, int P, int dtype, int offs_dtype, int heads_per_cta, int tile_w, int head_major,
                            void *stream);

int ape_msda_bwd(const void *value, const int64_t *spatial_shapes, const int64_t *level_start, const void *loc,
                 const void *attn, const void *grad_out, float *grad_value_f32, void *grad_loc, void *grad_attn, int B,
                 int S, int H, int D, int L, int Q, int P, int dtype, void *stream);

int ape_gemm_tn(const void *A, int64_t lda, const void *W, int64_t ldw, void *C, int64_t ldc, const float *bias,
                const void *residual, int64_t ldr, int M, int N, int K, int in_dtype, int out_dtype, int act,
                int tile_n, void *stream);

int ape_gemm_tn_ex(const void *A, int64_t lda, const void *W, int64_t ldw, void *C, int64_t ldc, const float *bias,
                   const void *residual, int64_t ldr, int res_dtype, int M, int N, int K, int in_dtype, int out_dtype,
                   int act, int tile_n, void *stream);

int ape_gemm_tn_fused(const void *A, int64_t lda, const void *W, int64_t ldw, void *C, int64_t ldc, const float *bias,
                      const void *residual, int64_t ldr, int res_dtype, int M, int N, int K, int in_dtype, int out_dtype,
                      int act, int tile_n, const float *ln_part, int ln_nparts, const float *ln_colsum, float ln_inv_c,
                      float ln_eps, float *stats_out, int stats_nslab, void *stream);

int ape_gemm_tn_e4m3(const void *A, int64_t lda, const void *W, int64_t ldw, const float *a_scale, const float *w_scale, void *C,
                     int64_t ldc, const float *bias, int M, int N, int K, int out_dtype, int act, float *stats_out,
                     int stats_nslab, void *stream);

int ape_conv3x3_nhwc(const void *x, const void *w, void *y, const float *bias, int B, int H, int W, int Cin, int Cout,
                     int dtype, int act, void *stream);

int ape_gemm_tn_rope(const void *A, int64_t lda, const void *W, int64_t ldw, void *C, int64_t ldc, const float *bias,
                     int M, int N, int K, int in_dtype, int out_dtype, const float *cos_table, const float *sin_table,
                     const int *pos_map, int npos, int head_dim, int rope_cols, int tile_n, void *stream);

int ape_ffn_fused(const void *x, int64_t ldx, const void *w1, int64_t ldw1, const float *b1, const void *w2, int64_t ldw2,
                  const float *b2, float *out, int64_t ldo, int M, int E, int F, int dtype, int variant, void *stream);

void ape_gemm_set_trace(long long *device_buffer);

int ape_layernorm(const void *x, int64_t ldx, void *y, int64_t ldy, const float *weight, const float *bias,
                  const int *row_map, int rows, int C, float eps, int in_dtype, int out_dtype, void *stream);

int ape_layernorm_e4m3(const void *x, int64_t ldx, void *y, int64_t ldy, float *scale, const float *weight, const float *bias,
                       const int *row_map, int rows, int C, float eps, int in_dtype, void *stream);

int ape_layernorm_ex(const void *x, int64_t ldx, void *y, int64_t ldy, const float *weight, const float *bias, float eps,
                     const float *weight2, const float *bias2, float eps2, const float *col_add, int64_t col_add_stride,
                     int rows_per_image, const void *row_add, int64_t ld_add, void *y2, int64_t ldy2, int rows, int C,
                     int in_dtype, int out_dtype, void *stream);

int64_t ape_groupnorm_workspace_bytes(int B, int rows_per_image, int C);
int ape_groupnorm_nhwc(const void *x, int64_t ldx, void *y, int64_t ldy, int64_t y_batch_stride, const float *weight,
                       const float *bias, void *workspace, int B, int rows_per_image, int C, int groups, float eps,
                       int in_dtype, int out_dtype, void *stream);

int ape_rope_qk(void *qkv, int64_t ld, const float *cos_table, const float *sin_table, const int *pos_map, int M,
                int C, int head_dim, int npos, int dtype, void *stream);

int ape_text_embed_packed(const float *token_embedding, const float *positional_embedding, const int *tok, const int *pos,
                          float *x, int rows, int D, int vocab, int ctx, void *stream);
int ape_rows_gather(const float *x, int64_t ldx, const int64_t *rows, float *out, int64_t ldo, int n, int D, void *stream);

int ape_attn_fwd(const void *qkv, int64_t ld, void *out, int64_t ldo, int num_seq, int n, int heads, int head_dim,
                 float scale, int dtype, void *stream);
int ape_attn_fwd_ex(const void *qkv, int64_t ld, void *out, int64_t ldo, int num_seq, int n, int n_valid, int heads,
                    int head_dim, float scale, int dtype, float *stats_out, int seq_stride, int causal, int64_t total_rows,
                    void *stream);
int ape_attn_fwd_mapped(const void *qkv, int64_t ld, void *out, int64_t ldo, int num_seq, int n, int n_valid, int heads,
                        int head_dim, float scale, int dtype, float *stats_out, int seq_stride, int causal, int64_t total_rows,
                        const int *out_row_map, void *stream);
int ape_attn_fwd_seg(const void *qkv, int64_t ld, void *out, int64_t ldo, int num_seq, int n, int n_valid, int heads,
                     int head_dim, float scale, int dtype, float *stats_out, int seq_stride, int causal, int64_t total_rows,
                     const int *seg_start, void *stream);

int ape_attn_variant(int set);

int ape_attn_cross_fwd(const void *q, int64_t ldq, const void *k, int64_t ldk, const void *v, int64_t ldv, void *out, int64_t ldo,
                       int num_seq, int nq, int nkv, int n_valid, int heads, int head_dim, float scale, int dtype, void *stream);

int64_t ape_vlf_pool_workspace_bytes(int B, int S, int C, int NH);
int ape_vlf_pool(const void *v, const float *qa, const float *qc, void *workspace, float **partial_out, int *strips_out,
                 int B, int S, int C, int NH, int stable_softmax_2d, int dtype, void *stream);

int64_t ape_nms_workspace_bytes(int n);
int ape_nms_sorted(const float *boxes_sorted, int n, float iou_threshold, void *workspace, uint8_t *keep, int *count,
                   void *stream);
int ape_nms_sorted_dev(const float *boxes_sorted, int n_max, const int *n_dev, float iou_threshold, void *workspace,
                       uint8_t *keep, int *count, void *stream);

int64_t ape_nms_classwise_workspace_bytes(int Q);
int ape_nms_classwise(const float *boxes, const float *scores, int64_t ld_scores, const uint8_t *row_valid, int Q, int N,
                      float score_thresh, float iou_threshold, void *workspace, float *out, void *stream);

int ape_resample_ksize(int in_size, int out_size);
int ape_resample_coeffs_u8(int in_size, int out_size, int *bounds_host, int *kk_host);
int ape_resample_u8(const uint8_t *src, int64_t src_pitch, uint8_t *tmp, float *out, int64_t plane_stride, int64_t row_stride,
                    const int *bounds_h, const int *kk_h, int ksize_h, const int *bounds_v, const int *kk_v, int ksize_v, int H,
                    int W, int C, int new_h, int new_w, int flip_channels, void *stream);

int ape_ref_update(const float *delta, const float *ref, const float *valid_ratios, float *new_ref, float *ref_in, int B, int Q,
                   int L, float eps, void *stream);

int ape_gemv_f32(const float *W, const float *x, const float *bias, float *y, int B, int N, int K, void *stream);

int64_t ape_mask_crop_workspace_bytes(int K, int Hp, int Wp);
int ape_mask_crop(const void *logits, const int64_t *index, const float *boxes, void *workspace, uint8_t *out, int K, int h, int w,
                  int Hp, int Wp, int S, int dtype, void *stream);
int ape_mask_paste(const uint8_t *masks, const float *boxes, uint8_t *out, int N, int S, int img_h, int img_w, float threshold,
                   void *stream);
int ape_mask_paste_rle(const uint8_t *masks, const float *boxes, int N, int S, int img_h, int img_w, float threshold,
                       int *col_count, const int64_t *col_offset, int *positions, void *stream);
int ape_rle_to_string(const uint32_t *counts, int m, char *out);

int ape_semseg_resample(const void *logits, const int64_t *index, void *A, int64_t lda, int K, int h, int w, int Hp, int Wp,
                        int img_h, int img_w, int out_h, int out_w, int row0, int rows, int logit_dtype, int a_dtype, void *stream);
int ape_semseg_keys_init(uint64_t *keys, int64_t n, float value, int column, void *stream);
int ape_gemm_tn_argmax(const void *A, int64_t lda, const void *W, int64_t ldw, uint64_t *keys, int M, int N, int K, int col_base,
                       int in_dtype, void *stream);
int ape_semseg_keys_decode(const uint64_t *keys, int64_t n, int64_t *label, float *score, void *stream);

#define APE_PANOPTIC_MAX_K 4096
int ape_panoptic_winners(const void *logits, const int64_t *index, const float *scores, int *ids, int *counts, int K, int h, int w,
                         int Hp, int Wp, int img_h, int img_w, int out_h, int out_w, float prob, int logit_dtype, void *stream);

#ifdef __cplusplus
}
#endif
#endif
```

Before: 43.05.

## Fuse input and output layernorms into the FFN kernel and pipeline its GEMMs

Adds an FFN kernel variant that applies the pre-norm layernorm to fp32 input rows on the fly, staging them into shared memory in place of the TMA load. It also applies the following layernorm(s), with column and row adds, to the FFN output by staging fp32 results in the freed weight buffers. The main loop is restructured so the next chunk's first GEMM is issued alongside the current chunk's second GEMM, with double-buffered activation fragments. The encoder layers are rewired to pass the next layer's norm and adds as a tail, removing separate layernorm launches and their fp32 round trips. The cost is more register pressure and extra shared-memory traffic in the epilogue.

Result: no change. 42.89 (median of 6 runs) (-0.4%).

```diff
diff --git a/ape_b200/_lib.py b/ape_b200/_lib.py
--- a/ape_b200/_lib.py
+++ b/ape_b200/_lib.py
@@ -70,6 +70,10 @@
     lib.ape_gemm_set_trace.argtypes = [_vp]
     lib.ape_ffn_fused.restype = _i
     lib.ape_ffn_fused.argtypes = [_vp, _i64, _vp, _i64, _vp, _vp, _i64, _vp, _vp, _i64] + [_i] * 5 + [_vp]
+    lib.ape_ffn_fused_ln.restype = _i
+    lib.ape_ffn_fused_ln.argtypes = [_vp, _i64, _vp, _vp, ctypes.c_float, _vp, _i64, _vp, _vp, _i64, _vp, _vp, _i64,
+                                     _vp, _vp, ctypes.c_float, _vp, _vp, ctypes.c_float, _vp, _i64, _i, _vp, _i64,
+                                     _vp, _i64, _vp, _i64] + [_i] * 4 + [_vp]
     lib.ape_gemm_tn_rope.restype = _i
     lib.ape_gemm_tn_rope.argtypes = [_vp, _i64, _vp, _i64, _vp, _i64, _vp, _i, _i, _i, _i, _i, _vp, _vp, _vp, _i, _i, _i, _i, _vp]
 
@@ -172,6 +176,7 @@
     "ape_conv3x3_nhwc",
     "ape_gemm_tn_rope",
     "ape_ffn_fused",
+    "ape_ffn_fused_ln",
     "ape_gemm_set_trace",
     "ape_layernorm",
     "ape_layernorm_e4m3",
diff --git a/ape_b200/csrc/ffn_fused.cu b/ape_b200/csrc/ffn_fused.cu
--- a/ape_b200/csrc/ffn_fused.cu
+++ b/ape_b200/csrc/ffn_fused.cu
@@ -1,5 +1,6 @@
 #include "attn.cuh"
 #include "common.cuh"
+#include "ln_row.cuh"
 #include "tc.cuh"
 
 namespace ape {
@@ -15,15 +16,28 @@
   uint64_t x_full, w1_full[2], w1_empty[2], w2_full[2], w2_empty[2];
 };
 
+static_assert(offsetof(FfnSmem, w2) == offsetof(FfnSmem, w1) + sizeof(FfnSmem::w1) &&
+              sizeof(FfnSmem::w1) + sizeof(FfnSmem::w2) == BM * E * sizeof(float), "LN_OUT staging area");
+
 struct FfnParams {
   const float *b1, *b2;
   const void *x;
   float *out;
   long long ldx, ldo;
   int M, F;
+  const float *nw, *nb;
+  float neps;
+  const float *ow, *ob, *ow2, *ob2;
+  float oeps, oeps2;
+  const float *col_add;
+  long long col_add_stride;
+  int rows_per_image;
+  const void *row_add;
+  void *y, *y2;
+  long long ld_add, ldy, ldy2;
 };
 
-template <typename T, int CL>
+template <typename T, int CL, bool LN_IN, bool LN_OUT>
 __global__ void __launch_bounds__(kThreads, 1)
 ffn_fused_kernel(const __grid_constant__ CUtensorMap map_x, const __grid_constant__ CUtensorMap map_w1,
                  const __grid_constant__ CUtensorMap map_w2, const FfnParams p) {
@@ -56,11 +70,13 @@
   if (warp >= 8) {
     tc::setmaxnreg_dec<40>();
     if (warp == 8 && lane == 0) {
-      tc::mbar_expect_tx(&s.x_full, E * BM * 2);
-#pragma unroll
-      for (int c = 0; c < E / 64; ++c)
-#pragma unroll
-        for (int h = 0; h < 2; ++h) tc::tma_load_2d(s.x[c] + h * 64 * 128, &map_x, &s.x_full, c * 64, row0 + h * 64);
+      if (!LN_IN) {
+        tc::mbar_expect_tx(&s.x_full, E * BM * 2);
+#pragma unroll
+        for (int c = 0; c < E / 64; ++c)
+#pragma unroll
+          for (int h = 0; h < 2; ++h) tc::tma_load_2d(s.x[c] + h * 64 * 128, &map_x, &s.x_full, c * 64, row0 + h * 64);
+      }
       for (int j = 0; j < nch; ++j) {
         const int b = j & 1, n = j >> 1;
         tc::mbar_wait(&s.w1_empty[b], (n & 1) ^ 1);
@@ -104,11 +120,59 @@
         for (int k = 0; k < 4; ++k) tc::Wgmma<64, T>::template ss<0>(sc, dx + 2 * k, dw + 2 * k, (c | k) != 0);
       }
     };
+    if constexpr (LN_IN) {
+      const float *xf = reinterpret_cast<const float *>(p.x);
+#pragma unroll 1
+      for (int i0 = 0; i0 < 16; i0 += 16) {
+        float v[16][1][8], sum[16];
+#pragma unroll
+        for (int i = 0; i < 16; ++i) {
+          const int m = row0 + g * 64 + (warp & 3) * 16 + i0 + i;
+          if (m < p.M) load8<float>(xf + (size_t)m * p.ldx + 8 * lane, v[i][0]);
+          else
+#pragma unroll
+            for (int k = 0; k < 8; ++k) v[i][0][k] = 0.f;
+        }
+#pragma unroll
+        for (int i = 0; i < 16; ++i) {
+          sum[i] = 0.f;
+#pragma unroll
+          for (int k = 0; k < 8; ++k) sum[i] += v[i][0][k];
+        }
+#pragma unroll
+        for (int i = 0; i < 16; ++i) ln_ex_norm<1>(v[i], sum[i], lane, E / 8, E, p.nw, p.nb, p.neps, nullptr, nullptr, 0.f);
+#pragma unroll
+        for (int i = 0; i < 16; ++i) {
+          const int r = g * 64 + (warp & 3) * 16 + i0 + i;
+          const uint4 q = row0 + r < p.M ? Elem<T>::pack(v[i][0]) : make_uint4(0u, 0u, 0u, 0u);
+          *reinterpret_cast<uint4 *>(s.x[lane >> 3] + r * 128 + (((lane & 7) ^ (r & 7)) << 4)) = q;
+        }
+      }
+      tc::fence_proxy_async();
+      tc::named_bar_sync(1 + g, 128);
+    }
     float o[E / 2];
 #pragma unroll
     for (int i = 0; i < E / 2; ++i) o[i] = 0.f;
     float sc[32];
-    tc::mbar_wait(&s.x_full, 0);
+    uint32_t pa[2][4][4];
+    auto make_p = [&](uint32_t(&pd)[4][4], int j) {
+#pragma unroll
+      for (int jj = 0; jj < 8; ++jj) {
+        float2 bb = make_float2(0.f, 0.f);
+        if (p.b1 != nullptr) bb = __ldg(reinterpret_cast<const float2 *>(p.b1 + j * HC + 8 * jj + 2 * tq));
+#pragma unroll
+        for (int h = 0; h < 2; ++h) {
+          float v0 = sc[4 * jj + 2 * h], v1 = sc[4 * jj + 2 * h + 1];
+          if (p.b1 != nullptr) {
+            v0 += bb.x;
+            v1 += bb.y;
+          }
+          pd[jj >> 1][2 * (jj & 1) + h] = attn::pack2<T>(fmaxf(v0, 0.f), fmaxf(v1, 0.f));
+        }
+      }
+    };
+    if (!LN_IN) tc::mbar_wait(&s.x_full, 0);
     tc::mbar_wait(&s.w1_full[0], 0);
     tc::wgmma_fence();
     issue_s(sc, 0);
@@ -116,43 +180,41 @@
     tc::wgmma_wait<0>();
     tc::fence_regs<32>(sc);
     release(&s.w1_empty[0]);
-
+    make_p(pa[0], 0);
+
+#pragma unroll 1
     for (int j = 0; j < nch; ++j) {
       const int b = j & 1, n = j >> 1;
-      uint32_t pa[4][4];
-#pragma unroll
-      for (int jj = 0; jj < 8; ++jj) {
-        float2 bb = make_float2(0.f, 0.f);
-        if (p.b1 != nullptr) bb = __ldg(reinterpret_cast<const float2 *>(p.b1 + j * HC + 8 * jj + 2 * tq));
-#pragma unroll
-        for (int h = 0; h < 2; ++h) {
-          float v0 = sc[4 * jj + 2 * h], v1 = sc[4 * jj + 2 * h + 1];
-          if (p.b1 != nullptr) {
-            v0 += bb.x;
-            v1 += bb.y;
-          }
-          pa[jj >> 1][2 * (jj & 1) + h] = attn::pack2<T>(fmaxf(v0, 0.f), fmaxf(v1, 0.f));
-        }
-      }
-      tc::mbar_wait(&s.w2_full[b], n & 1);
-      tc::fence_regs<E / 2>(o);
-      tc::wgmma_fence();
       const uint64_t dw2 = tc::make_smem_desc_sw128(tc::smem_u32(s.w2[b]));
-#pragma unroll
-      for (int kk = 0; kk < 4; ++kk) tc::Wgmma<256, T>::template rs<0>(o, pa[kk], dw2 + 2 * kk, (j | kk) != 0);
-      tc::wgmma_commit();
       if (j + 1 < nch) {
-        const int b1 = b ^ 1;
-        tc::mbar_wait(&s.w1_full[b1], ((j + 1) >> 1) & 1);
-        issue_s(sc, b1);
+        tc::mbar_wait(&s.w1_full[b ^ 1], ((j + 1) >> 1) & 1);
+        tc::mbar_wait(&s.w2_full[b], n & 1);
+        tc::fence_regs<E / 2>(o);
+        tc::wgmma_fence();
+        issue_s(sc, b ^ 1);
+        tc::wgmma_commit();
+#pragma unroll
+        for (int kk = 0; kk < 4; ++kk) tc::Wgmma<256, T>::template rs<0>(o, pa[0][kk], dw2 + 2 * kk, (j | kk) != 0);
         tc::wgmma_commit();
         tc::wgmma_wait<1>();
+        tc::fence_regs<32>(sc);
+        release(&s.w1_empty[b ^ 1]);
+        make_p(pa[1], j + 1);
+        tc::wgmma_wait<0>();
         tc::fence_regs<E / 2>(o);
+        tc::fence_regs<16>(reinterpret_cast<float *>(&pa[0][0][0]));
         release(&s.w2_empty[b]);
-        tc::wgmma_wait<0>();
-        tc::fence_regs<32>(sc);
-        release(&s.w1_empty[b1]);
+#pragma unroll
+        for (int kk = 0; kk < 4; ++kk)
+#pragma unroll
+          for (int q = 0; q < 4; ++q) pa[0][kk][q] = pa[1][kk][q];
       } else {
+        tc::mbar_wait(&s.w2_full[b], n & 1);
+        tc::fence_regs<E / 2>(o);
+        tc::wgmma_fence();
+#pragma unroll
+        for (int kk = 0; kk < 4; ++kk) tc::Wgmma<256, T>::template rs<0>(o, pa[0][kk], dw2 + 2 * kk, (j | kk) != 0);
+        tc::wgmma_commit();
         tc::wgmma_wait<0>();
         tc::fence_regs<E / 2>(o);
         release(&s.w2_empty[b]);
@@ -160,9 +222,11 @@
     }
 
     const T *xg = reinterpret_cast<const T *>(p.x);
+    float *stage = reinterpret_cast<float *>(s.w1[0][0]);
+    if (LN_OUT) tc::named_bar_sync(3, 256);
 #pragma unroll
     for (int h = 0; h < 2; ++h) {
-      const int m = row0 + g * 64 + (warp & 3) * 16 + (lane >> 2) + 8 * h;
+      const int r = g * 64 + (warp & 3) * 16 + (lane >> 2) + 8 * h, m = row0 + r;
       if (m < p.M) {
         const T *xr = xg + (size_t)m * p.ldx + 2 * tq;
         float *dst = p.out + (size_t)m * p.ldo + 2 * tq;
@@ -174,10 +238,70 @@
             v0 += bb.x;
             v1 += bb.y;
           }
-          const float2 r = Elem<T>::load2(xr + 8 * jj);
-          v0 += r.x;
-          v1 += r.y;
-          *reinterpret_cast<float2 *>(dst + 8 * jj) = make_float2(v0, v1);
+          float2 rx;
+          if constexpr (LN_IN) {
+            const uint32_t u = *reinterpret_cast<const uint32_t *>(s.x[jj >> 3] + r * 128 + (((jj & 7) ^ (r & 7)) << 4) + 4 * tq);
+            float f[8];
+            Elem<T>::unpack(make_uint4(u, 0u, 0u, 0u), f);
+            rx = make_float2(f[0], f[1]);
+          } else {
+            rx = Elem<T>::load2(xr + 8 * jj);
+          }
+          v0 += rx.x;
+          v1 += rx.y;
+          if constexpr (LN_OUT)
+            *reinterpret_cast<float2 *>(stage + r * E + (((2 * jj + (tq >> 1)) ^ (r & 7)) << 2) + 2 * (tq & 1)) = make_float2(v0, v1);
+          else
+            *reinterpret_cast<float2 *>(dst + 8 * jj) = make_float2(v0, v1);
+        }
+      }
+    }
+    if constexpr (LN_OUT) {
+      tc::named_bar_sync(3, 256);
+      T *ra = reinterpret_cast<T *>(s.x[0]);
+      if (p.y2 != nullptr) {
+        uint4 q[16];
+#pragma unroll
+        for (int i = 0; i < 16; ++i)
+          if (row0 + warp * 16 + i < p.M)
+            q[i] = *reinterpret_cast<const uint4 *>(reinterpret_cast<const T *>(p.row_add) + (size_t)(row0 + warp * 16 + i) * p.ld_add + 8 * lane);
+#pragma unroll
+        for (int i = 0; i < 16; ++i)
+          if (row0 + warp * 16 + i < p.M) *reinterpret_cast<uint4 *>(ra + (warp * 16 + i) * E + 8 * lane) = q[i];
+        __syncwarp();
+      }
+#pragma unroll 1
+      for (int i0 = 0; i0 < 16; i0 += 8) {
+        float v[8][1][8], sum[8];
+#pragma unroll
+        for (int i = 0; i < 8; ++i) {
+          const int r = warp * 16 + i0 + i;
+          const float4 *sr = reinterpret_cast<const float4 *>(stage + r * E);
+          const float4 a = sr[(2 * lane) ^ (r & 7)], b = sr[(2 * lane + 1) ^ (r & 7)];
+          v[i][0][0] = a.x, v[i][0][1] = a.y, v[i][0][2] = a.z, v[i][0][3] = a.w;
+          v[i][0][4] = b.x, v[i][0][5] = b.y, v[i][0][6] = b.z, v[i][0][7] = b.w;
+          sum[i] = 0.f;
+#pragma unroll
+          for (int k = 0; k < 8; ++k) sum[i] += v[i][0][k];
+        }
+#pragma unroll
+        for (int i = 0; i < 8; ++i) ln_ex_norm<1>(v[i], sum[i], lane, E / 8, E, p.ow, p.ob, p.oeps, nullptr, nullptr, 0.f);
+        if (p.ow2 != nullptr) {
+#pragma unroll
+          for (int i = 0; i < 8; ++i) {
+            sum[i] = 0.f;
+#pragma unroll
+            for (int k = 0; k < 8; ++k) sum[i] += v[i][0][k];
+          }
+#pragma unroll
+          for (int i = 0; i < 8; ++i) ln_ex_norm<1>(v[i], sum[i], lane, E / 8, E, p.ow2, p.ob2, p.oeps2, nullptr, nullptr, 0.f);
+        }
+#pragma unroll
+        for (int i = 0; i < 8; ++i) {
+          const int r = warp * 16 + i0 + i;
+          if (row0 + r < p.M)
+            ln_ex_out<T, 1, true>(v[i], lane, E / 8, row0 + r, reinterpret_cast<T *>(p.y), p.ldy, p.col_add, p.col_add_stride,
+                                  p.rows_per_image, ra + r * E, reinterpret_cast<T *>(p.y2), p.ldy2);
         }
       }
     }
@@ -186,10 +310,10 @@
   if (CL > 1) tc::cluster_sync_all();
 }
 
-template <typename T, int CL>
+template <typename T, int CL, bool LN_IN = false, bool LN_OUT = false>
 int launch(const CUtensorMap &mx, const CUtensorMap &m1, const CUtensorMap &m2, const FfnParams &p, cudaStream_t st) {
   const size_t smem = sizeof(FfnSmem) + 1024;
-  auto k = ffn_fused_kernel<T, CL>;
+  auto k = ffn_fused_kernel<T, CL, LN_IN, LN_OUT>;
   static bool set = false;
   if (!set) {
     cudaError_t e = cudaFuncSetAttribute(k, cudaFuncAttributeMaxDynamicSharedMemorySize, (int)smem);
@@ -244,10 +368,66 @@
   if (int rc = attn::make_map(&mx, x, dtype, M, E, ldx)) return rc;
   if (int rc = attn::make_map(&m1, w1, dtype, F, E, ldw1)) return rc;
   if (int rc = attn::make_map(&m2, w2, dtype, E, F, ldw2)) return rc;
-  FfnParams p{b1, b2, x, out, ldx, ldo, M, F};
+  FfnParams p{};
+  p.b1 = b1, p.b2 = b2, p.x = x, p.out = out, p.ldx = ldx, p.ldo = ldo, p.M = M, p.F = F;
   const bool cluster = variant == 2;
   cudaStream_t st = reinterpret_cast<cudaStream_t>(stream);
   if (dtype == APE_DTYPE_BF16)
     return cluster ? launch<__nv_bfloat16, 2>(mx, m1, m2, p, st) : launch<__nv_bfloat16, 1>(mx, m1, m2, p, st);
   return cluster ? launch<__half, 2>(mx, m1, m2, p, st) : launch<__half, 1>(mx, m1, m2, p, st);
 }
+
+extern "C" int ape_ffn_fused_ln(const void *x, int64_t ldx, const float *norm_w, const float *norm_b, float norm_eps,
+                                const void *w1, int64_t ldw1, const float *b1, const void *w2, int64_t ldw2, const float *b2,
+                                float *out, int64_t ldo, const float *out_w, const float *out_b, float out_eps,
+                                const float *out_w2, const float *out_b2, float out_eps2, const float *col_add,
+                                int64_t col_add_stride, int rows_per_image, const void *row_add, int64_t ld_add, void *y,
+                                int64_t ldy, void *y2, int64_t ldy2, int M, int E_, int F, int dtype, void *stream) {
+  if (dtype != APE_DTYPE_F16 && dtype != APE_DTYPE_BF16)
+    return fail(APE_ERR_INVALID_ARG, "ffn_fused_ln: operands must be fp16 or bf16 (got dtype %d)", dtype);
+  if (E_ != E) return fail(APE_ERR_UNSUPPORTED, "ffn_fused_ln: embedding width %d (only %d)", E_, E);
+  if (F <= 0 || F % HC) return fail(APE_ERR_UNSUPPORTED, "ffn_fused_ln: hidden width %d is not a positive multiple of %d", F, HC);
+  if (M < 0) return fail(APE_ERR_INVALID_ARG, "ffn_fused_ln: bad row count %d", M);
+  if (M == 0) return APE_OK;
+  const bool ln_in = norm_w != nullptr, ln_out = out_w != nullptr;
+  if (!x || !w1 || !w2 || (ln_in && !norm_b) || (ln_out ? (!out_b || !y || (out_w2 && !out_b2) || (y2 && !row_add)) : !out) ||
+      (col_add && rows_per_image <= 0))
+    return fail(APE_ERR_NULL_PTR, "ffn_fused_ln: null pointer argument");
+  if (!ln_out && (out_w2 || col_add || y2))
+    return fail(APE_ERR_INVALID_ARG, "ffn_fused_ln: a second norm, col_add or y2 needs out_w");
+  const uintptr_t al16 = reinterpret_cast<uintptr_t>(x) | reinterpret_cast<uintptr_t>(w1) | reinterpret_cast<uintptr_t>(w2) |
+                         reinterpret_cast<uintptr_t>(norm_w) | reinterpret_cast<uintptr_t>(norm_b) |
+                         reinterpret_cast<uintptr_t>(out_w) | reinterpret_cast<uintptr_t>(out_b) |
+                         reinterpret_cast<uintptr_t>(out_w2) | reinterpret_cast<uintptr_t>(out_b2) |
+                         reinterpret_cast<uintptr_t>(col_add) | reinterpret_cast<uintptr_t>(row_add) |
+                         reinterpret_cast<uintptr_t>(y) | reinterpret_cast<uintptr_t>(y2);
+  if ((al16 & 15) || ldx % (ln_in ? 4 : 8) || ldw1 % 8 || ldw2 % 8 || (ln_out && (ldy % 8 || (y2 && (ldy2 % 8 || ld_add % 8)))) ||
+      (col_add && col_add_stride % 4))
+    return fail(APE_ERR_INVALID_ARG, "ffn_fused_ln: bases, row pitches and vectors must be 16-byte aligned");
+  if (ldx < E || ldw1 < E || ldw2 < F || (!ln_out && ldo < E) || (ln_out && (ldy < E || (y2 && (ldy2 < E || ld_add < E)))))
+    return fail(APE_ERR_INVALID_ARG, "ffn_fused_ln: row pitch smaller than the row");
+  if (!ln_out && ((reinterpret_cast<uintptr_t>(out) & 7) || ldo % 2))
+    return fail(APE_ERR_INVALID_ARG, "ffn_fused_ln: out and its row pitch must allow 8-byte pairs");
+  if ((reinterpret_cast<uintptr_t>(b1) | reinterpret_cast<uintptr_t>(b2)) & 7)
+    return fail(APE_ERR_INVALID_ARG, "ffn_fused_ln: b1 / b2 must allow 8-byte pairs");
+  CUtensorMap mx, m1, m2;
+  if (int rc = attn::make_map(&m1, w1, dtype, F, E, ldw1)) return rc;
+  if (int rc = attn::make_map(&m2, w2, dtype, E, F, ldw2)) return rc;
+  if (ln_in)
+    mx = m1;
+  else if (int rc = attn::make_map(&mx, x, dtype, M, E, ldx))
+    return rc;
+  FfnParams p{};
+  p.b1 = b1, p.b2 = b2, p.x = x, p.out = out, p.ldx = ldx, p.ldo = ldo, p.M = M, p.F = F;
+  p.nw = norm_w, p.nb = norm_b, p.neps = norm_eps;
+  p.ow = out_w, p.ob = out_b, p.oeps = out_eps, p.ow2 = out_w2, p.ob2 = out_b2, p.oeps2 = out_eps2;
+  p.col_add = col_add, p.col_add_stride = col_add_stride, p.rows_per_image = rows_per_image > 0 ? rows_per_image : 1;
+  p.row_add = row_add, p.ld_add = ld_add, p.y = y, p.ldy = ldy, p.y2 = y2, p.ldy2 = ldy2;
+  cudaStream_t st = reinterpret_cast<cudaStream_t>(stream);
+#define APE_FFN_LN(T)                                                                      \
+  return ln_in ? (ln_out ? launch<T, 1, true, true>(mx, m1, m2, p, st) : launch<T, 1, true, false>(mx, m1, m2, p, st)) \
+               : (ln_out ? launch<T, 1, false, true>(mx, m1, m2, p, st) : launch<T, 1>(mx, m1, m2, p, st))
+  if (dtype == APE_DTYPE_BF16) APE_FFN_LN(__nv_bfloat16);
+  APE_FFN_LN(__half);
+#undef APE_FFN_LN
+}
diff --git a/ape_b200/csrc/ln_row.cuh b/ape_b200/csrc/ln_row.cuh
--- /dev/null
+++ b/ape_b200/csrc/ln_row.cuh
@@ -0,0 +1,126 @@
+#pragma once
+#include "common.cuh"
+
+namespace ape {
+namespace {
+
+template <typename T>
+__device__ __forceinline__ void load8(const T *p, float *f) {
+  if constexpr (sizeof(T) == 4) {
+    const float4 a = *reinterpret_cast<const float4 *>(p), b = *reinterpret_cast<const float4 *>(p + 4);
+    f[0] = a.x; f[1] = a.y; f[2] = a.z; f[3] = a.w; f[4] = b.x; f[5] = b.y; f[6] = b.z; f[7] = b.w;
+  } else {
+    const uint4 v = *reinterpret_cast<const uint4 *>(p);
+    Elem<T>::unpack(v, f);
+  }
+}
+template <typename T>
+__device__ __forceinline__ void store8(T *p, const float *f) {
+  if constexpr (sizeof(T) == 4) {
+    *reinterpret_cast<float4 *>(p) = make_float4(f[0], f[1], f[2], f[3]);
+    *reinterpret_cast<float4 *>(p + 4) = make_float4(f[4], f[5], f[6], f[7]);
+  } else {
+    *reinterpret_cast<uint4 *>(p) = Elem<T>::pack(f);
+  }
+}
+
+__device__ __forceinline__ float warp_sum(float v) {
+#pragma unroll
+  for (int o = 16; o > 0; o >>= 1) v += __shfl_xor_sync(0xffffffffu, v, o);
+  return v;
+}
+
+template <int MAXV>
+__device__ __forceinline__ void ln_ex_norm(float (&v)[MAXV][8], float sum, int lane, int nvec, int C, const float *__restrict__ w,
+                                           const float *__restrict__ b, float eps, const float *__restrict__ w2,
+                                           const float *__restrict__ b2, float eps2) {
+  float mean = warp_sum(sum) / (float)C;
+  float sq = 0.f;
+#pragma unroll
+  for (int i = 0; i < MAXV; ++i)
+    if (lane + 32 * i < nvec) {
+#pragma unroll
+      for (int k = 0; k < 8; ++k) {
+        const float d = v[i][k] - mean;
+        sq += d * d;
+      }
+    }
+  float rstd = rsqrtf(warp_sum(sq) / (float)C + eps);
+  sum = 0.f;
+#pragma unroll
+  for (int i = 0; i < MAXV; ++i) {
+    const int j = lane + 32 * i;
+    if (j < nvec) {
+      float ww[8], bb[8];
+      load8<float>(w + 8 * j, ww);
+      load8<float>(b + 8 * j, bb);
+#pragma unroll
+      for (int k = 0; k < 8; ++k) {
+        v[i][k] = (v[i][k] - mean) * rstd * ww[k] + bb[k];
+        sum += v[i][k];
+      }
+    }
+  }
+  if (w2) {
+    mean = warp_sum(sum) / (float)C;
+    sq = 0.f;
+#pragma unroll
+    for (int i = 0; i < MAXV; ++i)
+      if (lane + 32 * i < nvec) {
+#pragma unroll
+        for (int k = 0; k < 8; ++k) {
+          const float d = v[i][k] - mean;
+          sq += d * d;
+        }
+      }
+    rstd = rsqrtf(warp_sum(sq) / (float)C + eps2);
+#pragma unroll
+    for (int i = 0; i < MAXV; ++i) {
+      const int j = lane + 32 * i;
+      if (j < nvec) {
+        float ww[8], bb[8];
+        load8<float>(w2 + 8 * j, ww);
+        load8<float>(b2 + 8 * j, bb);
+#pragma unroll
+        for (int k = 0; k < 8; ++k) v[i][k] = (v[i][k] - mean) * rstd * ww[k] + bb[k];
+      }
+    }
+  }
+}
+
+template <typename TO, int MAXV, bool NORM>
+__device__ __forceinline__ void ln_ex_out(float (&v)[MAXV][8], int lane, int nvec, int row, TO *__restrict__ y, long long ldy,
+                                          const float *__restrict__ col_add, long long col_add_stride, int rows_per_image,
+                                          const TO *__restrict__ ra, TO *__restrict__ y2, long long ldy2) {
+  const float *ca = col_add ? col_add + (size_t)(row / rows_per_image) * col_add_stride : nullptr;
+#pragma unroll
+  for (int i = 0; i < MAXV; ++i) {
+    const int j = lane + 32 * i;
+    if (j < nvec) {
+      if (ca) {
+        float cc[8];
+        load8<float>(ca + 8 * j, cc);
+#pragma unroll
+        for (int k = 0; k < 8; ++k) v[i][k] += cc[k];
+      }
+      if (NORM || y) store8<TO>(y + (size_t)row * ldy + 8 * j, v[i]);
+      if (y2) {
+        float a[8], o[8];
+        load8<TO>(ra + 8 * j, a);
+        float r[8];
+        if constexpr (sizeof(TO) == 4) {
+#pragma unroll
+          for (int k = 0; k < 8; ++k) r[k] = v[i][k];
+        } else {
+          Elem<TO>::unpack(Elem<TO>::pack(v[i]), r);
+        }
+#pragma unroll
+        for (int k = 0; k < 8; ++k) o[k] = r[k] + a[k];
+        store8<TO>(y2 + (size_t)row * ldy2 + 8 * j, o);
+      }
+    }
+  }
+}
+
+}
+}
diff --git a/ape_b200/csrc/norm_rope.cu b/ape_b200/csrc/norm_rope.cu
--- a/ape_b200/csrc/norm_rope.cu
+++ b/ape_b200/csrc/norm_rope.cu
@@ -1,6 +1,7 @@
 #include <cuda_fp8.h>
 
 #include "common.cuh"
+#include "ln_row.cuh"
 
 namespace ape {
 namespace {
@@ -9,32 +10,6 @@
 struct Vec8 {
   static constexpr int kBytes = 8 * sizeof(T);
 };
-
-template <typename T>
-__device__ __forceinline__ void load8(const T *p, float *f) {
-  if constexpr (sizeof(T) == 4) {
-    const float4 a = *reinterpret_cast<const float4 *>(p), b = *reinterpret_cast<const float4 *>(p + 4);
-    f[0] = a.x; f[1] = a.y; f[2] = a.z; f[3] = a.w; f[4] = b.x; f[5] = b.y; f[6] = b.z; f[7] = b.w;
-  } else {
-    const uint4 v = *reinterpret_cast<const uint4 *>(p);
-    Elem<T>::unpack(v, f);
-  }
-}
-template <typename T>
-__device__ __forceinline__ void store8(T *p, const float *f) {
-  if constexpr (sizeof(T) == 4) {
-    *reinterpret_cast<float4 *>(p) = make_float4(f[0], f[1], f[2], f[3]);
-    *reinterpret_cast<float4 *>(p + 4) = make_float4(f[4], f[5], f[6], f[7]);
-  } else {
-    *reinterpret_cast<uint4 *>(p) = Elem<T>::pack(f);
-  }
-}
-
-__device__ __forceinline__ float warp_sum(float v) {
-#pragma unroll
-  for (int o = 16; o > 0; o >>= 1) v += __shfl_xor_sync(0xffffffffu, v, o);
-  return v;
-}
 
 template <typename TI, typename TO, int MAXV>
 __global__ void __launch_bounds__(256)
@@ -196,88 +171,9 @@
       for (int k = 0; k < 8; ++k) sum += v[i][k];
     }
   }
-  if constexpr (NORM) {
-  float mean = warp_sum(sum) / (float)C;
-  float sq = 0.f;
-#pragma unroll
-  for (int i = 0; i < MAXV; ++i)
-    if (lane + 32 * i < nvec) {
-#pragma unroll
-      for (int k = 0; k < 8; ++k) {
-        const float d = v[i][k] - mean;
-        sq += d * d;
-      }
-    }
-  float rstd = rsqrtf(warp_sum(sq) / (float)C + eps);
-  sum = 0.f;
-#pragma unroll
-  for (int i = 0; i < MAXV; ++i) {
-    const int j = lane + 32 * i;
-    if (j < nvec) {
-      float ww[8], bb[8];
-      load8<float>(w + 8 * j, ww);
-      load8<float>(b + 8 * j, bb);
-#pragma unroll
-      for (int k = 0; k < 8; ++k) {
-        v[i][k] = (v[i][k] - mean) * rstd * ww[k] + bb[k];
-        sum += v[i][k];
-      }
-    }
-  }
-  if (w2) {
-    mean = warp_sum(sum) / (float)C;
-    sq = 0.f;
-#pragma unroll
-    for (int i = 0; i < MAXV; ++i)
-      if (lane + 32 * i < nvec) {
-#pragma unroll
-        for (int k = 0; k < 8; ++k) {
-          const float d = v[i][k] - mean;
-          sq += d * d;
-        }
-      }
-    rstd = rsqrtf(warp_sum(sq) / (float)C + eps2);
-#pragma unroll
-    for (int i = 0; i < MAXV; ++i) {
-      const int j = lane + 32 * i;
-      if (j < nvec) {
-        float ww[8], bb[8];
-        load8<float>(w2 + 8 * j, ww);
-        load8<float>(b2 + 8 * j, bb);
-#pragma unroll
-        for (int k = 0; k < 8; ++k) v[i][k] = (v[i][k] - mean) * rstd * ww[k] + bb[k];
-      }
-    }
-  }
-  }
-  const float *ca = col_add ? col_add + (size_t)(warp / rows_per_image) * col_add_stride : nullptr;
-#pragma unroll
-  for (int i = 0; i < MAXV; ++i) {
-    const int j = lane + 32 * i;
-    if (j < nvec) {
-      if (ca) {
-        float cc[8];
-        load8<float>(ca + 8 * j, cc);
-#pragma unroll
-        for (int k = 0; k < 8; ++k) v[i][k] += cc[k];
-      }
-      if (NORM || y) store8<TO>(y + (size_t)warp * ldy + 8 * j, v[i]);
-      if (y2) {
-        float a[8], o[8];
-        load8<TO>(row_add + (size_t)warp * ld_add + 8 * j, a);
-        float r[8];
-        if constexpr (sizeof(TO) == 4) {
-#pragma unroll
-          for (int k = 0; k < 8; ++k) r[k] = v[i][k];
-        } else {
-          Elem<TO>::unpack(Elem<TO>::pack(v[i]), r);
-        }
-#pragma unroll
-        for (int k = 0; k < 8; ++k) o[k] = r[k] + a[k];
-        store8<TO>(y2 + (size_t)warp * ldy2 + 8 * j, o);
-      }
-    }
-  }
+  if constexpr (NORM) ln_ex_norm<MAXV>(v, sum, lane, nvec, C, w, b, eps, w2, b2, eps2);
+  ln_ex_out<TO, MAXV, NORM>(v, lane, nvec, warp, y, ldy, col_add, col_add_stride, rows_per_image, row_add + (size_t)warp * ld_add,
+                            y2, ldy2);
 }
 
 __device__ __forceinline__ float block_sum_256(float v, float *s_part) {
diff --git a/ape_b200/layers/common.py b/ape_b200/layers/common.py
--- a/ape_b200/layers/common.py
+++ b/ape_b200/layers/common.py
@@ -75,6 +75,29 @@
             return ops.linear_module_tc(fc2, h, residual=x.contiguous(), out_dtype=out_dtype)
         return x + self.layers[1](F.relu(self.layers[0][0](x)))
 
+    def forward_ln(self, x, norm, dtype, tail_norms=(), col_add=None, row_add=None):
+        from .. import ops
+
+        fc1 = self.layers[0][0]
+        nw, nb = ops.packed(norm, torch.float32)
+        tail = None
+        if tail_norms:
+            tw, tb = ops.packed(tail_norms[0], torch.float32)
+            tail = dict(weight=tw, bias=tb, eps=tail_norms[0].eps, col_add=col_add, row_add=row_add)
+            if len(tail_norms) > 1:
+                tail["weight2"], tail["bias2"] = ops.packed(tail_norms[1], torch.float32)
+                tail["eps2"] = tail_norms[1].eps
+        if x.shape[-1] == 256 and fc1.out_features % 64 == 0:
+            w1, b1 = ops.packed(fc1, dtype)
+            w2, b2 = ops.packed(self.layers[1], dtype)
+            return ops.ffn_fused(x.contiguous(), w1, b1, w2, b2, norm=(nw, nb, norm.eps), tail=tail)
+        s = self(ops.layernorm(x, nw, nb, eps=norm.eps, out_dtype=dtype), out_dtype=torch.float32)
+        if tail is None:
+            return s
+        return ops.layernorm_ex(s.contiguous(), tail["weight"], tail["bias"], tail["eps"], weight2=tail.get("weight2"),
+                                bias2=tail.get("bias2"), eps2=tail.get("eps2", 0.0), col_add=col_add, row_add=row_add,
+                                out_dtype=dtype)
+
 
 def inverse_sigmoid(x, eps=1e-3):
     x = x.clamp(min=0, max=1)
diff --git a/ape_b200/modeling/transformer.py b/ape_b200/modeling/transformer.py
--- a/ape_b200/modeling/transformer.py
+++ b/ape_b200/modeling/transformer.py
@@ -83,18 +83,20 @@
         self.norms = nn.ModuleList([nn.LayerNorm(embed_dim), nn.LayerNorm(embed_dim)])
 
     def forward(self, query, query_pos, key_padding_mask, reference_points, spatial_shapes, level_start_index,
-                host_shapes=None, query_with_pos=None, defer_last_norm=False):
+                host_shapes=None, query_with_pos=None, defer_last_norm=False, tail=None):
         x = self.attentions[0](query, None, query, None, query_pos=query_pos, key_padding_mask=key_padding_mask,
                                reference_points=reference_points, spatial_shapes=spatial_shapes,
                                level_start_index=level_start_index, host_shapes=host_shapes,
                                query_with_pos=query_with_pos,
                                sum_dtype=torch.float32 if query.dtype != torch.float32 else None)
         if query.dtype in (torch.float16, torch.bfloat16):
-            x = ops.layernorm_module(self.norms[0], x, out_dtype=query.dtype)
-            x = self.ffns[0](x, out_dtype=torch.float32)
-            if defer_last_norm:
-                return x
-            return ops.layernorm_module(self.norms[1], x, out_dtype=query.dtype)
+            dt = query.dtype
+            if defer_last_norm and tail is None:
+                return self.ffns[0].forward_ln(x, self.norms[0], dt)
+            t = tail or {}
+            y, y2 = self.ffns[0].forward_ln(x, self.norms[0], dt, (self.norms[1],) + tuple(t.get("norms", ())),
+                                            t.get("col_add"), t.get("row_add"))
+            return (y, y2) if tail is not None else y
         x = self.norms[0](x)
         x = self.ffns[0](x)
         return self.norms[1](x)
@@ -176,33 +178,40 @@
         return query, query_l
 
     def _engine_single_token(self, x, query_pos, query_l, key_padding_mask, kwargs):
-        pending = None
         dt = x.dtype
         if self.record_taps:
             self.taps = {}
-        for i, (vl_layer, layer) in enumerate(zip(self.vl_layers, self.layers)):
-            b = vl_layer.b_attn
+
+        def language_side(b, query_l):
             with torch.autocast("cuda", enabled=False):
                 ln_l = ops.layernorm(query_l.float().contiguous(), b.layer_norm_l.weight.float(), b.layer_norm_l.bias.float(),
                                      eps=b.layer_norm_l.eps, out_dtype=torch.float32)
                 dv, qa, qc = b.single_token_language_side(ln_l)
                 shift = (b.gamma_v.float() * dv.float()).reshape(x.shape[0], -1).contiguous()
-            vw, vb = ops.packed(b.layer_norm_v, dt)
-            if pending is None:
-                query, qpos = ops.layernorm_ex(x, vw, vb, b.layer_norm_v.eps, col_add=shift, row_add=query_pos, out_dtype=dt)
-            else:
-                query, qpos = ops.layernorm_ex(x, pending[0], pending[1], pending[2], weight2=vw, bias2=vb,
-                                               eps2=b.layer_norm_v.eps, col_add=shift, row_add=query_pos, out_dtype=dt)
+            return ln_l, qa, qc, shift
+
+        b = self.vl_layers[0].b_attn
+        lang = language_side(b, query_l)
+        vw, vb = ops.packed(b.layer_norm_v, dt)
+        query, qpos = ops.layernorm_ex(x, vw, vb, b.layer_norm_v.eps, col_add=lang[3], row_add=query_pos, out_dtype=dt)
+        last = len(self.layers) - 1
+        for i, (vl_layer, layer) in enumerate(zip(self.vl_layers, self.layers)):
+            b = vl_layer.b_attn
+            ln_l, qa, qc, shift = lang
             if self.record_taps:
                 self.taps[f"vlf{i}.v"] = query
             with torch.autocast("cuda", enabled=False):
                 dl = b.single_token_pool(query, qa, qc, shift=shift)
                 query_l = ln_l + b.gamma_l.float() * dl
-            x = layer(query, query_pos, key_padding_mask, kwargs["reference_points"], kwargs["spatial_shapes"],
-                      kwargs["level_start_index"], kwargs.get("host_shapes"), query_with_pos=qpos, defer_last_norm=True)
-            nw, nb = ops.packed(layer.norms[1], dt)
-            pending = (nw, nb, layer.norms[1].eps)
-        x = ops.layernorm(x, pending[0], pending[1], eps=pending[2], out_dtype=dt)
+            args = (query, query_pos, key_padding_mask, kwargs["reference_points"], kwargs["spatial_shapes"],
+                    kwargs["level_start_index"], kwargs.get("host_shapes"))
+            if i < last:
+                nxt = self.vl_layers[i + 1].b_attn
+                lang = language_side(nxt, query_l)
+                query, qpos = layer(*args, query_with_pos=qpos,
+                                    tail=dict(norms=(nxt.layer_norm_v,), col_add=lang[3], row_add=query_pos))
+            else:
+                x = layer(*args, query_with_pos=qpos)
         if self.post_norm_layer is not None:
             x = self.post_norm_layer(x)
         return x, query_l
diff --git a/ape_b200/ops.py b/ape_b200/ops.py
--- a/ape_b200/ops.py
+++ b/ape_b200/ops.py
@@ -263,10 +263,11 @@
     return (out, stats) if stats_out else out
 
 
-def ffn_fused(x, w1, b1, w2, b2, out=None, variant=0):
+def ffn_fused(x, w1, b1, w2, b2, out=None, variant=0, norm=None, tail=None):
     _require(x.is_cuda and w1.is_cuda and w2.is_cuda, "ffn_fused: CUDA tensors only")
-    _require(x.dtype in (torch.float16, torch.bfloat16) and w1.dtype == x.dtype and w2.dtype == x.dtype,
-             "ffn_fused: fp16/bf16 operands of one dtype")
+    dt = w1.dtype
+    _require(dt in (torch.float16, torch.bfloat16) and w2.dtype == dt and x.dtype == (torch.float32 if norm else dt),
+             "ffn_fused: fp16/bf16 operands of one dtype (x fp32 with `norm`)")
     E = x.shape[-1]
     F = w1.shape[0]
     _require(w1.dim() == 2 and w2.dim() == 2 and tuple(w1.shape) == (F, E) and tuple(w2.shape) == (E, F) and
@@ -277,20 +278,56 @@
     if x2.stride(1) != 1 or x2.stride(0) % 8 or x2.data_ptr() % 16:
         x2 = x2.contiguous()
     M = x2.shape[0]
-    if out is None:
+    if norm is None and tail is None:
+        if out is None:
+            out = torch.empty((M, E), dtype=torch.float32, device=x.device)
+            res = out.view(*x.shape[:-1], E)
+        else:
+            _require(out.dtype == torch.float32 and out.dim() == 2 and tuple(out.shape) == (M, E) and out.stride(1) == 1 and
+                     out.is_cuda, "ffn_fused: out must be fp32 [M, E] with unit inner stride")
+            res = out
+        with torch.cuda.device(x.device), _timed(("ffn_fused", M, E, F)):
+            rc = _lib.lib.ape_ffn_fused(x2.data_ptr(), x2.stride(0), w1.data_ptr(), w1.stride(0),
+                                        b1.data_ptr() if b1 is not None else None, w2.data_ptr(), w2.stride(0),
+                                        b2.data_ptr() if b2 is not None else None, out.data_ptr(), out.stride(0), M, E, F,
+                                        _lib.dtype_code(x.dtype), int(variant), _lib.current_stream_ptr())
+        _lib.check(rc, "ape_ffn_fused")
+        return res
+    _require(out is None and variant == 0, "ffn_fused: `out` and `variant` are for the plain FFN")
+    ptr = lambda t: None if t is None else t.data_ptr()
+    nw = nb = None
+    neps = 0.0
+    if norm is not None:
+        nw, nb, neps = norm
+    t = dict(tail or {})
+    for v in (nw, nb, t.get("weight"), t.get("bias"), t.get("weight2"), t.get("bias2")):
+        _require(v is None or (v.dtype == torch.float32 and v.is_contiguous() and v.numel() == E), "ffn_fused: fp32 [E] norm weights")
+    lead = x.shape[:-1]
+    y = y2 = out = None
+    col_add, row_add, rpi = t.get("col_add"), t.get("row_add"), 0
+    if tail is None:
         out = torch.empty((M, E), dtype=torch.float32, device=x.device)
-        res = out.view(*x.shape[:-1], E)
     else:
-        _require(out.dtype == torch.float32 and out.dim() == 2 and tuple(out.shape) == (M, E) and out.stride(1) == 1 and out.is_cuda,
-                 "ffn_fused: out must be fp32 [M, E] with unit inner stride")
-        res = out
+        y = torch.empty((M, E), dtype=dt, device=x.device)
+        if row_add is not None:
+            _require(row_add.dtype == dt and row_add.is_contiguous() and row_add.numel() == M * E,
+                     "ffn_fused: row_add must match the output in w1's dtype")
+            y2 = torch.empty((M, E), dtype=dt, device=x.device)
+        if col_add is not None:
+            rpi = lead[-1] if len(lead) >= 2 else M
+            col_add = col_add.reshape(-1, E)
+            _require(col_add.dtype == torch.float32 and col_add.is_contiguous() and col_add.shape[0] * rpi == M,
+                     "ffn_fused: col_add must be fp32 [images, E]")
     with torch.cuda.device(x.device), _timed(("ffn_fused", M, E, F)):
-        rc = _lib.lib.ape_ffn_fused(x2.data_ptr(), x2.stride(0), w1.data_ptr(), w1.stride(0),
-                                    b1.data_ptr() if b1 is not None else None, w2.data_ptr(), w2.stride(0),
-                                    b2.data_ptr() if b2 is not None else None, out.data_ptr(), out.stride(0), M, E, F,
-                                    _lib.dtype_code(x.dtype), int(variant), _lib.current_stream_ptr())
-    _lib.check(rc, "ape_ffn_fused")
-    return res
+        rc = _lib.lib.ape_ffn_fused_ln(
+            x2.data_ptr(), x2.stride(0), ptr(nw), ptr(nb), float(neps), w1.data_ptr(), w1.stride(0), ptr(b1), w2.data_ptr(),
+            w2.stride(0), ptr(b2), ptr(out), E, ptr(t.get("weight")), ptr(t.get("bias")), float(t.get("eps", 0.0)),
+            ptr(t.get("weight2")), ptr(t.get("bias2")), float(t.get("eps2", 0.0)), ptr(col_add), E, int(rpi), ptr(row_add), E,
+            ptr(y), E, ptr(y2), E, M, E, F, _lib.dtype_code(dt), _lib.current_stream_ptr())
+    _lib.check(rc, "ape_ffn_fused_ln")
+    if tail is None:
+        return out.view(*lead, E)
+    return y.view(*lead, E), None if y2 is None else y2.view(*lead, E)
 
 
 def conv3x3_supported(H, W, Cin, Cout, dtype):
diff --git a/include/ape_b200.h b/include/ape_b200.h
--- a/include/ape_b200.h
+++ b/include/ape_b200.h
@@ -78,6 +78,12 @@
 
 int ape_ffn_fused(const void *x, int64_t ldx, const void *w1, int64_t ldw1, const float *b1, const void *w2, int64_t ldw2,
                   const float *b2, float *out, int64_t ldo, int M, int E, int F, int dtype, int variant, void *stream);
+
+int ape_ffn_fused_ln(const void *x, int64_t ldx, const float *norm_w, const float *norm_b, float norm_eps, const void *w1,
+                     int64_t ldw1, const float *b1, const void *w2, int64_t ldw2, const float *b2, float *out, int64_t ldo,
+                     const float *out_w, const float *out_b, float out_eps, const float *out_w2, const float *out_b2,
+                     float out_eps2, const float *col_add, int64_t col_add_stride, int rows_per_image, const void *row_add,
+                     int64_t ld_add, void *y, int64_t ldy, void *y2, int64_t ldy2, int M, int E, int F, int dtype, void *stream);
 
 void ape_gemm_set_trace(long long *device_buffer);
 
```
